# ylongqi/openrec

Measured on NVIDIA H100. Metric: bpr_triplets_per_sec, higher is better.
Workload: dtype f32

## Files before the change

include/orx.h:

```cpp
#ifndef ORX_H_
#define ORX_H_

#include <stdint.h>

#ifdef __cplusplus
extern "C" {
#endif

#define ORX_ABI_VERSION 1
#define ORX_API __attribute__((visibility("default")))

typedef struct orx_ctx* orx_handle_t;
typedef void* orx_stream_t;

enum orx_status {
  ORX_OK = 0,
  ORX_ERR_INVALID = -1,
  ORX_ERR_CUDA = -2,
  ORX_ERR_UNSUPPORTED = -3,
  ORX_ERR_NOMEM = -4
};

enum orx_pair_kind { ORX_PAIR_BPR = 0, ORX_PAIR_UCML = 1 };
enum orx_point_kind { ORX_POINT_GMF = 0, ORX_POINT_WRMF = 1 };
enum orx_score_kind { ORX_SCORE_DOT = 0, ORX_SCORE_NEG_SQDIST = 1 };

enum orx_opt_kind { ORX_OPT_SGD = 0, ORX_OPT_ADAGRAD = 1, ORX_OPT_ADAM_LAZY = 2, ORX_OPT_ADAM_DENSE = 3 };

typedef struct {
  int32_t kind;
  float lr, eps, beta1, beta2;
  int64_t step;
} orx_opt_t;

typedef struct {
  float* var;
  float* s0;
  float* s1;
  int64_t rows;
  int32_t dim;
} orx_table_t;

ORX_API int orx_abi_version(void);
ORX_API const char* orx_last_error_string(void);
ORX_API int orx_create(int device, orx_handle_t* out);
ORX_API int orx_destroy(orx_handle_t h);
ORX_API int orx_device_count(int* n_out_host);
ORX_API int orx_stream_synchronize(orx_handle_t h, orx_stream_t stream);
ORX_API int orx_debug_set_epoch(orx_handle_t h, uint32_t epoch);
enum orx_dispatch_op {
  ORX_OP_GEMM = 0,
  ORX_OP_INTERACT_FWD = 1,
  ORX_OP_INTERACT_BWD = 2,
  ORX_OP_PAIRWISE_STEP = 3,
  ORX_OP_POINTWISE_STEP = 4
};
enum orx_dispatch_variant {
  ORX_VARIANT_GEMM_TMA = 0,
  ORX_VARIANT_GEMM_SIMT = 1,
  ORX_VARIANT_INTERACT_WARP = 2,
  ORX_VARIANT_INTERACT = 3,
  ORX_VARIANT_STEP = 4,
  ORX_VARIANT_STEP_PIPE = 5,
  ORX_VARIANT_STEP_GENERIC = 6
};
#define ORX_DISPATCH_LOG_CAP 64
ORX_API int orx_debug_dispatch_log(orx_handle_t h, int32_t* rec_host, int32_t cap, int32_t* n_host);

ORX_API int orx_profile_enable(orx_handle_t h, int32_t on);
ORX_API int orx_profile_read(orx_handle_t h, float* ms_host, int32_t n_phases, int32_t* n_steps_host);

ORX_API int orx_fill_uniform(orx_handle_t h, float* dst, int64_t n, float lo, float hi, uint64_t seed, orx_stream_t s);
ORX_API int orx_gather(orx_handle_t h, const float* tab, int64_t rows, int32_t dim, const void* ids, int32_t id_is_i64,
               int64_t n, float* out, int32_t* n_bad, orx_stream_t s);
ORX_API int orx_censor(orx_handle_t h, float* tab, int64_t rows, int32_t dim, const int32_t* ids, int32_t n,
               float min_norm, orx_stream_t s);

ORX_API int orx_pairwise_step(orx_handle_t h, int32_t kind, const orx_table_t* user, const orx_table_t* item,
                      const orx_table_t* item_bias, const int32_t* uid, const int32_t* pid, const int32_t* nid,
                      int32_t B, float margin, float c_loss, float c_l2, const orx_opt_t* opt_host,
                      float* out4, orx_stream_t s);
ORX_API int orx_pairwise_step_host(orx_handle_t h, int32_t kind, const orx_table_t* user, const orx_table_t* item,
                           const orx_table_t* item_bias, const int32_t* uid_host, const int32_t* pid_host,
                           const int32_t* nid_host, int32_t B, float margin, float c_loss, float c_l2,
                           const orx_opt_t* opt_host, float* out4_host, orx_stream_t s);
ORX_API int orx_pairwise_prefetch(orx_handle_t h, const orx_table_t* user, const orx_table_t* item, const int32_t* uid,
                                  const int32_t* pid, const int32_t* nid, int32_t B, int32_t opt_kind, int32_t ids_ready,
                                  orx_stream_t ids_stream);
ORX_API int orx_pairwise_fwd(orx_handle_t h, int32_t kind, const orx_table_t* user, const orx_table_t* item,
                     const orx_table_t* item_bias, const int32_t* uid, const int32_t* pid, const int32_t* nid,
                     int32_t B, float margin, float* out4, orx_stream_t s);
ORX_API int orx_pairwise_grad(orx_handle_t h, int32_t kind, const orx_table_t* user, const orx_table_t* item,
                      const orx_table_t* item_bias, const int32_t* uid, const int32_t* pid, const int32_t* nid,
                      int32_t B, float margin, float c_loss, float c_l2, float* d_user, float* d_pos, float* d_neg,
                      float* d_bp, float* d_bn, float* g_out, orx_stream_t s);

ORX_API int orx_pointwise_step(orx_handle_t h, int32_t kind, const orx_table_t* user, const orx_table_t* item,
                       const orx_table_t* item_bias, const orx_table_t* w, const int32_t* uid, const int32_t* iid,
                       const float* label, int32_t B, float a, float b, int32_t use_sigmoid, float c_loss,
                       float c_l2, const orx_opt_t* opt_host, float* out4, orx_stream_t s);
ORX_API int orx_pointwise_fwd(orx_handle_t h, int32_t kind, const orx_table_t* user, const orx_table_t* item,
                      const orx_table_t* item_bias, const orx_table_t* w, const int32_t* uid, const int32_t* iid,
                      const float* label, int32_t B, float a, float b, int32_t use_sigmoid, float* out4,
                      orx_stream_t s);
ORX_API int orx_pointwise_grad(orx_handle_t h, int32_t kind, const orx_table_t* user, const orx_table_t* item,
                       const orx_table_t* item_bias, const orx_table_t* w, const int32_t* uid, const int32_t* iid,
                       const float* label, int32_t B, float a, float b, int32_t use_sigmoid, float c_loss,
                       float c_l2, float* d_user, float* d_item, float* d_bias, float* d_w, float* g_out,
                       orx_stream_t s);

ORX_API int orx_sparse_apply(orx_handle_t h, const orx_table_t* tab, const int32_t* ids, const float* values,
                             int32_t n, const orx_opt_t* opt_host, orx_stream_t s);
ORX_API int orx_sparse_apply_strided(orx_handle_t h, const orx_table_t* tab, const int32_t* ids, int64_t id_stride,
                                     const float* values, int64_t value_ld, int32_t n, const orx_opt_t* opt_host,
                                     orx_stream_t s);
ORX_API int orx_owner_bucket_combined(orx_handle_t h, const int32_t* ids, int32_t n, int32_t n_user, int64_t total_users,
                                      int32_t world, int32_t* counts, int32_t* send_local, int32_t* slot, orx_stream_t s);
ORX_API int orx_pairwise_grad_rows(orx_handle_t h, int32_t kind, const float* rows, int64_t ld, int32_t dim,
                                   const int32_t* uslot, const int32_t* pslot, const int32_t* nslot, int32_t B,
                                   float margin, float c_loss, float c_l2, float inv_B, float* d_rows, float* out4,
                                   orx_stream_t s);

typedef struct {
  int32_t world, rank, dim, batch_cap, home_cap, req_cap, gin_cap, timeout_ms;
  void *tripbox, *idbox, *got, *gotb, *gin, *ginb, *meta, *flags;
} orx_shard_t;
ORX_API int orx_peer_alloc(orx_handle_t h, int64_t bytes, void** dev_ptr_out, uint8_t* handle_out64);
ORX_API int orx_peer_open(orx_handle_t h, const uint8_t* handle64, void** dev_ptr_out);
ORX_API int orx_peer_close(orx_handle_t h, void* dev_ptr);
ORX_API int orx_peer_free(orx_handle_t h, void* dev_ptr);
ORX_API int orx_shard_sizes(const orx_shard_t* x_host, int64_t* n8_host);
ORX_API int orx_shard_step(orx_handle_t h, int32_t kind, const orx_shard_t* x_host, const orx_table_t* user,
                           const orx_table_t* item, const orx_table_t* item_bias, const int32_t* uid, const int32_t* pid,
                           const int32_t* nid, int32_t B, const int32_t* next_uid, const int32_t* next_pid,
                           const int32_t* next_nid, int32_t next_B, int64_t total_users, int64_t total_items, float margin,
                           float c_loss, float c_l2, float inv_B, const orx_opt_t* opt_host, int32_t epoch,
                           int32_t phase_lo, int32_t phase_hi, float* out4, orx_stream_t s);
ORX_API int orx_dense_apply(orx_handle_t h, float* var, float* s0, float* s1, const float* grad, int64_t n,
                    const orx_opt_t* opt_host, orx_stream_t s);

ORX_API int orx_gather_strided(orx_handle_t h, const float* tab, int64_t rows, int32_t dim, const int32_t* ids,
                               int64_t id_stride, int64_t n, float* out, int64_t out_ld, int32_t* n_bad,
                               orx_stream_t s);
ORX_API int orx_mlp_layer_fwd(orx_handle_t h, const float* x, int64_t ldx, int32_t B, int32_t in, const float* w,
                              const float* bias, int32_t out, int32_t act, float* y, int64_t ldy, orx_stream_t s);
ORX_API int orx_mlp_layer_bwd(orx_handle_t h, const float* x, int64_t ldx, const float* y, int64_t ldy, const float* w,
                              int32_t B, int32_t in, int32_t out, int32_t act, float* dy, int64_t lddy, float* dx,
                              int64_t lddx, float* dw, float* db, orx_stream_t s);
ORX_API int orx_interact_fwd(orx_handle_t h, const float* emb, int64_t emb_ld, const float* dense, int64_t dense_ld,
                             int32_t B, int32_t F, int32_t D, int32_t self_interaction, int32_t mode, float* out,
// ... 37 lines not shown
```

openrec_b200/_lib.py:

```python
from __future__ import annotations

import ctypes as C
import os

HERE = os.path.dirname(os.path.abspath(__file__))
LIB_PATH = os.path.join(HERE, "csrc", "liborx.so")

ORX_PAIR_BPR, ORX_PAIR_UCML = 0, 1
ORX_POINT_GMF, ORX_POINT_WRMF = 0, 1
ORX_SCORE_DOT, ORX_SCORE_NEG_SQDIST = 0, 1
ORX_OPT_SGD, ORX_OPT_ADAGRAD, ORX_OPT_ADAM_LAZY, ORX_OPT_ADAM_DENSE = 0, 1, 2, 3
ORX_OP_GEMM, ORX_OP_INTERACT_FWD, ORX_OP_INTERACT_BWD, ORX_OP_PAIRWISE_STEP, ORX_OP_POINTWISE_STEP = 0, 1, 2, 3, 4
ORX_VARIANT_GEMM_TMA, ORX_VARIANT_GEMM_SIMT, ORX_VARIANT_INTERACT_WARP, ORX_VARIANT_INTERACT = 0, 1, 2, 3
ORX_VARIANT_STEP, ORX_VARIANT_STEP_PIPE, ORX_VARIANT_STEP_GENERIC = 4, 5, 6
ORX_DISPATCH_LOG_CAP = 64


class OrxOpt(C.Structure):
    _fields_ = [("kind", C.c_int32), ("lr", C.c_float), ("eps", C.c_float), ("beta1", C.c_float),
                ("beta2", C.c_float), ("step", C.c_int64)]


class OrxTable(C.Structure):
    _fields_ = [("var", C.c_void_p), ("s0", C.c_void_p), ("s1", C.c_void_p), ("rows", C.c_int64),
                ("dim", C.c_int32)]


class OrxShard(C.Structure):
    _fields_ = [("world", C.c_int32), ("rank", C.c_int32), ("dim", C.c_int32), ("batch_cap", C.c_int32),
                ("home_cap", C.c_int32), ("req_cap", C.c_int32), ("gin_cap", C.c_int32), ("timeout_ms", C.c_int32),
                ("tripbox", C.c_void_p), ("idbox", C.c_void_p), ("got", C.c_void_p), ("gotb", C.c_void_p),
                ("gin", C.c_void_p), ("ginb", C.c_void_p), ("meta", C.c_void_p), ("flags", C.c_void_p)]


class OrxSampler(C.Structure):
    _fields_ = [("rec_user", C.c_void_p), ("rec_item", C.c_void_p), ("perm_cur", C.c_void_p), ("perm_next", C.c_void_p),
                ("cursor", C.c_int64), ("n_records", C.c_int64), ("csr_off", C.c_void_p), ("csr_items", C.c_void_p),
                ("total_users", C.c_int32), ("total_items", C.c_int32)]


_vp, _i32, _i64, _f, _u64 = C.c_void_p, C.c_int32, C.c_int64, C.c_float, C.c_uint64
_T = C.POINTER(OrxTable)
_O = C.POINTER(OrxOpt)
_S = C.POINTER(OrxShard)

SIGNATURES = {
    "orx_abi_version": [],
    "orx_last_error_string": [],
    "orx_create": [C.c_int, C.POINTER(_vp)],
    "orx_destroy": [_vp],
    "orx_device_count": [C.POINTER(C.c_int)],
    "orx_stream_synchronize": [_vp, _vp],
    "orx_debug_set_epoch": [_vp, C.c_uint32],
    "orx_debug_dispatch_log": [_vp, C.POINTER(_i32), _i32, C.POINTER(_i32)],
    "orx_profile_enable": [_vp, _i32],
    "orx_profile_read": [_vp, C.POINTER(C.c_float), _i32, C.POINTER(_i32)],
    "orx_fill_uniform": [_vp, _vp, _i64, _f, _f, _u64, _vp],
    "orx_gather": [_vp, _vp, _i64, _i32, _vp, _i32, _i64, _vp, _vp, _vp],
    "orx_censor": [_vp, _vp, _i64, _i32, _vp, _i32, _f, _vp],
    "orx_pairwise_step": [_vp, _i32, _T, _T, _T, _vp, _vp, _vp, _i32, _f, _f, _f, _O, _vp, _vp],
    "orx_pairwise_step_host": [_vp, _i32, _T, _T, _T, _vp, _vp, _vp, _i32, _f, _f, _f, _O, _vp, _vp],
    "orx_pairwise_prefetch": [_vp, _T, _T, _vp, _vp, _vp, _i32, _i32, _i32, _vp],
    "orx_pairwise_fwd": [_vp, _i32, _T, _T, _T, _vp, _vp, _vp, _i32, _f, _vp, _vp],
    "orx_pairwise_grad": [_vp, _i32, _T, _T, _T, _vp, _vp, _vp, _i32, _f, _f, _f, _vp, _vp, _vp, _vp, _vp, _vp, _vp],
    "orx_sparse_apply": [_vp, _T, _vp, _vp, _i32, _O, _vp],
    "orx_sparse_apply_strided": [_vp, _T, _vp, _i64, _vp, _i64, _i32, _O, _vp],
    "orx_gather_strided": [_vp, _vp, _i64, _i32, _vp, _i64, _i64, _vp, _i64, _vp, _vp],
    "orx_mlp_layer_fwd": [_vp, _vp, _i64, _i32, _i32, _vp, _vp, _i32, _i32, _vp, _i64, _vp],
    "orx_mlp_layer_bwd": [_vp, _vp, _i64, _vp, _i64, _vp, _i32, _i32, _i32, _i32, _vp, _i64, _vp, _i64, _vp, _vp, _vp],
    "orx_interact_fwd": [_vp, _vp, _i64, _vp, _i64, _i32, _i32, _i32, _i32, _i32, _vp, _i64, _vp],
    "orx_interact_bwd": [_vp, _vp, _i64, _vp, _i64, _vp, _i64, _i32, _i32, _i32, _i32, _i32, _vp, _i64, _vp, _i64,
                         _vp],
    "orx_pred_loss": [_vp, _vp, _vp, _i32, _i32, _f, _vp, _vp, _vp, _vp],
    "orx_peer_alloc": [_vp, _i64, C.POINTER(_vp), C.c_char_p],
    "orx_peer_open": [_vp, C.c_char_p, C.POINTER(_vp)],
    "orx_peer_close": [_vp, _vp],
    "orx_peer_free": [_vp, _vp],
    "orx_shard_sizes": [_S, C.POINTER(_i64)],
    "orx_shard_step": [_vp, _i32, _S, _T, _T, _T, _vp, _vp, _vp, _i32, _vp, _vp, _vp, _i32, _i64, _i64, _f, _f, _f, _f, _O,
                       _i32, _i32, _i32, _vp, _vp],
    "orx_owner_bucket_combined": [_vp, _vp, _i32, _i32, _i64, _i32, _vp, _vp, _vp, _vp],
    "orx_pairwise_grad_rows": [_vp, _i32, _vp, _i64, _i32, _vp, _vp, _vp, _i32, _f, _f, _f, _f, _vp, _vp, _vp],
    "orx_pointwise_step": [_vp, _i32, _T, _T, _T, _T, _vp, _vp, _vp, _i32, _f, _f, _i32, _f, _f, _O, _vp, _vp],
    "orx_pointwise_fwd": [_vp, _i32, _T, _T, _T, _T, _vp, _vp, _vp, _i32, _f, _f, _i32, _vp, _vp],
    "orx_pointwise_grad": [_vp, _i32, _T, _T, _T, _T, _vp, _vp, _vp, _i32, _f, _f, _i32, _f, _f,
                           _vp, _vp, _vp, _vp, _vp, _vp],
    "orx_dense_apply": [_vp, _vp, _vp, _vp, _vp, _i64, _O, _vp],
    "orx_score_all": [_vp, _i32, _vp, _i64, _vp, _i32, _vp, _vp, _vp, _i64, _i32, _vp, _vp],
    "orx_sample_pairwise": [_vp, C.POINTER(OrxSampler), _u64, _i64, _i32, _vp, _vp, _vp, _vp],
    "orx_sample_stratified": [_vp, C.POINTER(OrxSampler), _u64, _i64, _i32, _f, _vp, _vp, _vp, _vp, _vp],
    "orx_sample_per_positive": [_vp, C.POINTER(OrxSampler), _u64, _i64, _i32, _i32, _vp, _vp, _vp, _vp],
    "orx_rank_metrics": [_vp, _vp, _vp, _vp, _i32, _i64, C.POINTER(_i32), _i32, _vp, _vp, _vp, _vp],
}

_lib = None


def lib():
    global _lib
    if _lib is None:
        if not os.path.exists(LIB_PATH):
            raise RuntimeError(
                f"liborx.so not found at {LIB_PATH}: build it with `python -m openrec_b200.build` "
                "(there is no CPU fallback)")
        l = C.CDLL(LIB_PATH)
        for name, argtypes in SIGNATURES.items():
            fn = getattr(l, name)
            fn.argtypes = argtypes
            fn.restype = C.c_char_p if name == "orx_last_error_string" else C.c_int
        _lib = l
    return _lib


def last_error() -> str:
    s = lib().orx_last_error_string()
    return s.decode() if s else ""


def check(rc: int, what: str = "liborx"):
    if rc != 0:
        raise RuntimeError(f"{what} failed (status {rc}): {last_error()}")
```

openrec_b200/csrc/orx_common.cuh:

```cuda
#pragma once
#include <cuda_runtime.h>
#include <stdint.h>
#include <stdio.h>

#include <initializer_list>
#include <type_traits>

#include "../../include/orx.h"

void orx_set_error(const char* fmt, ...);

#define ORX_CUDA(call)                                                                         \
  do {                                                                                         \
    cudaError_t e__ = (call);                                                                  \
    if (e__ != cudaSuccess) {                                                                  \
      orx_set_error("%s:%d %s -> %s", __FILE__, __LINE__, #call, cudaGetErrorString(e__));     \
      return ORX_ERR_CUDA;                                                                     \
    }                                                                                          \
  } while (0)

#define ORX_REQUIRE(cond, msg)                                  \
  do {                                                          \
    if (!(cond)) {                                              \
      orx_set_error("%s: %s", __func__, msg);                   \
      return ORX_ERR_INVALID;                                   \
    }                                                           \
  } while (0)

#define ORX_LAUNCH_CHECK() ORX_CUDA(cudaGetLastError())

struct OrxHash {
  unsigned long long* slots;
  int32_t* didx;
  int32_t* did;
  int32_t* counter;
  uint32_t mask;
  int32_t shift;
  uint32_t epoch;
};

struct orx_ctx {
  int device;
  int num_sms;
  int64_t cap_B;
  OrxHash hu, hi;
  OrxHash pf_u[2], pf_i[2];
  int32_t* counters;
  float *gu, *gi, *gb, *gw;
  int64_t g_rows_u, g_rows_i;
  int32_t g_dim;
  float* partials;
  int32_t cap_partials;
  int32_t* ids_stage[2];
  float* out_stage[2];
  int64_t stage_cap;
  uint32_t stage_flip;
  int prof_on, prof_n, prof_cap;
  int prof_step;
  cudaEvent_t* prof_ev;
  int32_t* bucket_cursor;
  cudaStream_t side_stream;
  cudaEvent_t side_ev;
  cudaEvent_t pf_done[2], pf_free[2], stage_free[2];
  int pf_free_valid[2], stage_free_valid[2];
  int pf_valid, pf_set, pf_next, pf_B, pf_mode;
  const int32_t *pf_uid, *pf_pid, *pf_nid;
  int64_t pf_rows_u, pf_rows_i;
  uint32_t epoch;
  void* shard_ws;
  int32_t dispatch[ORX_DISPATCH_LOG_CAP][8];
  int64_t dispatch_n;
};

static inline void orx_log_dispatch(orx_ctx* c, int op, int variant, int TA, int TB, int M, int N, int K, int S) {
  int32_t* r = c->dispatch[c->dispatch_n++ % ORX_DISPATCH_LOG_CAP];
  r[0] = op; r[1] = variant; r[2] = TA; r[3] = TB; r[4] = M; r[5] = N; r[6] = K; r[7] = S;
}

int orx_next_epoch(orx_ctx* c, cudaStream_t st);
void orx_shard_ws_release(orx_ctx* c);

#define ORX_PROF_EV 8
static inline bool orx_prof_sampled(const orx_ctx* c) {
  return c->prof_on && (c->prof_step & 7) == 0 && c->prof_n < c->prof_cap;
}
static inline void orx_prof_mark(orx_ctx* c, int k, cudaStream_t st) {
  if (orx_prof_sampled(c)) cudaEventRecord(c->prof_ev[c->prof_n * ORX_PROF_EV + k], st);
}
static inline void orx_prof_next(orx_ctx* c) {
  if (!c->prof_on) return;
  if (orx_prof_sampled(c)) c->prof_n++;
  c->prof_step++;
}

static inline int orx_current_sms() {
  static int sms[64] = {0};
  int dev = 0;
  if (cudaGetDevice(&dev) != cudaSuccess || dev < 0 || dev >= 64) return 132;
  if (sms[dev] <= 0 && cudaDeviceGetAttribute(&sms[dev], cudaDevAttrMultiProcessorCount, dev) != cudaSuccess) sms[dev] = 0;
  return sms[dev] > 0 ? sms[dev] : 132;
}

int orx_ensure_workspace(orx_ctx* c, int64_t B, int32_t dim);
int orx_ensure_stage(orx_ctx* c, int64_t n_ints);

template <int V, int... Vs, typename F>
static inline auto orx_dispatch(int v, F&& f) {
  if constexpr (sizeof...(Vs) == 0) {
    return f(std::integral_constant<int, V>{});
  } else {
    if (v == V) return f(std::integral_constant<int, V>{});
    return orx_dispatch<Vs...>(v, f);
  }
}
template <typename F>
static inline auto orx_dispatch_opt(int opt_kind, F&& f) {
  return orx_dispatch<ORX_OPT_SGD, ORX_OPT_ADAGRAD, ORX_OPT_ADAM_LAZY, ORX_OPT_ADAM_DENSE>(opt_kind, f);
}

static inline bool orx_opt_kind_ok(int kind) { return kind >= ORX_OPT_SGD && kind <= ORX_OPT_ADAM_DENSE; }
bool orx_opt_slots_ok(int kind, std::initializer_list<const orx_table_t*> tabs);

struct OrxOptDev {
  int32_t kind;
  float lr;
  float eps, beta1, beta2;
};

#ifdef __CUDACC__

#define ORX_FULL 0xffffffffu

__device__ __forceinline__ void orx_pdl_wait() { asm volatile("griddepcontrol.wait;" ::: "memory"); }
__device__ __forceinline__ void orx_pdl_trigger() { asm volatile("griddepcontrol.launch_dependents;" ::: "memory"); }

bool orx_pdl_enabled();

template <typename... KArgs, typename... Args>
static inline cudaError_t orx_launch_pdl(void (*kern)(KArgs...), dim3 grid, dim3 block, size_t smem, cudaStream_t st,
                                         Args... args) {
  cudaLaunchConfig_t cfg = {};
  cfg.gridDim = grid;
  cfg.blockDim = block;
  cfg.dynamicSmemBytes = smem;
  cfg.stream = st;
  cudaLaunchAttribute attr[1];
  attr[0].id = cudaLaunchAttributeProgrammaticStreamSerialization;
  attr[0].val.programmaticStreamSerializationAllowed = 1;
  cfg.attrs = attr;
  cfg.numAttrs = orx_pdl_enabled() ? 1 : 0;
// ... 243 lines not shown
  float *U, *Us0, *Us1;
  float *I, *Is0, *Is1;
  float *Bv, *Bs0, *Bs1;
  int D;
  OrxOptDev opt;
  OrxHash hu, hi;
  float *gu, *gi, *gb;
  const float* partials;
  int n_partials;
  float loss_scale;
  int32_t* counters;
  float* out4;
  float *W, *Ws0, *Ws1, *gw;
  float c_l2;
};

#ifdef __CUDACC__
template <int OPT>
__device__ __forceinline__ void orx_tail_rows(const TailArgs& a, int nu, int ni) {
  typedef OrxOptSlots<OPT> SL;
  constexpr bool ZERO_ONLY = SL::STAGE_ONLY;
  const int lane = threadIdx.x & 31;
  const int gwarp = (blockIdx.x * blockDim.x + threadIdx.x) >> 5;
  const int nwarps = (gridDim.x * blockDim.x) >> 5;
  const int D = a.D;
  const float4 z4 = make_float4(0.f, 0.f, 0.f, 0.f);
  const int sub = lane >> 3, sl = lane & 7;
  for (int r0 = gwarp * 4; r0 < nu + ni; r0 += nwarps * 4) {
    const int r = r0 + sub;
    const bool on = r < nu + ni;
    const bool is_u = on && r < nu;
    const int d = on ? (is_u ? r : r - nu) : 0;
    const int id = on ? (is_u ? a.hu.did[d] : a.hi.did[d]) : 0;
    float* G = (is_u ? a.gu : a.gi) + (int64_t)d * D;
    float* W = (is_u ? a.U : a.I) + (int64_t)id * D;
    float* P0 = (is_u ? a.Us0 : a.Is0) + (int64_t)id * D;
    float* P1 = (is_u ? a.Us1 : a.Is1) + (int64_t)id * D;
    if ((D & 3) == 0) {
      const int nq = D >> 2;
      for (int e0 = 0; e0 < nq; e0 += 32) {
        float4 g[4], w[4], s0v[4], s1v[4];
#pragma unroll
        for (int k = 0; k < 4; ++k) {
          const int e = e0 + sl + 8 * k;
          const bool ld = on && e < nq;
          g[k] = ld ? __ldcg(reinterpret_cast<const float4*>(G) + e) : z4;
          w[k] = (ld && !ZERO_ONLY) ? orx_ld4_stream(W + 4 * e) : z4;
          s0v[k] = (ld && SL::S0) ? orx_ld4_stream(P0 + 4 * e) : z4;
          s1v[k] = (ld && SL::S1) ? orx_ld4_stream(P1 + 4 * e) : z4;
        }
#pragma unroll
        for (int k = 0; k < 4; ++k) {
          const int e = e0 + sl + 8 * k;
          if (!on || e >= nq) continue;
          if (!ZERO_ONLY) {
            orx_st4_stream(W + 4 * e, orx_apply4<OPT>(w[k], g[k], s0v[k], s1v[k], a.opt));
            if (SL::S0) orx_st4_stream(P0 + 4 * e, s0v[k]);
            if (SL::S1) orx_st4_stream(P1 + 4 * e, s1v[k]);
          }
          __stcg(reinterpret_cast<float4*>(G) + e, z4);
        }
      }
    } else if (on) {
      for (int e = sl; e < D; e += 8) {
        if (!ZERO_ONLY) orx_update1<OPT>(W + e, P0 + e, P1 + e, W[e], G[e], a.opt);
        G[e] = 0.f;
      }
    }
    if (on && !is_u && sl == 0) {
      if (!ZERO_ONLY) orx_update1<OPT>(a.Bv + id, a.Bs0 + id, a.Bs1 + id, a.Bv[id], a.gb[d], a.opt);
      a.gb[d] = 0.f;
    }
  }
}
#endif

OrxOptDev orx_opt_to_dev(const orx_opt_t* o);
int orx_launch_index_build_strided(orx_ctx* c, const int32_t* a, int64_t stride, int64_t rows, int32_t n,
                                   bool stage_all, cudaStream_t st);
TailArgs orx_tail_args(const orx_ctx* c, const orx_table_t* user, const orx_table_t* item, const orx_table_t* bias,
                       const OrxHash& hu, const OrxHash& hi, const OrxOptDev& o);
int orx_launch_adam_sweeps(orx_ctx* c, const orx_table_t* user, const orx_table_t* item, const orx_table_t* bias,
                           const OrxHash& hu, const OrxHash& hi, const OrxOptDev& o, cudaStream_t st);
int orx_launch_tail(orx_ctx* c, const TailArgs& ta, int opt_kind, cudaStream_t st);
int orx_ensure_partials(orx_ctx* c, int need, cudaStream_t st);
int orx_launch_reduce_partials(const float* partials, int n, float loss_scale, float* out4, cudaStream_t st);
int orx_launch_index_build(orx_ctx* c, const int32_t* a, int64_t rows_a, const int32_t* b0, const int32_t* b1,
                           int64_t rows_b, int32_t n, int mode , cudaStream_t st);
```

openrec_b200/csrc/orx_ctx.cu:

```cuda
#include <stdarg.h>
#include <stdlib.h>
#include <string.h>

#include "orx_common.cuh"

static thread_local char g_err[512] = "";

void orx_set_error(const char* fmt, ...) {
  va_list ap;
  va_start(ap, fmt);
  vsnprintf(g_err, sizeof(g_err), fmt, ap);
  va_end(ap);
}

extern "C" const char* orx_last_error_string(void) { return g_err; }

bool orx_pdl_enabled() {
  static int v = -1;
  if (v < 0) {
    const char* e = getenv("ORX_PDL");
    v = (e && atoi(e) == 0) ? 0 : 1;
  }
  return v != 0;
}
extern "C" int orx_abi_version(void) { return ORX_ABI_VERSION; }

extern "C" int orx_device_count(int* n) {
  ORX_REQUIRE(n != nullptr, "null output");
  *n = 0;
  ORX_CUDA(cudaGetDeviceCount(n));
  return ORX_OK;
}

static void free_hash(OrxHash& t) {
  cudaFree(t.slots);
  cudaFree(t.didx);
  cudaFree(t.did);
  t.slots = nullptr;
  t.didx = nullptr;
  t.did = nullptr;
}

static void free_workspace(orx_ctx* c) {
  free_hash(c->hu);
  free_hash(c->hi);
  for (int k = 0; k < 2; ++k) {
    free_hash(c->pf_u[k]);
    free_hash(c->pf_i[k]);
  }
  cudaFree(c->gu);
  cudaFree(c->gi);
  cudaFree(c->gb);
  cudaFree(c->gw);
  c->gu = c->gi = c->gb = c->gw = nullptr;
  c->cap_B = 0;
  c->g_dim = 0;
}

static uint32_t pow2_at_least(int64_t n) {
  uint32_t p = 1024;
  while ((int64_t)p < n) p <<= 1;
  return p;
}

static int alloc_hash(OrxHash& t, int64_t lookups, int32_t* counter) {
  uint32_t cap = pow2_at_least(4 * lookups);
  int lg = 0;
  while ((1u << lg) < cap) ++lg;
  t.mask = cap - 1;
  t.shift = 32 - lg;
  t.counter = counter;
  ORX_CUDA(cudaMalloc(&t.slots, sizeof(unsigned long long) * cap));
  ORX_CUDA(cudaMalloc(&t.didx, sizeof(int32_t) * cap));
  ORX_CUDA(cudaMalloc(&t.did, sizeof(int32_t) * (lookups + 1)));
  ORX_CUDA(cudaMemset(t.slots, 0, sizeof(unsigned long long) * cap));
  return ORX_OK;
}

int orx_ensure_workspace(orx_ctx* c, int64_t B, int32_t dim) {
  if (B <= c->cap_B && dim <= c->g_dim) return ORX_OK;
  int64_t nb = B > c->cap_B ? B : c->cap_B;
  int32_t nd = dim > c->g_dim ? dim : c->g_dim;
  ORX_CUDA(cudaDeviceSynchronize());
  free_workspace(c);
  int rc;
  if ((rc = alloc_hash(c->hu, nb, c->counters + 0)) != ORX_OK) return rc;
  if ((rc = alloc_hash(c->hi, 2 * nb, c->counters + 1)) != ORX_OK) return rc;
  for (int k = 0; k < 2; ++k) {
    if ((rc = alloc_hash(c->pf_u[k], nb, c->counters + 4 * (1 + k))) != ORX_OK) return rc;
    if ((rc = alloc_hash(c->pf_i[k], 2 * nb, c->counters + 4 * (1 + k) + 1)) != ORX_OK) return rc;
  }
  c->pf_valid = 0;
  c->pf_free_valid[0] = c->pf_free_valid[1] = 0;
  c->g_rows_u = nb;
  c->g_rows_i = 2 * nb;
  size_t bu = sizeof(float) * (size_t)c->g_rows_u * nd, bi = sizeof(float) * (size_t)c->g_rows_i * nd;
  ORX_CUDA(cudaMalloc(&c->gu, bu));
  ORX_CUDA(cudaMalloc(&c->gi, bi));
  ORX_CUDA(cudaMalloc(&c->gb, sizeof(float) * (size_t)c->g_rows_i));
  ORX_CUDA(cudaMalloc(&c->gw, sizeof(float) * (size_t)nd));
  ORX_CUDA(cudaMemset(c->gu, 0, bu));
  ORX_CUDA(cudaMemset(c->gi, 0, bi));
  ORX_CUDA(cudaMemset(c->gb, 0, sizeof(float) * (size_t)c->g_rows_i));
  ORX_CUDA(cudaMemset(c->gw, 0, sizeof(float) * (size_t)nd));
  ORX_CUDA(cudaMemset(c->counters, 0, sizeof(int32_t) * 16));
  ORX_CUDA(cudaDeviceSynchronize());
  c->cap_B = nb;
  c->g_dim = nd;
  c->epoch = 0;
  return ORX_OK;
}

static int zero_hash(OrxHash& t) {
  if (!t.slots) return ORX_OK;
  ORX_CUDA(cudaMemset(t.slots, 0, sizeof(unsigned long long) * ((size_t)t.mask + 1)));
  return ORX_OK;
}

int orx_next_epoch(orx_ctx* c, cudaStream_t ) {
  c->epoch = (c->epoch + 1) & 0x7fffffffu;
  if (c->epoch == 0) {
    ORX_CUDA(cudaDeviceSynchronize());
    int rc;
    if ((rc = zero_hash(c->hu)) || (rc = zero_hash(c->hi))) return rc;
    for (int k = 0; k < 2; ++k)
      if ((rc = zero_hash(c->pf_u[k])) || (rc = zero_hash(c->pf_i[k]))) return rc;
    ORX_CUDA(cudaDeviceSynchronize());
    c->epoch = 1;
  }
  c->hu.epoch = c->hi.epoch = c->epoch;
  return ORX_OK;
}

extern "C" int orx_debug_set_epoch(orx_handle_t h, uint32_t epoch) {
  ORX_REQUIRE(h != nullptr && epoch < 0x80000000u, "null handle / epoch must be < 2^31");
  h->epoch = epoch;
  return ORX_OK;
}

extern "C" int orx_debug_dispatch_log(orx_handle_t h, int32_t* rec, int32_t cap, int32_t* n) {
  ORX_REQUIRE(h != nullptr && n && cap >= 0 && (rec || cap == 0), "bad arguments");
  const int64_t held = h->dispatch_n < ORX_DISPATCH_LOG_CAP ? h->dispatch_n : ORX_DISPATCH_LOG_CAP;
  const int64_t first = h->dispatch_n - held;
  const int64_t take = held < cap ? held : cap;
  for (int64_t i = 0; i < take; ++i) memcpy(rec + 8 * i, h->dispatch[(first + i) % ORX_DISPATCH_LOG_CAP], 8 * sizeof(int32_t));
  *n = (int32_t)take;
  h->dispatch_n = 0;
  return ORX_OK;
}

int orx_ensure_stage(orx_ctx* c, int64_t n_ints) {
  if (n_ints <= c->stage_cap) return ORX_OK;
  ORX_CUDA(cudaDeviceSynchronize());
  for (int i = 0; i < 2; ++i) {
    cudaFree(c->ids_stage[i]);
    c->ids_stage[i] = nullptr;
    ORX_CUDA(cudaMalloc(&c->ids_stage[i], sizeof(int32_t) * (size_t)n_ints));
  }
  c->stage_cap = n_ints;
  return ORX_OK;
}

extern "C" int orx_create(int device, orx_handle_t* out) {
  ORX_REQUIRE(out != nullptr, "null output handle");
  *out = nullptr;
  int n = 0;
  ORX_CUDA(cudaGetDeviceCount(&n));
  ORX_REQUIRE(device >= 0 && device < n, "device ordinal out of range");
  ORX_CUDA(cudaSetDevice(device));
  cudaDeviceProp prop;
  ORX_CUDA(cudaGetDeviceProperties(&prop, device));
  if (prop.major != 9 || prop.minor != 0) {
    orx_set_error("orx_create: liborx is built for sm_90a only; device %d is sm_%d%d", device, prop.major,
                  prop.minor);
    return ORX_ERR_UNSUPPORTED;
  }
  orx_ctx* c = new orx_ctx();
  memset(c, 0, sizeof(*c));
  c->device = device;
  c->num_sms = prop.multiProcessorCount;
  c->cap_partials = c->num_sms * 64;
  if (cudaMalloc(&c->counters, sizeof(int32_t) * 16) != cudaSuccess ||
      cudaMalloc(&c->partials, sizeof(float) * 2 * (size_t)c->cap_partials) != cudaSuccess ||
      cudaMalloc(&c->out_stage[0], sizeof(float) * 8) != cudaSuccess ||
      cudaMalloc(&c->out_stage[1], sizeof(float) * 8) != cudaSuccess) {
    orx_set_error("orx_create: workspace allocation failed: %s", cudaGetErrorString(cudaGetLastError()));
    delete c;
    return ORX_ERR_NOMEM;
  }
  cudaMemset(c->counters, 0, sizeof(int32_t) * 16);
  *out = c;
  return ORX_OK;
}

extern "C" int orx_destroy(orx_handle_t h) {
  if (!h) return ORX_OK;
  cudaSetDevice(h->device);
  cudaDeviceSynchronize();
  free_workspace(h);
  for (int i = 0; i < 2; ++i) {
    cudaFree(h->ids_stage[i]);
    cudaFree(h->out_stage[i]);
  }
  cudaFree(h->counters);
  cudaFree(h->partials);
  cudaFree(h->bucket_cursor);
  orx_shard_ws_release(h);
  if (h->side_stream) {
    cudaStreamDestroy(h->side_stream);
    cudaEventDestroy(h->side_ev);
    for (int i = 0; i < 2; ++i) {
      cudaEventDestroy(h->pf_done[i]);
      cudaEventDestroy(h->pf_free[i]);
      cudaEventDestroy(h->stage_free[i]);
    }
  }
  if (h->prof_ev) {
    for (int i = 0; i < h->prof_cap * ORX_PROF_EV; ++i) cudaEventDestroy(h->prof_ev[i]);
    delete[] h->prof_ev;
  }
  delete h;
  return ORX_OK;
}

extern "C" int orx_profile_enable(orx_handle_t h, int32_t on) {
  ORX_REQUIRE(h != nullptr, "null handle");
  ORX_CUDA(cudaSetDevice(h->device));
  if (on && !h->prof_ev) {
    h->prof_cap = 1024;
    h->prof_ev = new cudaEvent_t[h->prof_cap * ORX_PROF_EV];
    for (int i = 0; i < h->prof_cap * ORX_PROF_EV; ++i) ORX_CUDA(cudaEventCreate(&h->prof_ev[i]));
  }
  h->prof_on = on ? 1 : 0;
// ... 49 lines not shown
```

openrec_b200/csrc/orx_dlrm.cu:

```cuda
#include "orx_common.cuh"

__global__ void __launch_bounds__(256) k_gather_strided(const float* __restrict__ tab, int64_t rows, int D,
                                                        const int32_t* __restrict__ ids, int64_t id_stride, int64_t n,
                                                        float* __restrict__ out, int64_t out_ld, int32_t* n_bad) {
  const int lane = threadIdx.x & 31;
  const int64_t nw = ((int64_t)gridDim.x * blockDim.x) >> 5;
  const bool vec = ((D & 3) == 0) && ((out_ld & 3) == 0);
  for (int64_t b = ((int64_t)blockIdx.x * blockDim.x + threadIdx.x) >> 5; b < n; b += nw) {
    const int64_t id = ids[b * id_stride];
    const bool ok = id >= 0 && id < rows;
    if (!ok && lane == 0 && n_bad) atomicAdd(n_bad, 1);
    if (vec) {
      const float4* src = reinterpret_cast<const float4*>(tab + id * D);
      float4* dst = reinterpret_cast<float4*>(out + b * out_ld);
      for (int e = lane; e < D / 4; e += 32) dst[e] = ok ? __ldg(src + e) : make_float4(0.f, 0.f, 0.f, 0.f);
    } else {
      for (int e = lane; e < D; e += 32) out[b * out_ld + e] = ok ? __ldg(tab + id * D + e) : 0.f;
    }
  }
}

extern "C" int orx_gather_strided(orx_handle_t h, const float* tab, int64_t rows, int32_t dim, const int32_t* ids,
                                  int64_t id_stride, int64_t n, float* out, int64_t out_ld, int32_t* n_bad,
                                  orx_stream_t s) {
  ORX_REQUIRE(h != nullptr && tab && ids && out, "null pointer");
  ORX_REQUIRE(rows > 0 && dim > 0 && n >= 0 && id_stride >= 1 && out_ld >= dim, "bad sizes");
  if (n == 0) return ORX_OK;
  ORX_CUDA(cudaSetDevice(h->device));
  int64_t blocks = (n + 7) / 8;
  if (blocks > (int64_t)h->num_sms * 32) blocks = (int64_t)h->num_sms * 32;
  k_gather_strided<<<(int)blocks, 256, 0, (cudaStream_t)s>>>(tab, rows, dim, ids, id_stride, n, out, out_ld, n_bad);
  ORX_LAUNCH_CHECK();
  return ORX_OK;
}

#define ORX_MAX_F 64

__device__ __forceinline__ bool inter_selected(int mode, int self, int i, int j) {
  return mode == 0 ? (self ? j >= i : j > i) : (self ? j <= i : j < i);
}

__device__ __forceinline__ int inter_index(int mode, int self, int F, int i, int j) {
  if (mode == 0) return self ? i * F - i * (i - 1) / 2 + (j - i) : i * (F - 1) - i * (i - 1) / 2 + (j - i - 1);
  return self ? i * (i + 1) / 2 + j : i * (i - 1) / 2 + j;
}

__device__ __forceinline__ void inter_load(const float* __restrict__ emb, int64_t emb_ld, const float* __restrict__ dense,
                                           int64_t dense_ld, int b, int F, int D, float* sz) {
  const int warp = threadIdx.x >> 5, lane = threadIdx.x & 31, nw = blockDim.x >> 5, Dp = D + 1;
  for (int f = warp; f < F; f += nw) {
    const float* src = f < F - 1 ? emb + (int64_t)b * emb_ld + (int64_t)f * D : dense + (int64_t)b * dense_ld;
    for (int d = lane; d < D; d += 32) sz[f * Dp + d] = src[d];
  }
}

__global__ void __launch_bounds__(128) k_interact_fwd(const float* __restrict__ emb, int64_t emb_ld,
                                                      const float* __restrict__ dense, int64_t dense_ld, int B, int F,
                                                      int D, int self, int mode, float* __restrict__ out,
                                                      int64_t out_ld) {
  extern __shared__ float sz[];
  const int b = blockIdx.x;
  if (b >= B) return;
  const int Dp = D + 1;
  inter_load(emb, emb_ld, dense, dense_ld, b, F, D, sz);
  __syncthreads();
  for (int c = threadIdx.x; c < F * F; c += blockDim.x) {
    const int i = c / F, j = c - i * F;
    if (!inter_selected(mode, self, i, j)) continue;
    float a0 = 0.f, a1 = 0.f, a2 = 0.f, a3 = 0.f;
    if (mode == 1 || j == i) {
      const float* zi = sz + i * Dp;
      const float* zj = sz + j * Dp;
      int d = 0;
      for (; d + 3 < D; d += 4) {
        a0 += zi[d] * zj[d];
        a1 += zi[d + 1] * zj[d + 1];
        a2 += zi[d + 2] * zj[d + 2];
        a3 += zi[d + 3] * zj[d + 3];
      }
      for (; d < D; ++d) a0 += zi[d] * zj[d];
    }
    out[(int64_t)b * out_ld + inter_index(mode, self, F, i, j)] = (a0 + a1) + (a2 + a3);
  }
}

__global__ void __launch_bounds__(128) k_interact_bwd(const float* __restrict__ emb, int64_t emb_ld,
                                                      const float* __restrict__ dense, int64_t dense_ld,
                                                      const float* __restrict__ dout, int64_t dout_ld, int B, int F,
                                                      int D, int self, int mode, float* __restrict__ demb,
                                                      int64_t demb_ld, float* __restrict__ ddense,
                                                      int64_t ddense_ld) {
  extern __shared__ float sm[];
  const int b = blockIdx.x;
  if (b >= B) return;
  const int Dp = D + 1;
  float* sz = sm;
  float* sp = sm + F * Dp;
  inter_load(emb, emb_ld, dense, dense_ld, b, F, D, sz);
  for (int c = threadIdx.x; c < F * F; c += blockDim.x) {
    const int i = c / F, j = c - i * F;
    float v = 0.f;
    if (inter_selected(mode, self, i, j) && (mode == 1 || j == i))
      v = dout[(int64_t)b * dout_ld + inter_index(mode, self, F, i, j)];
    sp[c] = v;
  }
  __syncthreads();
  const int warp = threadIdx.x >> 5, lane = threadIdx.x & 31, nw = blockDim.x >> 5;
  for (int i = warp; i < F; i += nw) {
    for (int d = lane; d < D; d += 32) {
      float acc = 0.f;
      for (int j = 0; j < F; ++j) acc += (sp[i * F + j] + sp[j * F + i]) * sz[j * Dp + d];
// ... 74 lines not shown
        const bool up = lane & 1;
        const float send = up ? v[0] : v[1], keep = up ? v[1] : v[0];
        v[0] = keep + __shfl_xor_sync(0xffffffffu, send, 1);
      }
      if (p0 + lane < P) out[(int64_t)b * out_ld + p0 + lane] = v[0];
    }
  }
}

__global__ void __launch_bounds__(INTER_WARPS * 32) k_interact_bwd_warp(const float* __restrict__ emb, int64_t emb_ld,
                                                                        const float* __restrict__ dense, int64_t dense_ld,
                                                                        const float* __restrict__ dout, int64_t dout_ld,
                                                                        int B, int F, int D, int self,
                                                                        float* __restrict__ demb, int64_t demb_ld,
                                                                        float* __restrict__ ddense, int64_t ddense_ld) {
  extern __shared__ float4 sb_all[];
  constexpr int WLD = 36;
  const int lane = threadIdx.x & 31, wi = threadIdx.x >> 5;
  const size_t per_warp = (size_t)F * 32 + (size_t)F * WLD / 4;
  float4* sz = sb_all + (size_t)wi * per_warp;
  float* sw = reinterpret_cast<float*>(sz + (size_t)F * 32);
  const int nq = D >> 2;
  for (int b = blockIdx.x * INTER_WARPS + wi; b < B; b += gridDim.x * INTER_WARPS) {
    __syncwarp();
    inter_load_warp(emb, emb_ld, dense, dense_ld, b, F, D, lane, sz);
    for (int c = lane; c < F * WLD; c += 32) sw[c] = 0.f;
    __syncwarp();
    const int P = self ? F * (F + 1) / 2 : F * (F - 1) / 2;
    for (int p = lane; p < P; p += 32) {
      int i = (int)((sqrtf(8.f * (float)p + 1.f) - 1.f) * 0.5f) + (self ? 0 : 1);
      while ((self ? i * (i + 1) / 2 : i * (i - 1) / 2) > p) --i;
      while ((self ? (i + 1) * (i + 2) / 2 : (i + 1) * i / 2) <= p) ++i;
      const int j = p - (self ? i * (i + 1) / 2 : i * (i - 1) / 2);
      const float g = dout[(int64_t)b * dout_ld + p];
      if (i == j) sw[j * WLD + i] = 2.f * g;
      else { sw[j * WLD + i] = g; sw[i * WLD + j] = g; }
    }
    __syncwarp();
    for (int i0 = 0; i0 < F; i0 += 9) {
      float4 acc[9];
#pragma unroll
      for (int k = 0; k < 9; ++k) acc[k] = make_float4(0.f, 0.f, 0.f, 0.f);
      for (int j = 0; j < F; ++j) {
        const float4 zj = sz[j * 32 + lane];
        const float* wr = sw + j * WLD + i0;
        float wv[9];
#pragma unroll
        for (int k = 0; k < 9; ++k) wv[k] = wr[k];
#pragma unroll
        for (int k = 0; k < 9; ++k) {
          acc[k].x += wv[k] * zj.x; acc[k].y += wv[k] * zj.y; acc[k].z += wv[k] * zj.z; acc[k].w += wv[k] * zj.w;
        }
      }
      if (lane < nq) {
#pragma unroll
        for (int k = 0; k < 9; ++k) {
          const int i = i0 + k;
          if (i >= F) break;
          if (i < F - 1) {
            reinterpret_cast<float4*>(demb + (int64_t)b * demb_ld + (int64_t)i * D)[lane] = acc[k];
          } else {
            float4* dd = reinterpret_cast<float4*>(ddense + (int64_t)b * ddense_ld) + lane;
            float4 o = *dd;
            o.x += acc[k].x; o.y += acc[k].y; o.z += acc[k].z; o.w += acc[k].w;
            *dd = o;
          }
        }
      }
    }
  }
}

static bool inter_fast_ok(int F, int D, int mode, const void* a, const void* b, int64_t lda, int64_t ldb) {
  return mode == 1 && F >= 2 && F <= 32 && (D & 3) == 0 && D <= 128 && (lda & 3) == 0 && (ldb & 3) == 0 &&
         ((((uintptr_t)a) | ((uintptr_t)b)) & 15) == 0;
}

extern "C" int orx_interact_fwd(orx_handle_t h, const float* emb, int64_t emb_ld, const float* dense,
                                int64_t dense_ld, int32_t B, int32_t F, int32_t D, int32_t self_interaction,
                                int32_t mode, float* out, int64_t out_ld, orx_stream_t s) {
  ORX_REQUIRE(h != nullptr && dense && out && (F == 1 || emb), "null pointer");
  ORX_REQUIRE(B >= 0 && F >= 1 && F <= ORX_MAX_F && D > 0 && (mode == 0 || mode == 1), "bad sizes/mode");
  if (B == 0) return ORX_OK;
  ORX_CUDA(cudaSetDevice(h->device));
  if (inter_fast_ok(F, D, mode, emb ? (const void*)emb : (const void*)dense, dense, emb_ld, dense_ld)) {
    const size_t sm = sizeof(float4) * (size_t)INTER_WARPS * F * 32;
    static bool attr = false;
    if (!attr) { ORX_CUDA(cudaFuncSetAttribute(k_interact_fwd_warp, cudaFuncAttributeMaxDynamicSharedMemorySize, 200 * 1024)); attr = true; }
    int grid = (B + INTER_WARPS - 1) / INTER_WARPS;
    if (grid > h->num_sms * 4) grid = h->num_sms * 4;
    k_interact_fwd_warp<<<grid, INTER_WARPS * 32, sm, (cudaStream_t)s>>>(emb, emb_ld, dense, dense_ld, B, F, D, self_interaction, out, out_ld);
    ORX_LAUNCH_CHECK();
    orx_log_dispatch(h, ORX_OP_INTERACT_FWD, ORX_VARIANT_INTERACT_WARP, 0, 0, B, F, D, 1);
    return ORX_OK;
  }
  const size_t smem = sizeof(float) * (size_t)F * (D + 1);
  ORX_REQUIRE(smem <= 200 * 1024, "F*D too large for the interaction kernel");
  if (smem > 48 * 1024) ORX_CUDA(cudaFuncSetAttribute(k_interact_fwd, cudaFuncAttributeMaxDynamicSharedMemorySize, (int)smem));
  k_interact_fwd<<<B, 128, smem, (cudaStream_t)s>>>(emb, emb_ld, dense, dense_ld, B, F, D, self_interaction, mode, out, out_ld);
  ORX_LAUNCH_CHECK();
  orx_log_dispatch(h, ORX_OP_INTERACT_FWD, ORX_VARIANT_INTERACT, 0, 0, B, F, D, 1);
  return ORX_OK;
}

extern "C" int orx_interact_bwd(orx_handle_t h, const float* emb, int64_t emb_ld, const float* dense,
                                int64_t dense_ld, const float* dout, int64_t dout_ld, int32_t B, int32_t F, int32_t D,
                                int32_t self_interaction, int32_t mode, float* demb, int64_t demb_ld, float* ddense,
                                int64_t ddense_ld, orx_stream_t s) {
  ORX_REQUIRE(h != nullptr && dense && dout && ddense && (F == 1 || (emb && demb)), "null pointer");
  ORX_REQUIRE(B >= 0 && F >= 1 && F <= ORX_MAX_F && D > 0 && (mode == 0 || mode == 1), "bad sizes/mode");
  if (B == 0) return ORX_OK;
  ORX_CUDA(cudaSetDevice(h->device));
  if (inter_fast_ok(F, D, mode, emb ? (const void*)emb : (const void*)dense, dense, emb_ld, dense_ld) && (demb_ld & 3) == 0 &&
      (ddense_ld & 3) == 0 && ((((uintptr_t)(demb ? (const void*)demb : (const void*)ddense)) | ((uintptr_t)ddense)) & 15) == 0) {
    const size_t sm = (size_t)INTER_WARPS * (sizeof(float4) * (size_t)F * 32 + sizeof(float) * (size_t)F * 36);
    static bool attr = false;
    if (!attr) { ORX_CUDA(cudaFuncSetAttribute(k_interact_bwd_warp, cudaFuncAttributeMaxDynamicSharedMemorySize, 200 * 1024)); attr = true; }
    int grid = (B + INTER_WARPS - 1) / INTER_WARPS;
    if (grid > h->num_sms * 3) grid = h->num_sms * 3;
    k_interact_bwd_warp<<<grid, INTER_WARPS * 32, sm, (cudaStream_t)s>>>(emb, emb_ld, dense, dense_ld, dout, dout_ld, B, F, D, self_interaction, demb, demb_ld, ddense, ddense_ld);
    ORX_LAUNCH_CHECK();
    orx_log_dispatch(h, ORX_OP_INTERACT_BWD, ORX_VARIANT_INTERACT_WARP, 0, 0, B, F, D, 1);
    return ORX_OK;
  }
  const size_t smem = sizeof(float) * ((size_t)F * (D + 1) + (size_t)F * F);
  ORX_REQUIRE(smem <= 200 * 1024, "F*D too large for the interaction kernel");
  if (smem > 48 * 1024) ORX_CUDA(cudaFuncSetAttribute(k_interact_bwd, cudaFuncAttributeMaxDynamicSharedMemorySize, (int)smem));
  k_interact_bwd<<<B, 128, smem, (cudaStream_t)s>>>(emb, emb_ld, dense, dense_ld, dout, dout_ld, B, F, D, self_interaction, mode, demb, demb_ld, ddense, ddense_ld);
  ORX_LAUNCH_CHECK();
  orx_log_dispatch(h, ORX_OP_INTERACT_BWD, ORX_VARIANT_INTERACT, 0, 0, B, F, D, 1);
  return ORX_OK;
}

template <int TA, int TB>
__global__ void __launch_bounds__(256) k_gemm(const float* __restrict__ A, int64_t lda, const float* __restrict__ Bm,
                                              int64_t ldb, float* __restrict__ C, int64_t ldc, int M, int N, int K,
                                              const float* __restrict__ bias, int act, float* __restrict__ part) {
  constexpr int T = 64, KC = 16;
  __shared__ float sa[KC][T + 4], sb[KC][T + 4];
  const int tx = threadIdx.x & 15, ty = threadIdx.x >> 4;
  const int m0 = blockIdx.y * T, n0 = blockIdx.x * T;
  float acc[4][4];
#pragma unroll
  for (int i = 0; i < 4; ++i)
#pragma unroll
    for (int j = 0; j < 4; ++j) acc[i][j] = 0.f;
  const int kper = ((K + (int)gridDim.z - 1) / (int)gridDim.z + KC - 1) / KC * KC;
  const int k_lo = blockIdx.z * kper, k_hi = min(K, k_lo + kper);
  for (int k0 = k_lo; k0 < k_hi; k0 += KC) {
    for (int e = threadIdx.x; e < T * KC; e += 256) {
      int r, k;
      if (TA == 0) { r = e / KC; k = e % KC; } else { k = e / T; r = e % T; }
      float v = 0.f;
      if (m0 + r < M && k0 + k < k_hi) v = TA == 0 ? A[(int64_t)(m0 + r) * lda + k0 + k] : A[(int64_t)(k0 + k) * lda + m0 + r];
      sa[k][r] = v;
    }
    for (int e = threadIdx.x; e < T * KC; e += 256) {
      int c, k;
      if (TB == 0) { k = e / T; c = e % T; } else { c = e / KC; k = e % KC; }
      float v = 0.f;
      if (n0 + c < N && k0 + k < k_hi) v = TB == 0 ? Bm[(int64_t)(k0 + k) * ldb + n0 + c] : Bm[(int64_t)(n0 + c) * ldb + k0 + k];
      sb[k][c] = v;
    }
    __syncthreads();
#pragma unroll
    for (int k = 0; k < KC; ++k) {
      float a[4], b[4];
#pragma unroll
      for (int i = 0; i < 4; ++i) a[i] = sa[k][ty * 4 + i];
#pragma unroll
      for (int j = 0; j < 4; ++j) b[j] = sb[k][tx + 16 * j];
#pragma unroll
      for (int i = 0; i < 4; ++i)
#pragma unroll
        for (int j = 0; j < 4; ++j) acc[i][j] += a[i] * b[j];
    }
    __syncthreads();
  }
#pragma unroll
  for (int i = 0; i < 4; ++i) {
    const int m = m0 + ty * 4 + i;
    if (m >= M) continue;
#pragma unroll
    for (int j = 0; j < 4; ++j) {
      const int n = n0 + tx + 16 * j;
      if (n >= N) continue;
      if (gridDim.z > 1) {
        part[(size_t)blockIdx.z * (size_t)M * (size_t)N + (size_t)m * N + n] = acc[i][j];
        continue;
      }
      float v = acc[i][j] + (bias ? bias[n] : 0.f);
      if (act == 1) v = fmaxf(v, 0.f);
      else if (act == 2) v = orx_sigmoid(v);
      C[(int64_t)m * ldc + n] = v;
    }
  }
}

int orx_launch_gemm_tc(orx_ctx* h, int TA, int TB, const float* A, int64_t lda, const float* Bm, int64_t ldb, float* C,
                       int64_t ldc, int M, int N, int K, const float* bias, int act, cudaStream_t st);
float* orx_splitk_workspace(size_t floats);
int orx_launch_splitk_reduce(const float* part, int S, int M, int N, float* C, int64_t ldc, const float* bias, int act,
                             cudaStream_t st);

template <int TA, int TB>
static int launch_gemm(orx_ctx* h, const float* A, int64_t lda, const float* Bm, int64_t ldb, float* C, int64_t ldc, int M,
                       int N, int K, const float* bias, int act, cudaStream_t st) {
  const int rc = orx_launch_gemm_tc(h, TA, TB, A, lda, Bm, ldb, C, ldc, M, N, K, bias, act, st);
  if (rc != ORX_ERR_UNSUPPORTED) return rc;
  const int tiles = ((N + 63) / 64) * ((M + 63) / 64);
  int S = 1;
  const int sms = orx_current_sms();
  if (tiles < sms && K >= 1024) {
    S = (2 * sms + tiles - 1) / tiles;
    if (S > K / 256) S = K / 256;
    if (S > 65535) S = 65535;
  }
  float* part = nullptr;
  if (S > 1) {
    part = orx_splitk_workspace((size_t)S * (size_t)M * (size_t)N);
    if (!part) { orx_set_error("split-K workspace allocation failed"); return ORX_ERR_CUDA; }
  }
  dim3 grid((N + 63) / 64, (M + 63) / 64, S);
  k_gemm<TA, TB><<<grid, 256, 0, st>>>(A, lda, Bm, ldb, C, ldc, M, N, K, bias, act, part);
  ORX_LAUNCH_CHECK();
  orx_log_dispatch(h, ORX_OP_GEMM, ORX_VARIANT_GEMM_SIMT, TA, TB, M, N, K, S);
  if (S > 1) return orx_launch_splitk_reduce(part, S, M, N, C, ldc, bias, act, st);
  return ORX_OK;
}

extern "C" int orx_mlp_layer_fwd(orx_handle_t h, const float* x, int64_t ldx, int32_t B, int32_t in, const float* w,
                                 const float* bias, int32_t out, int32_t act, float* y, int64_t ldy, orx_stream_t s) {
  ORX_REQUIRE(h != nullptr && x && w && y, "null pointer");
  ORX_REQUIRE(B >= 0 && in > 0 && out > 0 && ldx >= in && ldy >= out && act >= 0 && act <= 2, "bad sizes");
  if (B == 0) return ORX_OK;
  ORX_CUDA(cudaSetDevice(h->device));
  return launch_gemm<0, 0>(h, x, ldx, w, out, y, ldy, B, out, in, bias, act, (cudaStream_t)s);
}

__global__ void k_act_bwd(const float* __restrict__ y, int64_t ldy, float* __restrict__ dy, int64_t lddy, int B,
                          int N, int act) {
  const int64_t i = (int64_t)blockIdx.x * blockDim.x + threadIdx.x;
  if (i >= (int64_t)B * N) return;
  const int b = (int)(i / N), n = (int)(i % N);
  const float yv = y[(int64_t)b * ldy + n];
  float g = dy[(int64_t)b * lddy + n];
  if (act == 1) g = yv > 0.f ? g : 0.f;
  else if (act == 2) g = g * yv * (1.f - yv);
  dy[(int64_t)b * lddy + n] = g;
}

__global__ void __launch_bounds__(256) k_col_sum(const float* __restrict__ dz, int64_t ld, int B, int N,
                                                 float* __restrict__ out) {
  __shared__ float sh[8][33];
  const int n = blockIdx.x * 32 + (threadIdx.x & 31), r = threadIdx.x >> 5;
  const int per = (B + (int)gridDim.y - 1) / (int)gridDim.y;
  const int b_lo = blockIdx.y * per, b_hi = min(B, b_lo + per);
  float acc = 0.f;
  if (n < N)
    for (int b = b_lo + r; b < b_hi; b += 8) acc += dz[(int64_t)b * ld + n];
  sh[r][threadIdx.x & 31] = acc;
  __syncthreads();
  if (r == 0 && n < N) {
    float t = 0.f;
    for (int k = 0; k < 8; ++k) t += sh[k][threadIdx.x & 31];
    out[(size_t)blockIdx.y * N + n] = t;
  }
}

extern "C" int orx_mlp_layer_bwd(orx_handle_t h, const float* x, int64_t ldx, const float* y, int64_t ldy,
                                 const float* w, int32_t B, int32_t in, int32_t out, int32_t act, float* dy,
                                 int64_t lddy, float* dx, int64_t lddx, float* dw, float* db, orx_stream_t s) {
  ORX_REQUIRE(h != nullptr && x && y && w && dy && dw, "null pointer");
  ORX_REQUIRE(B > 0 && in > 0 && out > 0 && act >= 0 && act <= 2, "bad sizes");
  ORX_CUDA(cudaSetDevice(h->device));
  cudaStream_t st = (cudaStream_t)s;
  if (act != 0) {
    const int64_t n = (int64_t)B * out;
    k_act_bwd<<<(unsigned)((n + 255) / 256), 256, 0, st>>>(y, ldy, dy, lddy, B, out, act);
    ORX_LAUNCH_CHECK();
  }
  if (db) {
    const int cb = (out + 31) / 32;
    int S = 1;
    if (B >= 4096) {
      S = (2 * h->num_sms + cb - 1) / cb;
      if (S > B / 256) S = B / 256;
    }
    if (S > 1) {
      float* part = orx_splitk_workspace((size_t)S * (size_t)out);
      if (!part) { orx_set_error("split workspace allocation failed"); return ORX_ERR_CUDA; }
      k_col_sum<<<dim3(cb, S), 256, 0, st>>>(dy, lddy, B, out, part);
      ORX_LAUNCH_CHECK();
      const int rc2 = orx_launch_splitk_reduce(part, S, 1, out, db, out, nullptr, 0, st);
      if (rc2) return rc2;
    } else {
      k_col_sum<<<cb, 256, 0, st>>>(dy, lddy, B, out, db);
      ORX_LAUNCH_CHECK();
    }
  }
  int rc = launch_gemm<1, 0>(h, x, ldx, dy, lddy, dw, out, in, out, B, nullptr, 0, st);
  if (rc) return rc;
  if (dx) rc = launch_gemm<0, 1>(h, dy, lddy, w, out, dx, lddx, B, in, out, nullptr, 0, st);
  return rc;
}

__global__ void __launch_bounds__(256) k_pred_loss(const float* __restrict__ pred, const float* __restrict__ label,
                                                   int B, int kind, float thr, float* __restrict__ pred_out,
                                                   float* __restrict__ dpred, float* partials) {
  __shared__ float sh[256];
  float acc = 0.f;
  const float invB = 1.f / (float)B;
  for (int b = blockIdx.x * blockDim.x + threadIdx.x; b < B; b += gridDim.x * blockDim.x) {
    float p = pred[b];
    float pass = 1.f;
    if (thr > 0.f && thr < 1.f) {
      pass = (p >= thr && p <= 1.f - thr) ? 1.f : 0.f;
      p = fminf(fmaxf(p, thr), 1.f - thr);
    }
    const float y = label[b];
    float d;
    if (kind == 0) {
      acc += (y - p) * (y - p);
      d = 2.f * (p - y) * invB;
    } else {
      const float eps = 1e-7f;
      const float ph = fminf(fmaxf(p, eps), 1.f - eps);
      acc += -(y * logf(ph + eps) + (1.f - y) * logf(1.f - ph + eps));
      d = (p >= eps && p <= 1.f - eps) ? -(y / (ph + eps) - (1.f - y) / (1.f - ph + eps)) * invB : 0.f;
    }
    if (pred_out) pred_out[b] = p;
    if (dpred) dpred[b] = d * pass;
  }
  sh[threadIdx.x] = acc;
  __syncthreads();
  for (int s = 128; s > 0; s >>= 1) {
    if (threadIdx.x < s) sh[threadIdx.x] += sh[threadIdx.x + s];
    __syncthreads();
  }
  if (threadIdx.x == 0) {
    partials[2 * blockIdx.x] = sh[0];
    partials[2 * blockIdx.x + 1] = 0.f;
  }
}

extern "C" int orx_pred_loss(orx_handle_t h, const float* pred, const float* label, int32_t B, int32_t kind,
                             float clip_threshold, float* pred_out, float* dpred, float* out4, orx_stream_t s) {
  ORX_REQUIRE(h != nullptr && pred && label && out4, "null pointer");
  ORX_REQUIRE(B > 0 && (kind == 0 || kind == 1), "bad sizes/kind");
  ORX_CUDA(cudaSetDevice(h->device));
  cudaStream_t st = (cudaStream_t)s;
  int blocks = (B + 255) / 256;
  if (blocks > 256) blocks = 256;
  int rc = orx_ensure_partials(h, blocks, st);
  if (rc) return rc;
  k_pred_loss<<<blocks, 256, 0, st>>>(pred, label, B, kind, clip_threshold, pred_out, dpred, h->partials);
  ORX_LAUNCH_CHECK();
  return orx_launch_reduce_partials(h->partials, blocks, 1.0f / (float)B, out4, st);
}
```

openrec_b200/csrc/orx_misc.cu:

```cuda
#include "orx_common.cuh"

__device__ __forceinline__ uint64_t splitmix64(uint64_t x) {
  x += 0x9E3779B97F4A7C15ull;
  x = (x ^ (x >> 30)) * 0xBF58476D1CE4E5B9ull;
  x = (x ^ (x >> 27)) * 0x94D049BB133111EBull;
  return x ^ (x >> 31);
}

__global__ void k_fill_uniform(float* dst, int64_t n, float lo, float hi, uint64_t seed) {
  const int64_t stride = (int64_t)gridDim.x * blockDim.x;
  const float top = nextafterf(hi, lo);
  for (int64_t i = (int64_t)blockIdx.x * blockDim.x + threadIdx.x; i < n; i += stride) {
    const uint64_t r = splitmix64(seed * 0xD1342543DE82EF95ull + (uint64_t)i);
    const float u = (float)(r >> 40) * (1.0f / 16777216.0f);
    dst[i] = fminf(lo + (hi - lo) * u, top);
  }
}

extern "C" int orx_fill_uniform(orx_handle_t h, float* dst, int64_t n, float lo, float hi, uint64_t seed,
                                orx_stream_t s) {
  ORX_REQUIRE(h != nullptr && dst != nullptr && n >= 0, "null handle/dst or negative n");
  if (n == 0) return ORX_OK;
  ORX_CUDA(cudaSetDevice(h->device));
  int64_t blocks = (n + 1023) / 1024;
  if (blocks > (int64_t)h->num_sms * 16) blocks = (int64_t)h->num_sms * 16;
  k_fill_uniform<<<(int)blocks, 256, 0, (cudaStream_t)s>>>(dst, n, lo, hi, seed);
  ORX_LAUNCH_CHECK();
  return ORX_OK;
}

template <typename IdT>
__global__ void __launch_bounds__(256) k_gather(const float* __restrict__ tab, int64_t rows, int D,
                                                const IdT* __restrict__ ids, int64_t n, float* __restrict__ out,
                                                int32_t* n_bad) {
  const int lane = threadIdx.x & 31;
  const int64_t nw = ((int64_t)gridDim.x * blockDim.x) >> 5;
  const bool vec = (D & 3) == 0;
  for (int64_t b = ((int64_t)blockIdx.x * blockDim.x + threadIdx.x) >> 5; b < n; b += nw) {
    const int64_t id = (int64_t)ids[b];
    const bool ok = id >= 0 && id < rows;
    if (!ok && lane == 0 && n_bad) atomicAdd(n_bad, 1);
    if (vec) {
      const float4* src = reinterpret_cast<const float4*>(tab + id * D);
      float4* dst = reinterpret_cast<float4*>(out + b * D);
      for (int e = lane; e < D / 4; e += 32) dst[e] = ok ? __ldg(src + e) : make_float4(0.f, 0.f, 0.f, 0.f);
    } else {
      for (int e = lane; e < D; e += 32) out[b * D + e] = ok ? __ldg(tab + id * D + e) : 0.f;
    }
  }
}

extern "C" int orx_gather(orx_handle_t h, const float* tab, int64_t rows, int32_t dim, const void* ids,
                          int32_t id_is_i64, int64_t n, float* out, int32_t* n_bad, orx_stream_t s) {
  ORX_REQUIRE(h != nullptr && tab, "null pointer");
  ORX_REQUIRE(rows > 0 && dim > 0 && n >= 0, "bad sizes");
  if (n == 0) return ORX_OK;
  ORX_REQUIRE(ids && out, "null pointer");
  ORX_CUDA(cudaSetDevice(h->device));
  int64_t blocks = (n + 7) / 8;
  if (blocks > (int64_t)h->num_sms * 32) blocks = (int64_t)h->num_sms * 32;
  if (id_is_i64)
    k_gather<int64_t><<<(int)blocks, 256, 0, (cudaStream_t)s>>>(tab, rows, dim, (const int64_t*)ids, n, out, n_bad);
  else
    k_gather<int32_t><<<(int)blocks, 256, 0, (cudaStream_t)s>>>(tab, rows, dim, (const int32_t*)ids, n, out, n_bad);
  ORX_LAUNCH_CHECK();
  return ORX_OK;
}

__global__ void __launch_bounds__(256) k_censor(float* tab, int64_t rows, int D, const int32_t* __restrict__ ids,
                                                int n, float min_norm, OrxHash hsh) {
  const int lane = threadIdx.x & 31;
  const int nw = (gridDim.x * blockDim.x) >> 5;
  const bool vec = (D & 3) == 0 && D <= 128;
  for (int b0 = ((blockIdx.x * blockDim.x + threadIdx.x) >> 5) * 8; b0 < n; b0 += nw * 8) {
    int32_t my_id = -1;
    if (lane < 8 && b0 + lane < n) {
      const int32_t id = ids[b0 + lane];
      if (id >= 0 && (int64_t)id < rows && orx_hash_insert(hsh, id, 2) == 0u) my_id = id;
    }
    if (vec) {
      const int nq = D >> 2;
      float4 v[8];
#pragma unroll
      for (int k = 0; k < 8; ++k) {
        const int32_t id = __shfl_sync(ORX_FULL, my_id, k);
        v[k] = (id >= 0 && lane < nq) ? __ldcg(reinterpret_cast<const float4*>(tab + (int64_t)id * D) + lane)
                                      : make_float4(0.f, 0.f, 0.f, 0.f);
      }
#pragma unroll
      for (int k = 0; k < 8; ++k) {
        const int32_t id = __shfl_sync(ORX_FULL, my_id, k);
        if (id < 0) continue;
        float sq = v[k].x * v[k].x + v[k].y * v[k].y + v[k].z * v[k].z + v[k].w * v[k].w;
        sq = orx_group_sum<32>(sq);
        const float den = fmaxf(sqrtf(sq), min_norm);
        if (lane < nq)
          __stcg(reinterpret_cast<float4*>(tab + (int64_t)id * D) + lane,
                 make_float4(v[k].x / den, v[k].y / den, v[k].z / den, v[k].w / den));
      }
    } else {
      for (int k = 0; k < 8; ++k) {
        const int32_t id = __shfl_sync(ORX_FULL, my_id, k);
        if (id < 0) continue;
        float* row = tab + (int64_t)id * D;
        float sq = 0.f;
        for (int e = lane; e < D; e += 32) sq += row[e] * row[e];
        sq = orx_group_sum<32>(sq);
        const float den = fmaxf(sqrtf(sq), min_norm);
        for (int e = lane; e < D; e += 32) row[e] = row[e] / den;
      }
    }
  }
}

extern "C" int orx_censor(orx_handle_t h, float* tab, int64_t rows, int32_t dim, const int32_t* ids, int32_t n,
                          float min_norm, orx_stream_t s) {
  ORX_REQUIRE(h != nullptr && tab && ids, "null pointer");
  ORX_REQUIRE(rows > 0 && dim > 0 && n >= 0, "bad sizes");
  if (n == 0) return ORX_OK;
  ORX_CUDA(cudaSetDevice(h->device));
  cudaStream_t st = (cudaStream_t)s;
  int rc = orx_ensure_workspace(h, n, h->g_dim > 0 ? h->g_dim : 1);
  if (rc) return rc;
  if ((rc = orx_next_epoch(h, st))) return rc;
  int blocks = (n + 63) / 64;
  if (blocks > h->num_sms * 8) blocks = h->num_sms * 8;
  k_censor<<<blocks, 256, 0, st>>>(tab, rows, dim, ids, n, min_norm, h->hu);
  ORX_LAUNCH_CHECK();
  return ORX_OK;
}

template <int OPT>
__global__ void k_dense_apply(float* var, float* s0, float* s1, const float* __restrict__ grad, int64_t n,
                              OrxOptDev o) {
  const int64_t stride = (int64_t)gridDim.x * blockDim.x;
  for (int64_t i = (int64_t)blockIdx.x * blockDim.x + threadIdx.x; i < n; i += stride)
    orx_update1<OPT>(var + i, s0 + i, s1 + i, var[i], grad[i], o);
}

extern "C" int orx_dense_apply(orx_handle_t h, float* var, float* s0, float* s1, const float* grad, int64_t n,
                               const orx_opt_t* opt, orx_stream_t s) {
  ORX_REQUIRE(h != nullptr && var && grad && opt, "null pointer");
  ORX_REQUIRE(n >= 0, "negative n");
  if (n == 0) return ORX_OK;
  ORX_CUDA(cudaSetDevice(h->device));
  const OrxOptDev o = orx_opt_to_dev(opt);
  int64_t blocks = (n + 255) / 256;
  if (blocks > (int64_t)h->num_sms * 16) blocks = (int64_t)h->num_sms * 16;
  cudaStream_t st = (cudaStream_t)s;
  ORX_REQUIRE(orx_opt_kind_ok(opt->kind), "unknown optimizer kind");
  const orx_table_t t = {var, s0, s1, n, 1};
  ORX_REQUIRE(orx_opt_slots_ok(opt->kind, {&t}), "optimizer slot rows missing");
  const int kind = opt->kind == ORX_OPT_ADAM_DENSE ? ORX_OPT_ADAM_LAZY : opt->kind;
  orx_dispatch<ORX_OPT_SGD, ORX_OPT_ADAGRAD, ORX_OPT_ADAM_LAZY>(kind, [&](auto O) {
    k_dense_apply<decltype(O)::value><<<(int)blocks, 256, 0, st>>>(var, s0, s1, grad, n, o);
  });
  ORX_LAUNCH_CHECK();
  return ORX_OK;
}

template <int KIND>
__global__ void __launch_bounds__(256) k_score_all(const float* __restrict__ user_tab, int64_t U,
                                                   const int32_t* __restrict__ uid, int Bu,
                                                   const float* __restrict__ scale, const float* __restrict__ item_tab,
                                                   const float* __restrict__ bias, int64_t I, int D,
                                                   float* __restrict__ scores) {
  constexpr int T = 64, KC = 16;
  __shared__ float su[KC][T + 1], si[KC][T + 1];
  const int tx = threadIdx.x & 15, ty = threadIdx.x >> 4;
  const int64_t i0 = (int64_t)blockIdx.x * T;
  const int u0 = blockIdx.y * T;
  float acc[4][4];
#pragma unroll
  for (int a = 0; a < 4; ++a)
#pragma unroll
    for (int b = 0; b < 4; ++b) acc[a][b] = 0.f;
  for (int k0 = 0; k0 < D; k0 += KC) {
    for (int e = threadIdx.x; e < T * KC; e += 256) {
      const int r = e / KC, k = e % KC;
      float uv = 0.f, iv = 0.f;
      if (k0 + k < D) {
        if (u0 + r < Bu) {
          const int32_t id = uid[u0 + r];
          if (id >= 0 && (int64_t)id < U) {
            uv = user_tab[(int64_t)id * D + k0 + k];
            if (scale) uv *= scale[k0 + k];
          }
        }
        if (i0 + r < I) iv = item_tab[(i0 + r) * D + k0 + k];
      }
      su[k][r] = uv;
      si[k][r] = iv;
    }
    __syncthreads();
#pragma unroll
    for (int k = 0; k < KC; ++k) {
      if (k0 + k < D) {
        float uu[4], ii[4];
#pragma unroll
        for (int a = 0; a < 4; ++a) uu[a] = su[k][ty * 4 + a];
#pragma unroll
        for (int b = 0; b < 4; ++b) ii[b] = si[k][tx + 16 * b];
#pragma unroll
        for (int a = 0; a < 4; ++a)
#pragma unroll
          for (int b = 0; b < 4; ++b) {
            if (KIND == ORX_SCORE_DOT) acc[a][b] += uu[a] * ii[b];
            else acc[a][b] -= (uu[a] - ii[b]) * (uu[a] - ii[b]);
          }
      }
    }
    __syncthreads();
  }
#pragma unroll
  for (int a = 0; a < 4; ++a) {
    const int u = u0 + ty * 4 + a;
    if (u >= Bu) continue;
#pragma unroll
    for (int b = 0; b < 4; ++b) {
      const int64_t i = i0 + tx + 16 * b;
      if (i < I) scores[(int64_t)u * I + i] = acc[a][b] + (bias ? bias[i] : 0.f);
    }
  }
}

extern "C" int orx_score_all(orx_handle_t h, int32_t kind, const float* user_tab, int64_t U, const int32_t* uid,
                             int32_t Bu, const float* scale, const float* item_tab, const float* item_bias, int64_t I,
                             int32_t dim, float* scores, orx_stream_t s) {
  ORX_REQUIRE(h != nullptr && user_tab && uid && item_tab && scores, "null pointer");
  ORX_REQUIRE(kind == ORX_SCORE_DOT || kind == ORX_SCORE_NEG_SQDIST, "unknown score kind");
  ORX_REQUIRE(U > 0 && I > 0 && dim > 0 && Bu >= 0, "bad sizes");
  if (Bu == 0) return ORX_OK;
  ORX_CUDA(cudaSetDevice(h->device));
  dim3 grid((unsigned)((I + 63) / 64), (unsigned)((Bu + 63) / 64));
  if (kind == ORX_SCORE_DOT)
    k_score_all<ORX_SCORE_DOT><<<grid, 256, 0, (cudaStream_t)s>>>(user_tab, U, uid, Bu, scale, item_tab, item_bias, I, dim, scores);
  else
    k_score_all<ORX_SCORE_NEG_SQDIST><<<grid, 256, 0, (cudaStream_t)s>>>(user_tab, U, uid, Bu, scale, item_tab, item_bias, I, dim, scores);
  ORX_LAUNCH_CHECK();
  return ORX_OK;
}

#define ORX_MAX_AT 8
struct RankArgs {
  const float* pred;
  const uint8_t *pos, *excl;
  int R;
  int64_t I;
  int at[ORX_MAX_AT];
  int n_at;
  float *auc, *ndcg, *recall;
};

__global__ void __launch_bounds__(256) k_rank_metrics(const RankArgs a) {
  constexpr int TILE = 1024;
  __shared__ int s_idx[TILE];
  __shared__ int s_n, s_npos, s_neval;
  __shared__ unsigned long long s_auc;
  __shared__ double s_dcg[ORX_MAX_AT];
  __shared__ int s_hit[ORX_MAX_AT];
  const int r = blockIdx.x;
  const float* pred = a.pred + (int64_t)r * a.I;
  const uint8_t* pos = a.pos + (int64_t)r * a.I;
  const uint8_t* excl = a.excl + (int64_t)r * a.I;
  const int lane = threadIdx.x & 31, warp = threadIdx.x >> 5, nwarp = blockDim.x >> 5;
  if (threadIdx.x == 0) {
    s_npos = 0;
    s_neval = 0;
    s_auc = 0ull;
  }
  if (threadIdx.x < ORX_MAX_AT) {
    s_dcg[threadIdx.x] = 0.0;
    s_hit[threadIdx.x] = 0;
  }
  __syncthreads();
  int np = 0, ne = 0;
  for (int64_t i = threadIdx.x; i < a.I; i += blockDim.x) {
    np += pos[i] ? 1 : 0;
    ne += (pos[i] || excl[i]) ? 0 : 1;
  }
  atomicAdd(&s_npos, np);
  atomicAdd(&s_neval, ne);
  for (int64_t t0 = 0; t0 < a.I; t0 += TILE) {
    __syncthreads();
    if (threadIdx.x == 0) s_n = 0;
    __syncthreads();
    for (int64_t i = t0 + threadIdx.x; i < t0 + TILE && i < a.I; i += blockDim.x)
      if (pos[i]) s_idx[atomicAdd(&s_n, 1)] = (int)i;
    __syncthreads();
    for (int q = warp; q < s_n; q += nwarp) {
      const int p = s_idx[q];
      const float pp = pred[p];
      const float sp = expf(pp) * (excl[p] ? 0.f : 1.f);
      unsigned int c_auc = 0, c_rank = 0;
      for (int64_t i = lane; i < a.I; i += 32) {
        const float pi = pred[i];
        const bool ex = excl[i] != 0;
        if (!(pos[i] || ex) && pi <= pp) ++c_auc;
        const float si = expf(pi) * (ex ? 0.f : 1.f);
        if (si > sp) ++c_rank;
      }
#pragma unroll
      for (int o = 16; o > 0; o >>= 1) {
        c_auc += __shfl_xor_sync(ORX_FULL, c_auc, o);
        c_rank += __shfl_xor_sync(ORX_FULL, c_rank, o);
      }
      if (lane == 0) {
        atomicAdd(&s_auc, (unsigned long long)c_auc);
        const float ra = (float)c_rank;
        const float rec = 1.f / (logf(ra + 2.f) / logf(2.0f));
        for (int k = 0; k < a.n_at; ++k)
          if (ra < (float)a.at[k]) {
            atomicAdd(&s_dcg[k], (double)rec);
            atomicAdd(&s_hit[k], 1);
          }
      }
    }
  }
  __syncthreads();
  if (threadIdx.x == 0 && a.auc) a.auc[r] = (float)s_auc / (float)((long long)s_npos * (long long)s_neval);
  if (threadIdx.x < a.n_at) {
    if (a.ndcg) a.ndcg[(int64_t)r * a.n_at + threadIdx.x] = (float)s_dcg[threadIdx.x];
    if (a.recall) a.recall[(int64_t)r * a.n_at + threadIdx.x] = (float)s_hit[threadIdx.x] / (float)s_npos;
  }
}

extern "C" int orx_rank_metrics(orx_handle_t h, const float* pred, const uint8_t* pos, const uint8_t* excl, int32_t R,
                                int64_t I, const int32_t* at_host, int32_t n_at, float* auc, float* ndcg,
                                float* recall, orx_stream_t s) {
  ORX_REQUIRE(h != nullptr && pred && pos && excl, "null pointer");
  ORX_REQUIRE(R >= 0 && I > 0 && n_at >= 0 && n_at <= ORX_MAX_AT, "bad sizes (at most 8 cut-offs)");
  ORX_REQUIRE(n_at == 0 || at_host, "null cut-offs");
  if (R == 0) return ORX_OK;
  ORX_CUDA(cudaSetDevice(h->device));
  RankArgs a;
  a.pred = pred; a.pos = pos; a.excl = excl; a.R = R; a.I = I; a.n_at = n_at;
  for (int k = 0; k < ORX_MAX_AT; ++k) a.at[k] = k < n_at ? at_host[k] : 0;
  a.auc = auc; a.ndcg = ndcg; a.recall = recall;
  k_rank_metrics<<<R, 256, 0, (cudaStream_t)s>>>(a);
  ORX_LAUNCH_CHECK();
  return ORX_OK;
}
```

openrec_b200/csrc/orx_pairwise.cu:

```cuda
#include <stdlib.h>
#include <string.h>

#include "orx_common.cuh"
#include "orx_pair.cuh"

__global__ void k_index_build(OrxHash hu, OrxHash hi, const int32_t* __restrict__ a, int64_t rows_a,
                              const int32_t* __restrict__ b0, const int32_t* __restrict__ b1, int64_t rows_b, int n,
                              int stage_all, int32_t* bad) {
  const int i = blockIdx.x * blockDim.x + threadIdx.x;
  if (i >= (b1 ? 3 : 2) * n) return;
  const int t = i < n ? i : (i < 2 * n ? i - n : i - 2 * n);
  const int32_t ia = a[t], ib0 = b0[t], ib1 = b1 ? b1[t] : 0;
  const bool ga = ia >= 0 && (int64_t)ia < rows_a, gb0 = ib0 >= 0 && (int64_t)ib0 < rows_b,
             gb1 = ib1 >= 0 && (int64_t)ib1 < rows_b;
  const bool all = ga && gb0 && gb1;
  if (i < n) {
    if (!ga) atomicAdd(bad, 1);
    else if (all) orx_hash_insert(hu, ia, stage_all);
  } else {
    const bool g = i < 2 * n ? gb0 : gb1;
    if (!g) atomicAdd(bad, 1);
    else if (all) orx_hash_insert(hi, i < 2 * n ? ib0 : ib1, stage_all);
  }
}

__global__ void k_index_build_strided(OrxHash hu, const int32_t* __restrict__ a, int64_t stride, int64_t rows, int n,
                                       int stage_all, int32_t* bad) {
  for (int i = blockIdx.x * blockDim.x + threadIdx.x; i < n; i += gridDim.x * blockDim.x) {
    const int32_t id = a[(int64_t)i * stride];
    if (id >= 0 && (int64_t)id < rows) orx_hash_insert(hu, id, stage_all);
    else atomicAdd(bad, 1);
  }
}

int orx_launch_index_build_strided(orx_ctx* c, const int32_t* a, int64_t stride, int64_t rows, int32_t n,
                                   bool stage_all, cudaStream_t st) {
  if (n <= 0) return ORX_OK;
  int rc = orx_next_epoch(c, st);
  if (rc) return rc;
  k_index_build_strided<<<(n + 255) / 256, 256, 0, st>>>(c->hu, a, stride, rows, n, stage_all ? 1 : 0, c->counters + 3);
  ORX_LAUNCH_CHECK();
  return ORX_OK;
}

int orx_launch_index_build(orx_ctx* c, const int32_t* a, int64_t rows_a, const int32_t* b0, const int32_t* b1,
                           int64_t rows_b, int32_t n, int mode, cudaStream_t st) {
  const int total = (b1 ? 3 : 2) * n;
  if (total <= 0) return ORX_OK;
  int rc = orx_next_epoch(c, st);
  if (rc) return rc;
  k_index_build<<<(total + 255) / 256, 256, 0, st>>>(c->hu, c->hi, a, rows_a, b0, b1, rows_b, n, mode, c->counters + 3);
  ORX_LAUNCH_CHECK();
  return ORX_OK;
}

template <int K, bool S0, bool S1>
struct TripRegs {
  float4 u[K], p[K], n[K];
  float4 us0[K], ps0[K], ns0[K];
  float4 us1[K], ps1[K], ns1[K];
  int fl, uu, pp, nn, du, dp, dn;
  float bp, bn;
};

template <int KIND, int OPT, int D, int CH, int MINB, bool PIPE>
__global__ void __launch_bounds__(256, MINB) k_pair_step(const PairArgs a) {
  constexpr int G = (D / 4 < 32) ? D / 4 : 32;
  constexpr int K = D / (4 * G);
  constexpr int TPW = 32 / G;
  typedef OrxOptSlots<OPT> SL;
  static_assert(CH % TPW == 0, "chunk must be a multiple of the triplets per warp");
  typedef TripRegs<K, SL::S0, SL::S1> Regs;

  const int lane = threadIdx.x & 31;
  const int warp = (blockIdx.x * blockDim.x + threadIdx.x) >> 5;
  const int grp = lane / G, gl = lane % G;
  const int t = warp * CH + lane;
  const float4 z4 = make_float4(0.f, 0.f, 0.f, 0.f);
  orx_pdl_wait();

  int u_id = 0, p_id = 0, n_id = 0, du = -1, dp = -1, dn = -1, flags = 0;
  if (lane < CH && t < a.B) {
    u_id = a.uid[t];
    p_id = a.pid[t];
    n_id = a.nid[t];
    flags = (u_id >= 0 && u_id < a.rowsU && p_id >= 0 && p_id < a.rowsI && n_id >= 0 && n_id < a.rowsI) ? 1 : 0;
  }

  auto load_var = [&](int j, Regs& r) {
    const int src = j + grp;
    r.fl = __shfl_sync(ORX_FULL, flags, src) & 1;
    r.uu = __shfl_sync(ORX_FULL, u_id, src);
    r.pp = __shfl_sync(ORX_FULL, p_id, src);
    r.nn = __shfl_sync(ORX_FULL, n_id, src);
#pragma unroll
    for (int k = 0; k < K; ++k) {
      const int off = (k * G + gl) * 4;
      r.u[k] = r.fl ? orx_ld4_stream(a.U + (int64_t)r.uu * D + off) : z4;
      r.p[k] = r.fl ? orx_ld4_stream(a.I + (int64_t)r.pp * D + off) : z4;
      r.n[k] = r.fl ? orx_ld4_stream(a.I + (int64_t)r.nn * D + off) : z4;
    }
  };
  Regs ra, rb;
  load_var(0, ra);
  if (PIPE && TPW < CH) load_var(TPW, rb);

  float bp = 0.f, bn = 0.f, bps0 = 0.f, bps1 = 0.f, bns0 = 0.f, bns1 = 0.f;
  if (flags & 1) {
    const uint32_t cu = orx_hash_find<!SL::STAGE_ONLY, true>(a.hu, u_id, &du);
    const uint32_t cp = orx_hash_find<!SL::STAGE_ONLY, true>(a.hi, p_id, &dp);
    const uint32_t cn = orx_hash_find<!SL::STAGE_ONLY, true>(a.hi, n_id, &dn);
    bp = orx_ld_keep(a.Bv + p_id);
    bn = orx_ld_keep(a.Bv + n_id);
    if (!SL::STAGE_ONLY) {
      flags |= (cu == 1u ? 2 : 0) | (cp == 1u ? 4 : 0) | (cn == 1u ? 8 : 0);
      if (SL::S0) {
        if (flags & 4) bps0 = orx_ld_keep(a.Bs0 + p_id);
        if (flags & 8) bns0 = orx_ld_keep(a.Bs0 + n_id);
      }
      if (SL::S1) {
        if (flags & 4) bps1 = orx_ld_keep(a.Bs1 + p_id);
        if (flags & 8) bns1 = orx_ld_keep(a.Bs1 + n_id);
      }
    }
  }

  auto load_slots = [&](int j, Regs& r) {
    const int src = j + grp;
    r.fl = __shfl_sync(ORX_FULL, flags, src);
    r.du = __shfl_sync(ORX_FULL, du, src);
    r.dp = __shfl_sync(ORX_FULL, dp, src);
    r.dn = __shfl_sync(ORX_FULL, dn, src);
    r.bp = __shfl_sync(ORX_FULL, bp, src);
    r.bn = __shfl_sync(ORX_FULL, bn, src);
// ... 119 lines not shown
  const int warp = (blockIdx.x * blockDim.x + threadIdx.x) >> 5;
  const int D = a.D;
  float loss_acc = 0.f, l2_acc = 0.f;
  orx_pdl_wait();
  for (int j = 0; j < CH; ++j) {
    const int t = warp * CH + j;
    if (t >= a.B) break;
    const int uu = a.uid[t], pp = a.pid[t], nn = a.nid[t];
    const bool ok = uu >= 0 && uu < a.rowsU && pp >= 0 && pp < a.rowsI && nn >= 0 && nn < a.rowsI;
    if (!ok) {
      if (a.g_out && lane == 0) a.g_out[t] = 0.f;
      continue;
    }
    int du, dp, dn;
    const uint32_t cu = orx_hash_find<!STAGE_ONLY>(a.hu, uu, &du);
    const uint32_t cp = orx_hash_find<!STAGE_ONLY>(a.hi, pp, &dp);
    const uint32_t cn = orx_hash_find<!STAGE_ONLY>(a.hi, nn, &dn);
    const bool fu = !STAGE_ONLY && cu == 1u, fp = !STAGE_ONLY && cp == 1u, fn = !STAGE_ONLY && cn == 1u;
    float* ur = a.U + (int64_t)uu * D;
    float* pr = a.I + (int64_t)pp * D;
    float* nr = a.I + (int64_t)nn * D;
    float s1 = 0.f, s2 = 0.f, sq = 0.f;
    for (int d = lane; d < D; d += 32) {
      const float u = ur[d], p = pr[d], n = nr[d];
      if (KIND == ORX_PAIR_BPR) {
        s1 += u * p;
        s2 += u * n;
      } else {
        s1 += (u - p) * (u - p);
        s2 += (u - n) * (u - n);
      }
      sq += u * u + p * p + n * n;
    }
    l2_acc += sq;
    s1 = orx_group_sum<32>(s1);
    s2 = orx_group_sum<32>(s2);
    const float bp = a.Bv[pp], bn = a.Bv[nn];
    float lt, g;
    pair_score<KIND>(s1, s2, bp, bn, a.margin, a.c_loss, a.inv_B, &lt, &g);
    if (lane == 0) loss_acc += lt;
    for (int d = lane; d < D; d += 32) {
      const float u = ur[d], p = pr[d], n = nr[d];
      float gu, gp, gn;
      pair_grads1<KIND>(g, a.c_l2, u, p, n, &gu, &gp, &gn);
      const int64_t ou = (int64_t)uu * D + d, op = (int64_t)pp * D + d, on = (int64_t)nn * D + d;
      if (fu) orx_update1<OPT>(ur + d, a.Us0 + ou, a.Us1 + ou, u, gu, a.opt);
      else atomicAdd(a.gu + (int64_t)du * D + d, gu);
      if (fp) orx_update1<OPT>(pr + d, a.Is0 + op, a.Is1 + op, p, gp, a.opt);
      else atomicAdd(a.gi + (int64_t)dp * D + d, gp);
      if (fn) orx_update1<OPT>(nr + d, a.Is0 + on, a.Is1 + on, n, gn, a.opt);
      else atomicAdd(a.gi + (int64_t)dn * D + d, gn);
    }
    if (lane == 0) {
      const float gbias = (KIND == ORX_PAIR_BPR) ? g : -g;
      if (fp) orx_update1<OPT>(a.Bv + pp, a.Bs0 + pp, a.Bs1 + pp, bp, gbias, a.opt);
      else atomicAdd(a.gb + dp, gbias);
      if (fn) orx_update1<OPT>(a.Bv + nn, a.Bs0 + nn, a.Bs1 + nn, bn, -gbias, a.opt);
      else atomicAdd(a.gb + dn, -gbias);
      if (a.g_out) a.g_out[t] = g;
    }
  }
  orx_block_partial(loss_acc, l2_acc, a.partials);
}

__global__ void __launch_bounds__(256) k_adam_sweep(float* var, float* m, float* v, int64_t rows, int D, OrxHash h,
                                                    const float* gstage, OrxOptDev o) {
  const int lane = threadIdx.x & 31;
  const int64_t nw = ((int64_t)gridDim.x * blockDim.x) >> 5;
  for (int64_t r = ((int64_t)blockIdx.x * blockDim.x + threadIdx.x) >> 5; r < rows; r += nw) {
    int d = -1;
    uint32_t c = 0;
    if (lane == 0) c = orx_hash_find(h, (int32_t)r, &d);
    c = __shfl_sync(ORX_FULL, c, 0);
    d = __shfl_sync(ORX_FULL, d, 0);
    for (int e = lane; e < D; e += 32)
      orx_adam_dense1(var, m, v, r * D + e, c ? gstage[(int64_t)d * D + e] : 0.f, o);
  }
}


template <int OPT>
__global__ void __launch_bounds__(256) k_sparse_tail(const TailArgs a) {
  __shared__ bool last;
  orx_pdl_wait();
  const int nu = *a.hu.counter, ni = a.I ? *a.hi.counter : 0;
  orx_tail_rows<OPT>(a, nu, ni);

  if (blockIdx.x == 0 && a.out4) {
    double l, q;
    orx_block_sum_partials(a.partials, a.n_partials, a.W, a.W ? a.D : 0, &l, &q);
    if (threadIdx.x == 0) {
      a.out4[0] = (float)(l * (double)a.loss_scale);
      a.out4[1] = (float)(0.5 * q);
      a.out4[2] = (float)a.counters[3];
      a.out4[3] = (float)(nu + ni);
    }
    if (a.W) {
      for (int e = threadIdx.x; e < a.D; e += blockDim.x) {
        const float g = a.gw[e] + a.c_l2 * a.W[e];
        if (OrxOptSlots<OPT>::STAGE_ONLY) orx_adam_dense1(a.W, a.Ws0, a.Ws1, e, g, a.opt);
        else orx_update1<OPT>(a.W + e, a.Ws0 + e, a.Ws1 + e, a.W[e], g, a.opt);
        a.gw[e] = 0.f;
      }
    }
  }
  __syncthreads();
  if (threadIdx.x == 0) {
    __threadfence();
    const int tk = atomicAdd(a.counters + 2, 1);
    last = (tk == (int)gridDim.x - 1);
  }
  __syncthreads();
  if (last && threadIdx.x < 4) a.counters[threadIdx.x] = 0;
}

int orx_launch_tail(orx_ctx* c, const TailArgs& ta, int opt_kind, cudaStream_t st) {
  const int grid = c->num_sms * 4;
  orx_dispatch_opt(opt_kind, [&](auto O) {
    orx_launch_pdl(k_sparse_tail<decltype(O)::value>, dim3(grid), dim3(256), 0, st, ta);
  });
  ORX_LAUNCH_CHECK();
  return ORX_OK;
}

int orx_launch_adam_sweeps(orx_ctx* c, const orx_table_t* user, const orx_table_t* item, const orx_table_t* bias,
                           const OrxHash& hu, const OrxHash& hi, const OrxOptDev& o, cudaStream_t st) {
  struct { const orx_table_t* t; int D; const OrxHash* h; const float* g; } sw[3] = {
      {user, user->dim, &hu, c->gu}, {item, user->dim, &hi, c->gi}, {bias, 1, &hi, c->gb}};
  for (const auto& s : sw) {
    if (!s.t) continue;
    int64_t blocks = (s.t->rows + 7) / 8;
    const int64_t cap = (int64_t)c->num_sms * 16;
    if (blocks > cap) blocks = cap;
    if (blocks < 1) blocks = 1;
    k_adam_sweep<<<(int)blocks, 256, 0, st>>>(s.t->var, s.t->s0, s.t->s1, s.t->rows, s.D, *s.h, s.g, o);
    ORX_LAUNCH_CHECK();
  }
  return ORX_OK;
}

TailArgs orx_tail_args(const orx_ctx* c, const orx_table_t* user, const orx_table_t* item, const orx_table_t* bias,
                       const OrxHash& hu, const OrxHash& hi, const OrxOptDev& o) {
  TailArgs ta;
  memset(&ta, 0, sizeof(ta));
  ta.U = user->var; ta.Us0 = user->s0; ta.Us1 = user->s1;
  if (item) { ta.I = item->var; ta.Is0 = item->s0; ta.Is1 = item->s1; }
  if (bias) { ta.Bv = bias->var; ta.Bs0 = bias->s0; ta.Bs1 = bias->s1; }
  ta.D = user->dim; ta.opt = o; ta.hu = hu; ta.hi = hi;
  ta.gu = c->gu; ta.gi = c->gi; ta.gb = c->gb;
  return ta;
}

template <int KIND, int OPT>
static int launch_pair_step_kind_opt(const PairArgs& pa, cudaStream_t st, int* n_partials, int* variant, int* minb) {
  const int B = pa.B;
  constexpr bool LAZY = (OPT == ORX_OPT_ADAM_LAZY);
  auto go = [&](auto kern, int ch, int v, int mb) {
    const int nw = (B + ch - 1) / ch;
    const int blocks = (nw + 7) / 8;
    *n_partials = blocks;
    *variant = v;
    *minb = mb;
    orx_launch_pdl(kern, dim3(blocks), dim3(256), 0, st, pa);
  };
  constexpr int PV = LAZY ? ORX_VARIANT_STEP : ORX_VARIANT_STEP_PIPE;
  switch (pa.D) {
    case 32: go(k_pair_step<KIND, OPT, 32, 8, 2, !LAZY>, 8, PV, 2); break;
    case 64: go(k_pair_step<KIND, OPT, 64, 8, 2, !LAZY>, 8, PV, 2); break;
    case 128:
      if (LAZY) go(k_pair_step<KIND, OPT, 128, 8, 3, false>, 8, ORX_VARIANT_STEP, 3);
      else go(k_pair_step<KIND, OPT, 128, 8, 4, false>, 8, ORX_VARIANT_STEP, 4);
      break;
    case 256: go(k_pair_step<KIND, OPT, 256, 8, 2, !LAZY>, 8, PV, 2); break;
    default: go(k_pair_step_generic<KIND, OPT>, 8, ORX_VARIANT_STEP_GENERIC, 0); break;
  }
  ORX_LAUNCH_CHECK();
  return ORX_OK;
}

static int check_tables(const orx_table_t* user, const orx_table_t* item, const orx_table_t* bias, int opt_kind) {
  ORX_REQUIRE(user && item && bias, "null table");
  ORX_REQUIRE(user->var && item->var && bias->var, "null table storage");
  ORX_REQUIRE(user->dim == item->dim && user->dim > 0, "user/item dims must match and be positive");
  ORX_REQUIRE(bias->dim == 1 && bias->rows == item->rows, "item_bias must be [item.rows, 1]");
  ORX_REQUIRE(user->rows > 0 && item->rows > 0 && user->rows <= 0x7fffffffLL && item->rows <= 0x7fffffffLL,
              "row counts must fit int32 ids");
  ORX_REQUIRE(orx_opt_slots_ok(opt_kind, {user, item, bias}), "optimizer slot rows missing");
  return ORX_OK;
}

static int side_stream_ensure(orx_ctx* c) {
  if (c->side_stream) return ORX_OK;
  ORX_CUDA(cudaStreamCreateWithFlags(&c->side_stream, cudaStreamNonBlocking));
  ORX_CUDA(cudaEventCreateWithFlags(&c->side_ev, cudaEventDisableTiming));
  for (int i = 0; i < 2; ++i) {
    ORX_CUDA(cudaEventCreateWithFlags(&c->pf_done[i], cudaEventDisableTiming));
    ORX_CUDA(cudaEventCreateWithFlags(&c->pf_free[i], cudaEventDisableTiming));
    ORX_CUDA(cudaEventCreateWithFlags(&c->stage_free[i], cudaEventDisableTiming));
    c->pf_free_valid[i] = c->stage_free_valid[i] = 0;
  }
  return ORX_OK;
}

static int prefetch_drop(orx_ctx* c, cudaStream_t st) {
  if (!c->pf_valid) return ORX_OK;
  const int k = c->pf_set;
  ORX_CUDA(cudaStreamWaitEvent(st, c->pf_done[k], 0));
  ORX_CUDA(cudaMemsetAsync(c->counters + 4 * (1 + k), 0, sizeof(int32_t) * 4, st));
  ORX_CUDA(cudaEventRecord(c->pf_free[k], st));
  c->pf_free_valid[k] = 1;
  c->pf_valid = 0;
  return ORX_OK;
}

static int prefetch_issue(orx_ctx* c, const int32_t* uid, const int32_t* pid, const int32_t* nid, int B, int64_t rows_u,
                          int64_t rows_i, int mode) {
  const int k = c->pf_next;
  c->pf_next ^= 1;
  cudaStream_t ss = c->side_stream;
  if (c->pf_free_valid[k]) ORX_CUDA(cudaStreamWaitEvent(ss, c->pf_free[k], 0));
  int rc = orx_next_epoch(c, ss);
  if (rc) return rc;
  c->pf_u[k].epoch = c->pf_i[k].epoch = c->epoch;
  k_index_build<<<(3 * B + 255) / 256, 256, 0, ss>>>(c->pf_u[k], c->pf_i[k], uid, rows_u, pid, nid, rows_i, B, mode,
                                                     c->counters + 4 * (1 + k) + 3);
  ORX_LAUNCH_CHECK();
  ORX_CUDA(cudaEventRecord(c->pf_done[k], ss));
  c->pf_valid = 1; c->pf_set = k; c->pf_uid = uid; c->pf_pid = pid; c->pf_nid = nid; c->pf_B = B;
  c->pf_rows_u = rows_u; c->pf_rows_i = rows_i; c->pf_mode = mode;
  return ORX_OK;
}

extern "C" int orx_pairwise_prefetch(orx_handle_t h, const orx_table_t* user, const orx_table_t* item, const int32_t* uid,
                                     const int32_t* pid, const int32_t* nid, int32_t B, int32_t opt_kind, int32_t ids_ready,
                                     orx_stream_t ids_stream) {
  ORX_REQUIRE(h != nullptr && user && item && uid && pid && nid && B > 0, "bad arguments");
  ORX_REQUIRE(orx_opt_kind_ok(opt_kind), "unknown optimizer kind");
  ORX_CUDA(cudaSetDevice(h->device));
  cudaStream_t is = (cudaStream_t)ids_stream;
  int rc = orx_ensure_workspace(h, B, user->dim);
  if (rc) return rc;
  if ((rc = side_stream_ensure(h))) return rc;
  if ((rc = prefetch_drop(h, is))) return rc;
  if (!ids_ready) {
    ORX_CUDA(cudaEventRecord(h->side_ev, is));
    ORX_CUDA(cudaStreamWaitEvent(h->side_stream, h->side_ev, 0));
  }
  return prefetch_issue(h, uid, pid, nid, B, user->rows, item->rows, opt_kind == ORX_OPT_ADAM_DENSE ? 1 : 0);
}

static int pairwise_step_impl(orx_ctx* c, int kind, const orx_table_t* user, const orx_table_t* item,
                              const orx_table_t* bias, const int32_t* uid, const int32_t* pid, const int32_t* nid,
                              int B, float margin, float c_loss, float c_l2, const orx_opt_t* opt, float* out4,
                              cudaStream_t st) {
  ORX_REQUIRE(kind == ORX_PAIR_BPR || kind == ORX_PAIR_UCML, "unknown pairwise kind");
  ORX_REQUIRE(opt != nullptr && out4 != nullptr, "null opt/out");
  ORX_REQUIRE(orx_opt_kind_ok(opt->kind), "unknown optimizer kind");
  ORX_REQUIRE(B > 0 && uid && pid && nid, "empty batch or null ids");
  int rc = check_tables(user, item, bias, opt->kind);
  if (rc) return rc;
  const int D = user->dim;
  if ((rc = orx_ensure_workspace(c, B, D))) return rc;
  const bool dense = opt->kind == ORX_OPT_ADAM_DENSE;
  PairArgs pa;
  pa.U = user->var; pa.Us0 = user->s0; pa.Us1 = user->s1;
  pa.I = item->var; pa.Is0 = item->s0; pa.Is1 = item->s1;
  pa.Bv = bias->var; pa.Bs0 = bias->s0; pa.Bs1 = bias->s1;
  pa.rowsU = user->rows; pa.rowsI = item->rows; pa.D = D;
  pa.uid = uid; pa.pid = pid; pa.nid = nid; pa.B = B;
  pa.margin = margin; pa.c_loss = c_loss; pa.c_l2 = c_l2; pa.inv_B = 1.0f / (float)B;
  pa.opt = orx_opt_to_dev(opt);
  pa.gu = c->gu; pa.gi = c->gi; pa.gb = c->gb;
  pa.g_out = nullptr;
  if ((rc = orx_ensure_partials(c, (B + 63) / 64 + 8 > c->num_sms ? (B + 63) / 64 + 8 : c->num_sms, st))) return rc;
  pa.partials = c->partials;
  orx_prof_mark(c, 0, st);
  int set = 0;
  if (c->pf_valid && c->pf_uid == uid && c->pf_pid == pid && c->pf_nid == nid && c->pf_B == B &&
      c->pf_rows_u == user->rows && c->pf_rows_i == item->rows && c->pf_mode == (dense ? 1 : 0)) {
    set = 1 + c->pf_set;
    ORX_CUDA(cudaStreamWaitEvent(st, c->pf_done[c->pf_set], 0));
    c->pf_valid = 0;
  } else {
    if ((rc = prefetch_drop(c, st))) return rc;
    if ((rc = orx_launch_index_build(c, uid, user->rows, pid, nid, item->rows, B, dense ? 1 : 0, st))) return rc;
  }
  const OrxHash& HU = set ? c->pf_u[set - 1] : c->hu;
  const OrxHash& HI = set ? c->pf_i[set - 1] : c->hi;
  int32_t* ctr = c->counters + 4 * set;
  orx_prof_mark(c, 1, st);
  pa.hu = HU; pa.hi = HI;
  int n_partials = 0, variant = 0, minb = 0;
  rc = orx_dispatch<ORX_PAIR_BPR, ORX_PAIR_UCML>(kind, [&](auto K) {
    return orx_dispatch_opt(opt->kind, [&](auto O) {
      return launch_pair_step_kind_opt<decltype(K)::value, decltype(O)::value>(pa, st, &n_partials, &variant, &minb);
    });
  });
  if (rc) return rc;
  orx_log_dispatch(c, ORX_OP_PAIRWISE_STEP, variant, kind, opt->kind, B, D, minb, set);
  orx_prof_mark(c, 2, st);
  if (dense && (rc = orx_launch_adam_sweeps(c, user, item, bias, HU, HI, pa.opt, st))) return rc;
  TailArgs ta = orx_tail_args(c, user, item, bias, HU, HI, pa.opt);
  ta.partials = c->partials; ta.n_partials = n_partials;
  ta.loss_scale = (kind == ORX_PAIR_BPR) ? pa.inv_B : 1.0f;
  ta.counters = ctr; ta.out4 = out4;
  rc = orx_launch_tail(c, ta, opt->kind, st);
  if (set) {
    ORX_CUDA(cudaEventRecord(c->pf_free[set - 1], st));
    c->pf_free_valid[set - 1] = 1;
  }
  orx_prof_mark(c, 3, st);
  orx_prof_next(c);
  return rc;
}

extern "C" int orx_pairwise_step(orx_handle_t h, int32_t kind, const orx_table_t* user, const orx_table_t* item,
                                 const orx_table_t* item_bias, const int32_t* uid, const int32_t* pid,
                                 const int32_t* nid, int32_t B, float margin, float c_loss, float c_l2,
                                 const orx_opt_t* opt, float* out4, orx_stream_t s) {
  ORX_REQUIRE(h != nullptr, "null handle");
  ORX_CUDA(cudaSetDevice(h->device));
  return pairwise_step_impl(h, kind, user, item, item_bias, uid, pid, nid, B, margin, c_loss, c_l2, opt, out4,
                            (cudaStream_t)s);
}

extern "C" int orx_pairwise_step_host(orx_handle_t h, int32_t kind, const orx_table_t* user, const orx_table_t* item,
                                      const orx_table_t* item_bias, const int32_t* uid_host, const int32_t* pid_host,
                                      const int32_t* nid_host, int32_t B, float margin, float c_loss, float c_l2,
                                      const orx_opt_t* opt, float* out4_host, orx_stream_t s) {
  ORX_REQUIRE(h != nullptr, "null handle");
  ORX_REQUIRE(B > 0 && uid_host && pid_host && nid_host && out4_host && user && item && opt, "empty batch or null host buffers");
  ORX_CUDA(cudaSetDevice(h->device));
  cudaStream_t st = (cudaStream_t)s;
  int rc = orx_ensure_stage(h, 3 * (int64_t)B);
  if (rc) return rc;
  if ((rc = orx_ensure_workspace(h, B, user->dim))) return rc;
  if ((rc = side_stream_ensure(h))) return rc;
  if ((rc = prefetch_drop(h, st))) return rc;
  const uint32_t f = (h->stage_flip++) & 1u;
  int32_t* ids = h->ids_stage[f];
  cudaStream_t ss = h->side_stream;
  if (h->stage_free_valid[f]) ORX_CUDA(cudaStreamWaitEvent(ss, h->stage_free[f], 0));
  ORX_CUDA(cudaMemcpyAsync(ids, uid_host, sizeof(int32_t) * B, cudaMemcpyHostToDevice, ss));
  ORX_CUDA(cudaMemcpyAsync(ids + B, pid_host, sizeof(int32_t) * B, cudaMemcpyHostToDevice, ss));
  ORX_CUDA(cudaMemcpyAsync(ids + 2 * (int64_t)B, nid_host, sizeof(int32_t) * B, cudaMemcpyHostToDevice, ss));
  if ((rc = prefetch_issue(h, ids, ids + B, ids + 2 * (int64_t)B, B, user->rows, item->rows,
                           opt->kind == ORX_OPT_ADAM_DENSE ? 1 : 0)))
    return rc;
  rc = pairwise_step_impl(h, kind, user, item, item_bias, ids, ids + B, ids + 2 * (int64_t)B, B, margin, c_loss, c_l2,
                          opt, h->out_stage[f], st);
  if (rc) return rc;
  ORX_CUDA(cudaEventRecord(h->stage_free[f], st));
  h->stage_free_valid[f] = 1;
  ORX_CUDA(cudaMemcpyAsync(out4_host, h->out_stage[f], sizeof(float) * 4, cudaMemcpyDeviceToHost, st));
  return ORX_OK;
}

struct PairGradArgs {
  const float *U, *I, *Bv;
  int64_t rowsU, rowsI;
  int D;
  const int32_t *uid, *pid, *nid;
  int B;
  float margin, c_loss, c_l2, inv_B;
  float *d_user, *d_pos, *d_neg, *d_bp, *d_bn, *g_out;
  float* partials;
  int64_t ld;
};

template <int KIND>
__global__ void __launch_bounds__(256) k_pair_fwd_grad(const PairGradArgs a) {
  const int lane = threadIdx.x & 31;
  const int warp = (blockIdx.x * blockDim.x + threadIdx.x) >> 5;
  const int D = a.D;
  const bool row_form = a.ld != 0;
  const int64_t ld = row_form ? a.ld : D;
  float loss_acc = 0.f, l2_acc = 0.f;
  for (int j = 0; j < 8; ++j) {
    const int t = warp * 8 + j;
    if (t >= a.B) break;
    const int uu = a.uid[t], pp = a.pid[t], nn = a.nid[t];
    const bool ok = uu >= 0 && uu < a.rowsU && pp >= 0 && pp < a.rowsI && nn >= 0 && nn < a.rowsI;
    float s1 = 0.f, s2 = 0.f, sq = 0.f, bp = 0.f, bn = 0.f, lt = 0.f, g = 0.f;
    const float* ur = a.U + (int64_t)uu * ld;
    const float* pr = a.I + (int64_t)pp * ld;
    const float* nr = a.I + (int64_t)nn * ld;
    if (ok) {
      for (int d = lane; d < D; d += 32) {
        const float u = ur[d], p = pr[d], n = nr[d];
        if (KIND == ORX_PAIR_BPR) {
          s1 += u * p;
          s2 += u * n;
        } else {
          s1 += (u - p) * (u - p);
          s2 += (u - n) * (u - n);
        }
        sq += u * u + p * p + n * n;
      }
      bp = row_form ? pr[D] : a.Bv[pp];
      bn = row_form ? nr[D] : a.Bv[nn];
    }
    l2_acc += sq;
    s1 = orx_group_sum<32>(s1);
    s2 = orx_group_sum<32>(s2);
    if (ok) pair_score<KIND>(s1, s2, bp, bn, a.margin, a.c_loss, a.inv_B, &lt, &g);
    if (lane == 0) loss_acc += lt;
    if (a.d_user || a.d_pos || a.d_neg) {
      for (int d = lane; d < D; d += 32) {
        float gu = 0.f, gp = 0.f, gn = 0.f;
        if (ok) pair_grads1<KIND>(g, a.c_l2, ur[d], pr[d], nr[d], &gu, &gp, &gn);
        if (row_form) {
          if (ok) {
            a.d_user[(int64_t)uu * ld + d] = gu;
            a.d_pos[(int64_t)pp * ld + d] = gp;
            a.d_neg[(int64_t)nn * ld + d] = gn;
          }
        } else {
          const int64_t o = (int64_t)t * D + d;
          if (a.d_user) a.d_user[o] = gu;
          if (a.d_pos) a.d_pos[o] = gp;
          if (a.d_neg) a.d_neg[o] = gn;
        }
      }
    }
    if (lane == 0) {
      const float gbias = (KIND == ORX_PAIR_BPR) ? g : -g;
      if (row_form) {
        if (ok) {
          for (int64_t c = D; c < ld; ++c) {
            a.d_user[(int64_t)uu * ld + c] = 0.f;
            a.d_pos[(int64_t)pp * ld + c] = c == D ? gbias : 0.f;
            a.d_neg[(int64_t)nn * ld + c] = c == D ? -gbias : 0.f;
          }
        }
      } else {
        if (a.d_bp) a.d_bp[t] = gbias;
        if (a.d_bn) a.d_bn[t] = -gbias;
      }
      if (a.g_out) a.g_out[t] = g;
    }
  }
  orx_warp_partial(loss_acc, l2_acc, a.partials);
}

__global__ void k_reduce_partials(const float* partials, int n, float loss_scale, float* out4) {
  double l, q;
  orx_block_sum_partials(partials, n, nullptr, 0, &l, &q);
  if (threadIdx.x == 0) {
    out4[0] = (float)(l * (double)loss_scale);
    out4[1] = (float)(0.5 * q);
    out4[2] = 0.f;
    out4[3] = 0.f;
  }
}

int orx_launch_reduce_partials(const float* partials, int n, float loss_scale, float* out4, cudaStream_t st) {
  k_reduce_partials<<<1, 256, 0, st>>>(partials, n, loss_scale, out4);
  ORX_LAUNCH_CHECK();
  return ORX_OK;
}

int orx_ensure_partials(orx_ctx* c, int need, cudaStream_t st) {
  if (need <= c->cap_partials) return ORX_OK;
  ORX_CUDA(cudaStreamSynchronize(st));
  cudaFree(c->partials);
  c->partials = nullptr;
  c->cap_partials = need * 2;
  ORX_CUDA(cudaMalloc(&c->partials, sizeof(float) * 2 * (size_t)c->cap_partials));
  return ORX_OK;
}

static int launch_pair_fwd_grad(orx_ctx* c, int kind, PairGradArgs a, float* out4, cudaStream_t st) {
  const int nw = (a.B + 7) / 8, blocks = (nw + 7) / 8;
  int rc = orx_ensure_partials(c, blocks * 8, st);
  if (rc) return rc;
  a.partials = c->partials;
  orx_dispatch<ORX_PAIR_BPR, ORX_PAIR_UCML>(kind, [&](auto K) {
    k_pair_fwd_grad<decltype(K)::value><<<blocks, 256, 0, st>>>(a);
  });
  ORX_LAUNCH_CHECK();
  if (!out4) return ORX_OK;
  return orx_launch_reduce_partials(c->partials, blocks * 8, kind == ORX_PAIR_BPR ? a.inv_B : 1.f, out4, st);
}

static int pair_fwd_grad(orx_ctx* c, int kind, const orx_table_t* user, const orx_table_t* item,
                         const orx_table_t* bias, const int32_t* uid, const int32_t* pid, const int32_t* nid, int B,
                         float margin, float c_loss, float c_l2, float* d_user, float* d_pos, float* d_neg,
                         float* d_bp, float* d_bn, float* g_out, float* out4, cudaStream_t st) {
  ORX_REQUIRE(kind == ORX_PAIR_BPR || kind == ORX_PAIR_UCML, "unknown pairwise kind");
  ORX_REQUIRE(B > 0 && uid && pid && nid, "empty batch or null ids");
  int rc = check_tables(user, item, bias, ORX_OPT_SGD);
  if (rc) return rc;
  PairGradArgs a = {};
  a.U = user->var; a.I = item->var; a.Bv = bias->var;
  a.rowsU = user->rows; a.rowsI = item->rows; a.D = user->dim;
  a.uid = uid; a.pid = pid; a.nid = nid; a.B = B;
  a.margin = margin; a.c_loss = c_loss; a.c_l2 = c_l2; a.inv_B = 1.0f / (float)B;
  a.d_user = d_user; a.d_pos = d_pos; a.d_neg = d_neg; a.d_bp = d_bp; a.d_bn = d_bn; a.g_out = g_out;
  return launch_pair_fwd_grad(c, kind, a, out4, st);
}

extern "C" int orx_pairwise_fwd(orx_handle_t h, int32_t kind, const orx_table_t* user, const orx_table_t* item,
                                const orx_table_t* item_bias, const int32_t* uid, const int32_t* pid,
                                const int32_t* nid, int32_t B, float margin, float* out4, orx_stream_t s) {
  ORX_REQUIRE(h != nullptr && out4 != nullptr, "null handle/out");
  ORX_CUDA(cudaSetDevice(h->device));
  return pair_fwd_grad(h, kind, user, item, item_bias, uid, pid, nid, B, margin, 1.f, 1.f, nullptr, nullptr, nullptr,
                       nullptr, nullptr, nullptr, out4, (cudaStream_t)s);
}

extern "C" int orx_pairwise_grad(orx_handle_t h, int32_t kind, const orx_table_t* user, const orx_table_t* item,
                                 const orx_table_t* item_bias, const int32_t* uid, const int32_t* pid,
                                 const int32_t* nid, int32_t B, float margin, float c_loss, float c_l2, float* d_user,
                                 float* d_pos, float* d_neg, float* d_bp, float* d_bn, float* g_out, orx_stream_t s) {
  ORX_REQUIRE(h != nullptr, "null handle");
  ORX_CUDA(cudaSetDevice(h->device));
  return pair_fwd_grad(h, kind, user, item, item_bias, uid, pid, nid, B, margin, c_loss, c_l2, d_user, d_pos, d_neg,
                       d_bp, d_bn, g_out, nullptr, (cudaStream_t)s);
}

extern "C" int orx_pairwise_grad_rows(orx_handle_t h, int32_t kind, const float* rows, int64_t ld, int32_t dim,
                                      const int32_t* uslot, const int32_t* pslot, const int32_t* nslot, int32_t B,
                                      float margin, float c_loss, float c_l2, float inv_B, float* d_rows, float* out4,
                                      orx_stream_t s) {
  ORX_REQUIRE(h != nullptr && rows && uslot && pslot && nslot && d_rows && out4, "null pointer");
  ORX_REQUIRE(kind == ORX_PAIR_BPR || kind == ORX_PAIR_UCML, "unknown pairwise kind");
  ORX_REQUIRE(B > 0 && dim > 0 && ld > dim, "bad sizes (ld must exceed dim: the bias lives in column dim)");
  ORX_CUDA(cudaSetDevice(h->device));
  PairGradArgs a = {};
  a.U = rows; a.I = rows;
  a.rowsU = 3 * (int64_t)B; a.rowsI = 3 * (int64_t)B; a.D = dim;
  a.uid = uslot; a.pid = pslot; a.nid = nslot; a.B = B;
  a.margin = margin; a.c_loss = c_loss; a.c_l2 = c_l2; a.inv_B = inv_B;
  a.d_user = d_rows; a.d_pos = d_rows; a.d_neg = d_rows;
  a.ld = ld;
  return launch_pair_fwd_grad(h, kind, a, out4, (cudaStream_t)s);
}
```

openrec_b200/csrc/orx_pointwise.cu:

```cuda
#include "orx_common.cuh"

struct PointArgs {
  float *U, *Us0, *Us1;
  float *I, *Is0, *Is1;
  float *Bv, *Bs0, *Bs1;
  const float* W;
  float* gw;
  int64_t rowsU, rowsI;
  int D;
  const int32_t *uid, *iid;
  const float* label;
  int B;
  float wa, wb, c_loss, c_l2, inv_B;
  int use_sigmoid;
  OrxOptDev opt;
  OrxHash hu, hi;
  float *gu, *gi, *gb;
  float* partials;
  float *d_user, *d_item, *d_bias, *g_out;
};

template <int KIND>
__device__ __forceinline__ void point_score(float s, float bias, float label, const PointArgs& a, float* lt,
                                            float* g) {
// ... 210 lines not shown
        if (a.d_bias) a.d_bias[t] = g;
        if (a.g_out) a.g_out[t] = g;
      }
    }
  }
  orx_warp_partial(loss_acc, l2_acc, a.partials);
}

__global__ void k_gmf_w_terms(const float* W, int D, float* out4, float* d_w, float c_l2) {
  __shared__ float sh[256];
  float q = 0.f;
  for (int e = threadIdx.x; e < D; e += blockDim.x) {
    q += W[e] * W[e];
    if (d_w) d_w[e] += c_l2 * W[e];
  }
  sh[threadIdx.x] = q;
  __syncthreads();
  for (int s = 128; s > 0; s >>= 1) {
    if (threadIdx.x < s) sh[threadIdx.x] += sh[threadIdx.x + s];
    __syncthreads();
  }
  if (threadIdx.x == 0 && out4) out4[1] += 0.5f * sh[0];
}

template <int KIND, int OPT>
static int launch_point_kind_opt(const PointArgs& pa, cudaStream_t st, int* n_partials, int* variant) {
  const int nw = (pa.B + 7) / 8, blocks = (nw + 7) / 8;
  *n_partials = blocks * 8;
  *variant = ORX_VARIANT_STEP;
  switch (pa.D) {
    case 32: k_point_step<KIND, OPT, 32, 8><<<blocks, 256, 0, st>>>(pa); break;
    case 64: k_point_step<KIND, OPT, 64, 8><<<blocks, 256, 0, st>>>(pa); break;
    case 128: k_point_step<KIND, OPT, 128, 8><<<blocks, 256, 0, st>>>(pa); break;
    case 256: k_point_step<KIND, OPT, 256, 8><<<blocks, 256, 0, st>>>(pa); break;
    default:
      *variant = ORX_VARIANT_STEP_GENERIC;
      k_point_generic<KIND, OPT, 0><<<blocks, 256, 0, st>>>(pa);
      break;
  }
  ORX_LAUNCH_CHECK();
  return ORX_OK;
}

static int check_point(int kind, const orx_table_t* user, const orx_table_t* item, const orx_table_t* bias,
                       const orx_table_t* w, int opt_kind) {
  ORX_REQUIRE(kind == ORX_POINT_GMF || kind == ORX_POINT_WRMF, "unknown pointwise kind");
  ORX_REQUIRE(user && item && bias && user->var && item->var && bias->var, "null table");
  ORX_REQUIRE(user->dim == item->dim && user->dim > 0, "user/item dims must match and be positive");
  ORX_REQUIRE(bias->dim == 1 && bias->rows == item->rows, "item_bias must be [item.rows, 1]");
  ORX_REQUIRE(user->rows > 0 && item->rows > 0 && user->rows <= 0x7fffffffLL && item->rows <= 0x7fffffffLL,
              "row counts must fit int32 ids");
  if (kind == ORX_POINT_GMF) ORX_REQUIRE(w && w->var && w->dim == user->dim, "GMF needs w with dim == D");
  ORX_REQUIRE(orx_opt_slots_ok(opt_kind, {user, item, bias, kind == ORX_POINT_GMF ? w : nullptr}),
              "optimizer slot rows missing");
  return ORX_OK;
}

static void fill_point_args(PointArgs& pa, orx_ctx* c, int kind, const orx_table_t* user, const orx_table_t* item,
                            const orx_table_t* bias, const orx_table_t* w, const int32_t* uid, const int32_t* iid,
                            const float* label, int B, float a, float b, int use_sigmoid, float c_loss, float c_l2) {
  pa.U = user->var; pa.Us0 = user->s0; pa.Us1 = user->s1;
  pa.I = item->var; pa.Is0 = item->s0; pa.Is1 = item->s1;
  pa.Bv = bias->var; pa.Bs0 = bias->s0; pa.Bs1 = bias->s1;
  pa.W = (kind == ORX_POINT_GMF) ? w->var : nullptr;
  pa.gw = nullptr;
  pa.rowsU = user->rows; pa.rowsI = item->rows; pa.D = user->dim;
  pa.uid = uid; pa.iid = iid; pa.label = label; pa.B = B;
  pa.wa = a; pa.wb = b; pa.c_loss = c_loss; pa.c_l2 = c_l2; pa.inv_B = 1.0f / (float)B;
  pa.use_sigmoid = use_sigmoid;
  pa.hu = c->hu; pa.hi = c->hi; pa.gu = c->gu; pa.gi = c->gi; pa.gb = c->gb;
  pa.partials = c->partials;
  pa.d_user = pa.d_item = pa.d_bias = pa.g_out = nullptr;
  pa.opt.kind = 0; pa.opt.lr = 0.f; pa.opt.eps = 0.f; pa.opt.beta1 = 0.f; pa.opt.beta2 = 0.f;
}

extern "C" int orx_pointwise_step(orx_handle_t h, int32_t kind, const orx_table_t* user, const orx_table_t* item,
                                  const orx_table_t* item_bias, const orx_table_t* w, const int32_t* uid,
                                  const int32_t* iid, const float* label, int32_t B, float a, float b,
                                  int32_t use_sigmoid, float c_loss, float c_l2, const orx_opt_t* opt, float* out4,
                                  orx_stream_t s) {
  ORX_REQUIRE(h != nullptr && opt != nullptr && out4 != nullptr, "null handle/opt/out");
  ORX_REQUIRE(orx_opt_kind_ok(opt->kind), "unknown optimizer kind");
  ORX_REQUIRE(B > 0 && uid && iid && label, "empty batch or null inputs");
  ORX_CUDA(cudaSetDevice(h->device));
  cudaStream_t st = (cudaStream_t)s;
  int rc = check_point(kind, user, item, item_bias, w, opt->kind);
  if (rc) return rc;
  const int D = user->dim;
  const bool dense = opt->kind == ORX_OPT_ADAM_DENSE;
  if ((rc = orx_ensure_workspace(h, B, D))) return rc;
  if ((rc = orx_ensure_partials(h, (B + 7) / 8 + 8, st))) return rc;
  if ((rc = orx_launch_index_build(h, uid, user->rows, iid, nullptr, item->rows, B, dense, st))) return rc;
  PointArgs pa;
  fill_point_args(pa, h, kind, user, item, item_bias, w, uid, iid, label, B, a, b, use_sigmoid, c_loss, c_l2);
  pa.opt = orx_opt_to_dev(opt);
  pa.gw = (kind == ORX_POINT_GMF) ? h->gw : nullptr;
  int n_partials = 0, variant = 0;
  rc = orx_dispatch<ORX_POINT_GMF, ORX_POINT_WRMF>(kind, [&](auto K) {
    return orx_dispatch_opt(opt->kind, [&](auto O) {
      return launch_point_kind_opt<decltype(K)::value, decltype(O)::value>(pa, st, &n_partials, &variant);
    });
  });
  if (rc) return rc;
  orx_log_dispatch(h, ORX_OP_POINTWISE_STEP, variant, kind, opt->kind, B, D, 0, 0);
  if (dense && (rc = orx_launch_adam_sweeps(h, user, item, item_bias, h->hu, h->hi, pa.opt, st))) return rc;
  TailArgs ta = orx_tail_args(h, user, item, item_bias, h->hu, h->hi, pa.opt);
  ta.partials = h->partials; ta.n_partials = n_partials;
  ta.loss_scale = (kind == ORX_POINT_GMF) ? pa.inv_B : 1.0f;
  ta.counters = h->counters; ta.out4 = out4;
  if (kind == ORX_POINT_GMF) {
    ta.W = w->var; ta.Ws0 = w->s0; ta.Ws1 = w->s1; ta.gw = h->gw; ta.c_l2 = c_l2;
  }
  return orx_launch_tail(h, ta, opt->kind, st);
}

static int point_fwd_grad(orx_ctx* h, int kind, const orx_table_t* user, const orx_table_t* item,
                          const orx_table_t* bias, const orx_table_t* w, const int32_t* uid, const int32_t* iid,
                          const float* label, int B, float a, float b, int use_sigmoid, float c_loss, float c_l2,
                          float* d_user, float* d_item, float* d_bias, float* d_w, float* g_out, float* out4,
                          cudaStream_t st) {
  ORX_REQUIRE(B > 0 && uid && iid && label, "empty batch or null inputs");
  int rc = check_point(kind, user, item, bias, w, ORX_OPT_SGD);
  if (rc) return rc;
  const int nw = (B + 7) / 8, blocks = (nw + 7) / 8;
  if ((rc = orx_ensure_partials(h, blocks * 8, st))) return rc;
  PointArgs pa;
  fill_point_args(pa, h, kind, user, item, bias, w, uid, iid, label, B, a, b, use_sigmoid, c_loss, c_l2);
  pa.d_user = d_user; pa.d_item = d_item; pa.d_bias = d_bias; pa.g_out = g_out;
  if (kind == ORX_POINT_GMF && d_w) {
    ORX_CUDA(cudaMemsetAsync(d_w, 0, sizeof(float) * user->dim, st));
    pa.gw = d_w;
  }
  if (kind == ORX_POINT_GMF) k_point_generic<ORX_POINT_GMF, ORX_OPT_SGD, 1><<<blocks, 256, 0, st>>>(pa);
  else k_point_generic<ORX_POINT_WRMF, ORX_OPT_SGD, 1><<<blocks, 256, 0, st>>>(pa);
  ORX_LAUNCH_CHECK();
  if (out4) {
    rc = orx_launch_reduce_partials(h->partials, blocks * 8, kind == ORX_POINT_GMF ? pa.inv_B : 1.f, out4, st);
    if (rc) return rc;
  }
  if (kind == ORX_POINT_GMF && (out4 || d_w)) {
    k_gmf_w_terms<<<1, 256, 0, st>>>(w->var, user->dim, out4, d_w, c_l2);
    ORX_LAUNCH_CHECK();
  }
  return ORX_OK;
}

extern "C" int orx_pointwise_fwd(orx_handle_t h, int32_t kind, const orx_table_t* user, const orx_table_t* item,
                                 const orx_table_t* item_bias, const orx_table_t* w, const int32_t* uid,
                                 const int32_t* iid, const float* label, int32_t B, float a, float b,
                                 int32_t use_sigmoid, float* out4, orx_stream_t s) {
  ORX_REQUIRE(h != nullptr && out4 != nullptr, "null handle/out");
  ORX_CUDA(cudaSetDevice(h->device));
  return point_fwd_grad(h, kind, user, item, item_bias, w, uid, iid, label, B, a, b, use_sigmoid, 1.f, 1.f, nullptr,
                        nullptr, nullptr, nullptr, nullptr, out4, (cudaStream_t)s);
}

extern "C" int orx_pointwise_grad(orx_handle_t h, int32_t kind, const orx_table_t* user, const orx_table_t* item,
                                  const orx_table_t* item_bias, const orx_table_t* w, const int32_t* uid,
                                  const int32_t* iid, const float* label, int32_t B, float a, float b,
                                  int32_t use_sigmoid, float c_loss, float c_l2, float* d_user, float* d_item,
                                  float* d_bias, float* d_w, float* g_out, orx_stream_t s) {
  ORX_REQUIRE(h != nullptr, "null handle");
  ORX_CUDA(cudaSetDevice(h->device));
  return point_fwd_grad(h, kind, user, item, item_bias, w, uid, iid, label, B, a, b, use_sigmoid, c_loss, c_l2, d_user,
                        d_item, d_bias, d_w, g_out, nullptr, (cudaStream_t)s);
}
```

openrec_b200/csrc/orx_sampler.cu:

```cuda
#include "orx_common.cuh"

__device__ __forceinline__ uint64_t smix64(uint64_t x) {
  x += 0x9E3779B97F4A7C15ull;
  x = (x ^ (x >> 30)) * 0xBF58476D1CE4E5B9ull;
  x = (x ^ (x >> 27)) * 0x94D049BB133111EBull;
  return x ^ (x >> 31);
}
__device__ __forceinline__ uint64_t srand3(uint64_t seed, uint64_t a, uint64_t b) { return smix64(seed ^ smix64((a << 24) ^ b)); }

struct SamplerData {
  const int32_t *rec_user, *rec_item;
  const int64_t *perm_cur, *perm_next;
  int64_t cursor, n_records;
  const int64_t* csr_off;
  const int32_t* csr_items;
  int32_t total_users, total_items;
};

__device__ __forceinline__ int64_t sampler_record(const SamplerData& d, int64_t k) {
  const int64_t left = d.n_records - d.cursor;
  return k < left ? d.perm_cur[d.cursor + k] : d.perm_next[(k - left) % d.n_records];
}
__device__ __forceinline__ bool sampler_is_positive(const SamplerData& d, int32_t u, int32_t i) {
  int64_t lo = d.csr_off[u];
// ... 44 lines not shown
    for (int w = 0; w < 32; ++w) {
      const int s = warp_sum[w];
      if (w < wid) before += s;
      total += s;
    }
    if (live) {
      int32_t u, i;
      if (pos) {
        const int64_t r = sampler_record(d, base + before);
        u = d.rec_user[r];
        i = d.rec_item[r];
      } else {
        for (uint32_t attempt = 1;; ++attempt) {
          const uint64_t x = srand3(seed, (uint64_t)(pos0 + b), attempt);
          u = (int32_t)((x >> 32) % (uint64_t)d.total_users);
          i = (int32_t)((x & 0xffffffffull) % (uint64_t)d.total_items);
          if (!sampler_is_positive(d, u, i) || attempt > 1000000u) break;
        }
      }
      uid[b] = u;
      iid[b] = i;
      label[b] = pos ? 1.f : 0.f;
    }
    __syncthreads();
    if (threadIdx.x == 0) base += total;
    __syncthreads();
  }
  if (threadIdx.x == 0) *n_pos_out = (int32_t)base;
}

#define ORX_MAX_QUOTA 64
__global__ void k_sample_per_positive(SamplerData d, uint64_t seed, int64_t pos0, int32_t B, int32_t quota,
                                      int32_t* __restrict__ uid, int32_t* __restrict__ iid, float* __restrict__ label) {
  const int b = blockIdx.x * blockDim.x + threadIdx.x;
  if (b >= B) return;
  const int64_t s = pos0 + b, g = quota + 1;
  const int64_t grp = s / g, grp0 = pos0 / g;
  const int m = (int)(s - grp * g);
  const int64_t r = sampler_record(d, grp - grp0);
  const int32_t u = d.rec_user[r], p = d.rec_item[r];
  int32_t item = p;
  if (m > 0) {
    int32_t cand[ORX_MAX_QUOTA + 1];
    int n = 0, kept = 0;
    uint32_t attempt = 0;
    while (n < quota + 1) {
      const int32_t c = (int32_t)(srand3(seed, (uint64_t)grp, attempt++) % (uint64_t)d.total_items);
      bool dup = false;
      for (int k = 0; k < n; ++k) dup = dup || cand[k] == c;
      if (dup && attempt < 100000u) continue;
      cand[n++] = c;
    }
    for (int k = 0; k < quota + 1; ++k) {
      if (cand[k] == p) continue;
      if (++kept == m) { item = cand[k]; break; }
    }
  }
  uid[b] = u;
  iid[b] = item;
  label[b] = m == 0 ? 1.f : 0.f;
}

static int sampler_check(orx_handle_t h, const orx_sampler_t* sd) {
  ORX_REQUIRE(h != nullptr && sd != nullptr, "null handle / sampler data");
  ORX_REQUIRE(sd->rec_user && sd->rec_item && sd->perm_cur && sd->perm_next && sd->csr_off && sd->csr_items, "null pointer");
  ORX_REQUIRE(sd->n_records > 0 && sd->cursor >= 0 && sd->cursor <= sd->n_records && sd->total_users > 0 && sd->total_items > 0,
              "bad sizes");
  return ORX_OK;
}
static SamplerData sampler_dev(const orx_sampler_t* s) {
  SamplerData d;
  d.rec_user = s->rec_user; d.rec_item = s->rec_item; d.perm_cur = s->perm_cur; d.perm_next = s->perm_next;
  d.cursor = s->cursor; d.n_records = s->n_records; d.csr_off = s->csr_off; d.csr_items = s->csr_items;
  d.total_users = s->total_users; d.total_items = s->total_items;
  return d;
}

extern "C" int orx_sample_pairwise(orx_handle_t h, const orx_sampler_t* sd, uint64_t seed, int64_t stream_pos, int32_t B,
                                   int32_t* uid, int32_t* pid, int32_t* nid, orx_stream_t s) {
  int rc = sampler_check(h, sd);
  if (rc) return rc;
  ORX_REQUIRE(uid && pid && nid && B >= 0 && (int64_t)B <= sd->n_records, "bad batch (at most one epoch per batch)");
  if (B == 0) return ORX_OK;
  ORX_CUDA(cudaSetDevice(h->device));
  k_sample_pairwise<<<(B + 255) / 256, 256, 0, (cudaStream_t)s>>>(sampler_dev(sd), seed, stream_pos, B, uid, pid, nid);
  ORX_LAUNCH_CHECK();
  return ORX_OK;
}

extern "C" int orx_sample_stratified(orx_handle_t h, const orx_sampler_t* sd, uint64_t seed, int64_t stream_pos, int32_t B,
                                     float pos_ratio, int32_t* uid, int32_t* iid, float* label, int32_t* n_pos_out,
                                     orx_stream_t s) {
  int rc = sampler_check(h, sd);
  if (rc) return rc;
  ORX_REQUIRE(uid && iid && label && n_pos_out && B >= 0 && (int64_t)B <= sd->n_records, "bad batch (at most one epoch per batch)");
  ORX_REQUIRE(pos_ratio >= 0.f && pos_ratio <= 1.f, "pos_ratio must be in [0, 1]");
  if (B == 0) return ORX_OK;
  ORX_CUDA(cudaSetDevice(h->device));
  k_sample_stratified<<<1, 1024, 0, (cudaStream_t)s>>>(sampler_dev(sd), seed, stream_pos, B, pos_ratio, uid, iid, label, n_pos_out);
  ORX_LAUNCH_CHECK();
  return ORX_OK;
}

extern "C" int orx_sample_per_positive(orx_handle_t h, const orx_sampler_t* sd, uint64_t seed, int64_t stream_pos, int32_t B,
                                       int32_t quota, int32_t* uid, int32_t* iid, float* label, orx_stream_t s) {
  int rc = sampler_check(h, sd);
  if (rc) return rc;
  ORX_REQUIRE(uid && iid && label && B >= 0 && quota >= 0 && quota <= ORX_MAX_QUOTA && quota < sd->total_items, "bad batch / quota");
  ORX_REQUIRE((int64_t)B / (quota + 1) + 2 <= sd->n_records, "at most one epoch of records per batch");
  if (B == 0) return ORX_OK;
  ORX_CUDA(cudaSetDevice(h->device));
  k_sample_per_positive<<<(B + 127) / 128, 128, 0, (cudaStream_t)s>>>(sampler_dev(sd), seed, stream_pos, B, quota, uid, iid, label);
  ORX_LAUNCH_CHECK();
  return ORX_OK;
}
```

openrec_b200/csrc/orx_shard.cu:

```cuda
#include <stdlib.h>
#include <string.h>

#include "orx_common.cuh"
#include "orx_pair.cuh"

#define SH_MAX_R 64
#define SH_META 16
#define SH_NPH 4
#define SH_ERR_WORD (SH_NPH * SH_MAX_R)
#define SH_IDX_BITS 24

enum { SH_M_TRIPS = 0,
       SH_M_REQS = 1,
       SH_M_GOTOFF = 2,
       SH_M_GINBASE = 3,
       SH_M_LOSS = 4, SH_M_L2 = 5 };

enum { SH_C_CURH = 0, SH_C_CURO = SH_MAX_R, SH_C_GOFF = 2 * SH_MAX_R, SH_C_RCO = 3 * SH_MAX_R + 1,
       SH_C_DONE = 4 * SH_MAX_R + 1, SH_C_T = SH_C_DONE + 8, SH_C_NREQ = SH_C_T + 1, SH_C_ACUR = SH_C_T + 2,
       SH_C_BAD = SH_C_T + 4 , SH_C_WORDS = SH_C_T + 8 };

struct ShardHost {
  int32_t world, rank, dim, batch_cap, home_cap, req_cap, gin_cap, timeout_ms;
  void *tripbox, *idbox, *got, *gotb, *gin, *ginb, *meta, *flags;
// ... 699 lines not shown

static int shard_check(orx_handle_t h, const ShardHost* x) {
  ORX_REQUIRE(h != nullptr && x != nullptr, "null handle / descriptor");
  ORX_REQUIRE(x->world >= 1 && x->world <= SH_MAX_R && x->rank >= 0 && x->rank < x->world, "bad world / rank");
  ORX_REQUIRE(x->dim >= 4 && (x->dim & 3) == 0 && x->dim <= 512, "dim must be a multiple of 4 in [4, 512]");
  ORX_REQUIRE(x->batch_cap > 0 && x->home_cap > 0 && x->req_cap > 0 && x->gin_cap >= 32 && x->timeout_ms > 0, "bad capacities");
  ORX_REQUIRE(x->req_cap < (1 << SH_IDX_BITS), "req_cap must stay below 2^24");
  ORX_REQUIRE(x->tripbox && x->idbox && x->got && x->gotb && x->gin && x->ginb && x->meta && x->flags, "null mailbox pointer table");
  return ORX_OK;
}

static ShardDev shard_to_dev(const ShardHost* x) {
  ShardDev d;
  d.world = x->world; d.rank = x->rank; d.D = x->dim; d.batch_cap = x->batch_cap; d.home_cap = x->home_cap;
  d.req_cap = x->req_cap; d.gin_cap = x->gin_cap; d.got_rows = sh_got_rows(x->home_cap, x->world);
  d.timeout_ns = (unsigned long long)x->timeout_ms * 1000000ull;
  d.tripbox = (int32_t* const*)x->tripbox; d.idbox = (int32_t* const*)x->idbox;
  d.got = (float* const*)x->got; d.gotb = (float* const*)x->gotb;
  d.gin = (float* const*)x->gin; d.ginb = (float* const*)x->ginb;
  d.meta = (int32_t* const*)x->meta; d.flags = (int32_t* const*)x->flags;
  return d;
}

extern "C" int orx_shard_sizes(const orx_shard_t* xs, int64_t* n8_host) {
  const ShardHost* x = (const ShardHost*)xs;
  ORX_REQUIRE(x != nullptr && n8_host != nullptr, "null pointer");
  ORX_REQUIRE(x->world >= 1 && x->world <= SH_MAX_R && x->dim > 0 && x->batch_cap > 0 && x->home_cap > 0 && x->req_cap > 0 &&
              x->gin_cap > 0, "bad descriptor");
  const int64_t got_rows = sh_got_rows(x->home_cap, x->world);
  n8_host[0] = (int64_t)x->world * 3 * x->batch_cap;
  n8_host[1] = (int64_t)x->world * x->req_cap;
  n8_host[2] = got_rows * x->dim;
  n8_host[3] = got_rows;
  n8_host[4] = (int64_t)x->gin_cap * x->dim;
  n8_host[5] = x->gin_cap;
  n8_host[6] = (int64_t)x->world * SH_META;
  n8_host[7] = SH_ERR_WORD + 1;
  return ORX_OK;
}

template <typename F>
static inline auto sh_dispatch_opt(int opt_kind, F&& f) {
  return orx_dispatch<ORX_OPT_SGD, ORX_OPT_ADAGRAD, ORX_OPT_ADAM_LAZY>(opt_kind, f);
}
template <typename F>
static inline auto sh_dispatch_nq(int nq, F&& f) {
  return orx_dispatch<1, 2, 4>(nq <= 32 ? 1 : (nq <= 64 ? 2 : 4), f);
}

static int shard_take_epochs(orx_ctx* c, cudaStream_t st, bool may_drain, uint32_t* eu, uint32_t* ei) {
  if (c->epoch >= 0x7ffffff0u) {
    if (!may_drain) return 1;
    c->epoch = 0x7fffffffu;
  }
  int rc;
  if ((rc = orx_next_epoch(c, st))) return rc;
  *eu = c->epoch;
  if ((rc = orx_next_epoch(c, st))) return rc;
  *ei = c->epoch;
  return ORX_OK;
}

extern "C" int orx_shard_step(orx_handle_t h, int32_t kind, const orx_shard_t* xs, const orx_table_t* user,
                              const orx_table_t* item, const orx_table_t* item_bias, const int32_t* uid, const int32_t* pid,
                              const int32_t* nid, int32_t B, const int32_t* next_uid, const int32_t* next_pid,
                              const int32_t* next_nid, int32_t next_B, int64_t total_users, int64_t total_items, float margin,
                              float c_loss, float c_l2, float inv_B, const orx_opt_t* opt, int32_t epoch, int32_t phase_lo,
                              int32_t phase_hi, float* out4, orx_stream_t s) {
  const ShardHost* x = (const ShardHost*)xs;
  int rc = shard_check(h, x);
  if (rc) return rc;
  ORX_REQUIRE(kind == ORX_PAIR_BPR || kind == ORX_PAIR_UCML, "unknown pairwise kind");
  ORX_REQUIRE(user && item && item_bias && user->var && item->var && item_bias->var && opt && out4, "null pointer");
  ORX_REQUIRE(user->dim == x->dim && item->dim == x->dim && item_bias->dim == 1 && item_bias->rows == item->rows, "table shapes");
  ORX_REQUIRE(B > 0 && B <= x->batch_cap && uid && pid && nid, "bad batch (larger than the mailboxes were built for?)");
  const bool announce = next_uid != nullptr;
  ORX_REQUIRE(announce == (next_pid != nullptr) && announce == (next_nid != nullptr), "next_uid / next_pid / next_nid: all or none");
  if (announce) ORX_REQUIRE(next_B > 0 && next_B <= x->batch_cap, "bad announced batch");
  ORX_REQUIRE(total_users > 0 && total_items > 0 && epoch > 0 && epoch < 0x7ffffffe, "bad totals / epoch");
  ORX_REQUIRE(phase_lo >= 0 && phase_hi <= 5 && phase_lo <= phase_hi, "bad phase range");
  ORX_REQUIRE(opt->kind == ORX_OPT_SGD || opt->kind == ORX_OPT_ADAGRAD || opt->kind == ORX_OPT_ADAM_LAZY,
              "the sharded step supports SGD, Adagrad and row-sparse Adam");
  ORX_REQUIRE(orx_opt_slots_ok(opt->kind, {user, item, item_bias}), "optimizer slot rows missing");
  ORX_CUDA(cudaSetDevice(h->device));
  cudaStream_t st = (cudaStream_t)s;
  const int64_t need = x->home_cap > (x->gin_cap + 1) / 2 ? x->home_cap : (x->gin_cap + 1) / 2;
  if ((rc = orx_ensure_workspace(h, need, x->dim))) return rc;
  if ((rc = shard_ws_ensure(h, x, st))) return rc;
  orx_shard_ws* S = (orx_shard_ws*)h->shard_ws;
  if (S->owner != x->flags) {
    ORX_REQUIRE(S->serve_epoch == S->tail_epoch && S->pro_route[0] <= S->tail_epoch && S->pro_route[1] <= S->tail_epoch,
                "another sharded model on this handle has a step in flight or an announced batch outstanding");
    memset(S->pro_route, 0, sizeof(S->pro_route));
    memset(S->pro_request, 0, sizeof(S->pro_request));
    S->serve_epoch = S->tail_epoch = 0;
    S->owner = x->flags;
  }
  ORX_REQUIRE(!h->pf_valid, "this handle has an index prefetched by orx_pairwise_prefetch outstanding (the sharded step uses the same index sets)");
  const ShardWs& w = S->w;
  const ShardDev xd = shard_to_dev(x);
  const int par = epoch & 1;
  const OrxOptDev od = orx_opt_to_dev(opt);
  const int nq = x->dim >> 2;
  if ((rc = orx_ensure_partials(h, h->num_sms * 4 * 8, st))) return rc;
  const int route_blocks = (B + 1023) / 1024;
  int request_blocks = (x->home_cap + 511) / 512;
  if (request_blocks > h->num_sms) request_blocks = h->num_sms;

  if (phase_lo == 0 && S->pro_route[par] != epoch) {
    if ((rc = shard_take_epochs(h, st, S->serve_epoch == S->tail_epoch, &S->ep_u[par], &S->ep_i[par])) != ORX_OK) {
      if (rc == 1) { orx_set_error("orx_shard_step: index epochs are about to wrap; issue this step's route after the previous step's tail"); return ORX_ERR_INVALID; }
      return rc;
    }
    S->ids_u[par] = uid; S->ids_p[par] = pid; S->ids_n[par] = nid; S->ids_B[par] = B;
  }
  if (S->pro_route[par] == epoch || phase_lo == 0)
    ORX_REQUIRE(S->ids_u[par] == uid && S->ids_p[par] == pid && S->ids_n[par] == nid && S->ids_B[par] == B,
                "this step's batch differs from the one its route was issued for (announced as next_* in the previous call)");
  OrxHash hu = h->pf_u[par];
  hu.epoch = S->ep_u[par];
  OrxHash hi = h->hi;
  hi.epoch = S->ep_i[par];

  ShCompArgs ca;
  ca.U = user->var; ca.Us0 = user->s0; ca.Us1 = user->s1; ca.hu = hu; ca.gu = h->gu;
  ca.margin = margin; ca.c_loss = c_loss; ca.c_l2 = c_l2; ca.inv_B = inv_B; ca.opt = od; ca.partials = h->partials;
  ca.loss_scale = kind == ORX_PAIR_BPR ? inv_B : 1.f;
  ShApplyArgs aa;
  aa.I = item->var; aa.Is0 = item->s0; aa.Is1 = item->s1;
  aa.Bv = item_bias->var; aa.Bs0 = item_bias->s0; aa.Bs1 = item_bias->s1;
  aa.hi = hi; aa.gi = h->gi; aa.gb = h->gb; aa.opt = od;
  const bool whole = phase_lo == 0 && phase_hi == 5;
  for (int ph = phase_lo; ph <= phase_hi; ++ph) {
    if (whole) orx_prof_mark(h, ph, st);
    switch (ph) {
      case 0: {
        if (S->pro_route[par] == epoch) break;
        ShRouteArgs ra;
        ra.uid = uid; ra.pid = pid; ra.nid = nid; ra.B = B; ra.U = total_users; ra.I = total_items;
        ORX_CUDA(orx_launch_pdl(k_sh_route, dim3(route_blocks), dim3(256), 0, st, xd, w, ra, epoch));
        S->pro_route[par] = epoch;
        break;
      }
      case 1:
        if (S->pro_request[par] == epoch) break;
        ORX_REQUIRE(S->pro_route[par] == epoch, "phase 1 before phase 0");
        ORX_CUDA(orx_launch_pdl(k_sh_request, dim3(request_blocks), dim3(256), 0, st, xd, w, hu, epoch));
        S->pro_request[par] = epoch;
        break;
      case 2:
        ORX_REQUIRE(S->pro_request[par] == epoch, "phase 2 before this step's phases 0 and 1");
        sh_dispatch_nq(nq, [&](auto Q) {
          auto kern = k_sh_serve<decltype(Q)::value>;
          orx_launch_pdl(kern, dim3(h->num_sms * sh_ctas_per_sm((const void*)kern, 4)), dim3(256), 0, st, xd, w,
                         (const float*)item->var, (const float*)item_bias->var, (int64_t)item->rows, hi, epoch);
        });
        S->serve_epoch = epoch;
        break;
      case 3:
        orx_dispatch<ORX_PAIR_BPR, ORX_PAIR_UCML>(kind, [&](auto K) {
          sh_dispatch_opt(opt->kind, [&](auto O) {
            sh_dispatch_nq(nq, [&](auto Q) {
              auto kern = k_sh_compute<decltype(K)::value, decltype(O)::value, decltype(Q)::value>;
              orx_launch_pdl(kern, dim3(h->num_sms * sh_ctas_per_sm((const void*)kern, 4)), dim3(256), 0, st, xd, w,
                             ca, epoch);
            });
          });
// ... 48 lines not shown
```

openrec_b200/csrc/orx_sharded.cu:

```cuda
#include "orx_common.cuh"

__global__ void k_owner_hist(const int32_t* __restrict__ ids, int n, int R, int32_t* counts) {
  extern __shared__ int32_t sh[];
  for (int r = threadIdx.x; r < R; r += blockDim.x) sh[r] = 0;
  __syncthreads();
  for (int i = blockIdx.x * blockDim.x + threadIdx.x; i < n; i += gridDim.x * blockDim.x) {
    const int32_t id = ids[i];
    atomicAdd(&sh[id >= 0 ? id % R : 0], 1);
  }
  __syncthreads();
  for (int r = threadIdx.x; r < R; r += blockDim.x)
    if (sh[r]) atomicAdd(counts + r, sh[r]);
}

__global__ void k_owner_scan(const int32_t* counts, int R, int32_t* cursor) {
  if (threadIdx.x == 0) {
    int acc = 0;
    for (int r = 0; r < R; ++r) {
      cursor[r] = acc;
      acc += counts[r];
    }
  }
}

__global__ void __launch_bounds__(256) k_owner_scatter(const int32_t* __restrict__ ids, int n, int n_user, int64_t U,
                                                       int R, int32_t* cursor, int32_t* __restrict__ send_local,
                                                       int32_t* __restrict__ slot) {
  extern __shared__ int32_t sh[];
  int32_t* cnt = sh;
  int32_t* base = sh + R;
  for (int r = threadIdx.x; r < R; r += blockDim.x) cnt[r] = 0;
  __syncthreads();
  const int i = blockIdx.x * blockDim.x + threadIdx.x;
  int32_t id = -1;
  int r = 0, rank_in_block = 0;
  if (i < n) {
    id = ids[i];
    r = id >= 0 ? id % R : 0;
    rank_in_block = atomicAdd(&cnt[r], 1);
  }
  __syncthreads();
  for (int q = threadIdx.x; q < R; q += blockDim.x) base[q] = cnt[q] ? atomicAdd(cursor + q, cnt[q]) : 0;
  __syncthreads();
  if (i < n) {
    const int s = base[r] + rank_in_block;
    const int32_t user_rows_on_r = (i >= n_user) ? (int32_t)((U - r + R - 1) / R) : 0;
    send_local[s] = id >= 0 ? id / R + user_rows_on_r : -1;
    slot[i] = s;
  }
}

extern "C" int orx_owner_bucket_combined(orx_handle_t h, const int32_t* ids, int32_t n, int32_t n_user,
                                         int64_t total_users, int32_t world, int32_t* counts, int32_t* send_local,
                                         int32_t* slot, orx_stream_t s) {
  ORX_REQUIRE(h != nullptr && ids && counts && send_local && slot, "null pointer");
  ORX_REQUIRE(n >= 0 && n_user >= 0 && n_user <= n && world >= 1 && world <= 1024 && total_users > 0, "bad sizes");
  ORX_CUDA(cudaSetDevice(h->device));
  cudaStream_t st = (cudaStream_t)s;
  ORX_CUDA(cudaMemsetAsync(counts, 0, sizeof(int32_t) * world, st));
  if (n == 0) return ORX_OK;
  if (!h->bucket_cursor) ORX_CUDA(cudaMalloc(&h->bucket_cursor, sizeof(int32_t) * 1024));
  int blocks = (n + 255) / 256;
  if (blocks > h->num_sms * 4) blocks = h->num_sms * 4;
  k_owner_hist<<<blocks, 256, sizeof(int32_t) * world, st>>>(ids, n, world, counts);
  ORX_LAUNCH_CHECK();
  k_owner_scan<<<1, 32, 0, st>>>(counts, world, h->bucket_cursor);
  ORX_LAUNCH_CHECK();
  k_owner_scatter<<<(n + 255) / 256, 256, 2 * sizeof(int32_t) * world, st>>>(ids, n, n_user, total_users, world,
                                                                             h->bucket_cursor, send_local, slot);
  ORX_LAUNCH_CHECK();
  return ORX_OK;
}

template <int OPT>
__global__ void __launch_bounds__(256) k_sparse_apply(float* var, float* s0, float* s1, int64_t rows, int D,
                                                      const int32_t* __restrict__ ids, int64_t id_stride,
                                                      const float* __restrict__ vals, int64_t val_ld, int n,
                                                      OrxHash hsh, float* gstage, OrxOptDev o) {
  typedef OrxOptSlots<OPT> SL;
  const int lane = threadIdx.x & 31;
  const int nw = (gridDim.x * blockDim.x) >> 5;
  for (int b0 = ((blockIdx.x * blockDim.x + threadIdx.x) >> 5) * 8; b0 < n; b0 += nw * 8) {
  int32_t my_id = -1;
  int my_d = -1;
  uint32_t my_c = 0;
  if (lane < 8 && b0 + lane < n) {
    my_id = ids[(int64_t)(b0 + lane) * id_stride];
    if (my_id < 0 || (int64_t)my_id >= rows) my_id = -1;
    else my_c = orx_hash_find(hsh, my_id, &my_d);
  }
#pragma unroll 2
  for (int k = 0; k < 8; ++k) {
  const int b = b0 + k;
  if (b >= n) break;
  const int32_t id = __shfl_sync(ORX_FULL, my_id, k);
  const uint32_t c = __shfl_sync(ORX_FULL, my_c, k);
  const int d = __shfl_sync(ORX_FULL, my_d, k);
  if (id < 0) continue;
  const float* v = vals + (int64_t)b * val_ld;
  const bool own = !SL::STAGE_ONLY && c == 1u;
  if (((D & 3) == 0) && ((val_ld & 3) == 0)) {
    const float4 z4 = make_float4(0.f, 0.f, 0.f, 0.f);
    for (int e = lane * 4; e < D; e += 128) {
      const int64_t off = (int64_t)id * D + e;
      const float4 g = __ldcg(reinterpret_cast<const float4*>(v + e));
      const float4 wv = own ? __ldcg(reinterpret_cast<const float4*>(var + off)) : z4;
      float4 a = (SL::S0 && own) ? __ldcg(reinterpret_cast<const float4*>(s0 + off)) : z4;
      float4 bb = (SL::S1 && own) ? __ldcg(reinterpret_cast<const float4*>(s1 + off)) : z4;
      orx_own_or_stage4<OPT, false>(own, var, s0, s1, id, gstage, d, D, e, wv, g, a, bb, o);
    }
  } else {
    for (int e = lane; e < D; e += 32) {
      const int64_t off = (int64_t)id * D + e;
      if (own) orx_update1<OPT>(var + off, s0 + off, s1 + off, var[off], v[e], o);
      else atomicAdd(gstage + (int64_t)d * D + e, v[e]);
    }
  }
  }
  }
}

static int sparse_apply_impl(orx_handle_t h, const orx_table_t* tab, const int32_t* ids, int64_t id_stride,
                             const float* values, int64_t value_ld, int32_t n, const orx_opt_t* opt, orx_stream_t s);

extern "C" int orx_sparse_apply(orx_handle_t h, const orx_table_t* tab, const int32_t* ids, const float* values,
                                int32_t n, const orx_opt_t* opt, orx_stream_t s) {
  ORX_REQUIRE(tab != nullptr, "null table");
  return sparse_apply_impl(h, tab, ids, 1, values, tab->dim, n, opt, s);
}

extern "C" int orx_sparse_apply_strided(orx_handle_t h, const orx_table_t* tab, const int32_t* ids, int64_t id_stride,
                                        const float* values, int64_t value_ld, int32_t n, const orx_opt_t* opt,
                                        orx_stream_t s) {
  ORX_REQUIRE(tab != nullptr && id_stride >= 1 && value_ld >= tab->dim, "bad strides");
  return sparse_apply_impl(h, tab, ids, id_stride, values, value_ld, n, opt, s);
}

static int sparse_apply_impl(orx_handle_t h, const orx_table_t* tab, const int32_t* ids, int64_t id_stride,
                             const float* values, int64_t value_ld, int32_t n, const orx_opt_t* opt, orx_stream_t s) {
  ORX_REQUIRE(h != nullptr && tab && tab->var && opt, "null pointer");
  ORX_REQUIRE(n >= 0 && tab->rows > 0 && tab->dim > 0, "bad sizes");
  ORX_REQUIRE(orx_opt_kind_ok(opt->kind), "unknown optimizer kind");
  ORX_REQUIRE(orx_opt_slots_ok(opt->kind, {tab}), "optimizer slot rows missing");
  ORX_CUDA(cudaSetDevice(h->device));
  cudaStream_t st = (cudaStream_t)s;
  const bool dense = opt->kind == ORX_OPT_ADAM_DENSE;
  if (n == 0 && !dense) return ORX_OK;
  ORX_REQUIRE(n == 0 || (ids && values), "null ids/values");
  const int D = tab->dim;
  int rc = orx_ensure_workspace(h, n > 0 ? n : 1, D);
  if (rc) return rc;
  const OrxOptDev o = orx_opt_to_dev(opt);
  if (n > 0) {
    if ((rc = orx_launch_index_build_strided(h, ids, id_stride, tab->rows, n, dense, st))) return rc;
    const int blocks = (n + 63) / 64;
    orx_dispatch_opt(opt->kind, [&](auto O) {
      k_sparse_apply<decltype(O)::value><<<blocks, 256, 0, st>>>(tab->var, tab->s0, tab->s1, tab->rows, D, ids, id_stride,
                                                                 values, value_ld, n, h->hu, h->gu, o);
    });
    ORX_LAUNCH_CHECK();
  }
  if (dense && (rc = orx_launch_adam_sweeps(h, tab, nullptr, nullptr, h->hu, h->hi, o, st))) return rc;
  TailArgs ta = orx_tail_args(h, tab, nullptr, nullptr, h->hu, h->hi, o);
  ta.counters = h->counters;
  return orx_launch_tail(h, ta, opt->kind, st);
}
```

openrec_b200/native.py:

```python
from __future__ import annotations

import ctypes as C
from collections import namedtuple

import torch

from . import _lib
from ._lib import (ORX_OP_GEMM, ORX_OP_INTERACT_BWD, ORX_OP_INTERACT_FWD, ORX_OP_PAIRWISE_STEP, ORX_OP_POINTWISE_STEP,
                   ORX_OPT_ADAGRAD, ORX_OPT_ADAM_DENSE, ORX_OPT_ADAM_LAZY, ORX_OPT_SGD, ORX_PAIR_BPR, ORX_PAIR_UCML,
                   ORX_POINT_GMF, ORX_POINT_WRMF, ORX_SCORE_DOT, ORX_SCORE_NEG_SQDIST, ORX_VARIANT_GEMM_SIMT,
                   ORX_VARIANT_GEMM_TMA, ORX_VARIANT_INTERACT, ORX_VARIANT_INTERACT_WARP, ORX_VARIANT_STEP,
                   ORX_VARIANT_STEP_GENERIC, ORX_VARIANT_STEP_PIPE, OrxOpt, OrxTable)

__all__ = ["Engine", "engine", "table", "opt", "ORX_PAIR_BPR", "ORX_PAIR_UCML", "ORX_POINT_GMF", "ORX_POINT_WRMF",
           "ORX_OPT_SGD", "ORX_OPT_ADAGRAD", "ORX_OPT_ADAM_LAZY", "ORX_OPT_ADAM_DENSE", "ORX_SCORE_DOT",
           "ORX_SCORE_NEG_SQDIST", "ORX_OP_GEMM", "ORX_OP_INTERACT_FWD", "ORX_OP_INTERACT_BWD", "ORX_OP_PAIRWISE_STEP",
           "ORX_OP_POINTWISE_STEP", "ORX_VARIANT_GEMM_TMA", "ORX_VARIANT_GEMM_SIMT", "ORX_VARIANT_INTERACT_WARP",
           "ORX_VARIANT_INTERACT", "ORX_VARIANT_STEP", "ORX_VARIANT_STEP_PIPE", "ORX_VARIANT_STEP_GENERIC", "Dispatch"]

_engines = {}

Dispatch = namedtuple("Dispatch", "op variant ta tb m n k s")


# ... 22 lines not shown
    rows, dim = (var.shape[0], var.shape[1]) if var.dim() == 2 else (1, var.numel())
    return OrxTable(var.data_ptr(), s0.data_ptr() if s0 is not None else None,
                    s1.data_ptr() if s1 is not None else None, rows, dim)


def opt(kind, lr, eps=1e-7, beta1=0.9, beta2=0.999, step=1):
    return OrxOpt(kind, lr, eps, beta1, beta2, step)


class Engine:

    def __init__(self, index: int):
        self.index = index
        self.lib = _lib.lib()
        h = C.c_void_p()
        _lib.check(self.lib.orx_create(index, C.byref(h)), "orx_create")
        self.h = h
        self.device = torch.device("cuda", index)

    def close(self):
        if self.h:
            self.lib.orx_destroy(self.h)
            self.h = None

    def stream(self):
        return C.c_void_p(torch.cuda.current_stream(self.device).cuda_stream)

    make_table = staticmethod(table)
    make_opt = staticmethod(opt)

    def profile_enable(self, on=True):
        _lib.check(self.lib.orx_profile_enable(self.h, 1 if on else 0))

    def profile_read(self, n_phases=3):
        ms = (C.c_float * n_phases)()
        n = C.c_int32()
        _lib.check(self.lib.orx_profile_read(self.h, ms, n_phases, C.byref(n)))
        return list(ms), n.value

    def fill_uniform(self, dst, lo, hi, seed):
        _lib.check(self.lib.orx_fill_uniform(self.h, _ptr(_f32(dst, "dst")), dst.numel(), lo, hi, seed, self.stream()))

    def gather(self, tab, ids, n_bad=None):
        is64 = ids.dtype == torch.int64
        if not is64:
            ids = ids32(ids)
        ids = ids.contiguous().reshape(-1)
        out = torch.empty((ids.numel(), tab.shape[1]), dtype=torch.float32, device=tab.device)
        _lib.check(self.lib.orx_gather(self.h, _ptr(_f32(tab, "tab")), tab.shape[0], tab.shape[1], _ptr(ids),
                                       1 if is64 else 0, ids.numel(), _ptr(out), _ptr(n_bad), self.stream()))
        return out

    def censor(self, tab, ids, min_norm=0.1):
        ids = ids32(ids)
        _lib.check(self.lib.orx_censor(self.h, _ptr(_f32(tab, "tab")), tab.shape[0], tab.shape[1], _ptr(ids),
                                       ids.numel(), min_norm, self.stream()))

    def pairwise_step(self, kind, user, item, bias, uid, pid, nid, o, out4, margin=0.5, c_loss=1.0, c_l2=1.0):
        _lib.check(self.lib.orx_pairwise_step(self.h, kind, C.byref(user), C.byref(item), C.byref(bias), _ptr(uid),
                                              _ptr(pid), _ptr(nid), uid.numel(), margin, c_loss, c_l2, C.byref(o),
                                              _ptr(out4), self.stream()), "orx_pairwise_step")

    def pairwise_step_host(self, kind, user, item, bias, uid_h, pid_h, nid_h, o, out4_h, margin=0.5, c_loss=1.0,
                           c_l2=1.0):
        _lib.check(self.lib.orx_pairwise_step_host(self.h, kind, C.byref(user), C.byref(item), C.byref(bias),
                                                   _ptr(uid_h), _ptr(pid_h), _ptr(nid_h), uid_h.numel(), margin,
                                                   c_loss, c_l2, C.byref(o), _ptr(out4_h), self.stream()),
                   "orx_pairwise_step_host")

    def pairwise_prefetch(self, user, item, uid, pid, nid, opt_kind, ids_ready=False):
        _lib.check(self.lib.orx_pairwise_prefetch(self.h, C.byref(user), C.byref(item), _ptr(uid), _ptr(pid), _ptr(nid),
                                                  uid.numel(), opt_kind, 1 if ids_ready else 0, self.stream()),
                   "orx_pairwise_prefetch")

    def debug_set_epoch(self, epoch):
        _lib.check(self.lib.orx_debug_set_epoch(self.h, epoch), "orx_debug_set_epoch")

    def debug_dispatch_log(self):
        rec = (C.c_int32 * (8 * _lib.ORX_DISPATCH_LOG_CAP))()
        n = C.c_int32()
        _lib.check(self.lib.orx_debug_dispatch_log(self.h, rec, _lib.ORX_DISPATCH_LOG_CAP, C.byref(n)),
                   "orx_debug_dispatch_log")
        return [Dispatch(*rec[8 * i:8 * i + 8]) for i in range(n.value)]

    def pairwise_fwd(self, kind, user, item, bias, uid, pid, nid, out4, margin=0.5):
        _lib.check(self.lib.orx_pairwise_fwd(self.h, kind, C.byref(user), C.byref(item), C.byref(bias), _ptr(uid),
                                             _ptr(pid), _ptr(nid), uid.numel(), margin, _ptr(out4), self.stream()),
                   "orx_pairwise_fwd")

    def pairwise_grad(self, kind, user, item, bias, uid, pid, nid, margin=0.5, c_loss=1.0, c_l2=1.0, *, d_user=None,
                      d_pos=None, d_neg=None, d_bp=None, d_bn=None, g_out=None):
        _lib.check(self.lib.orx_pairwise_grad(self.h, kind, C.byref(user), C.byref(item), C.byref(bias), _ptr(uid),
                                              _ptr(pid), _ptr(nid), uid.numel(), margin, c_loss, c_l2, _ptr(d_user),
                                              _ptr(d_pos), _ptr(d_neg), _ptr(d_bp), _ptr(d_bn), _ptr(g_out),
                                              self.stream()), "orx_pairwise_grad")

    def sparse_apply(self, tab, ids, values, o):
        n = 0 if ids is None else ids.numel()
        _lib.check(self.lib.orx_sparse_apply(self.h, C.byref(tab), _ptr(ids), _ptr(values), n, C.byref(o),
                                             self.stream()), "orx_sparse_apply")

    def sparse_apply_strided(self, tab, ids2d, col, values3d, o):
        n, F = ids2d.shape
        D = values3d.shape[2]
        _lib.check(self.lib.orx_sparse_apply_strided(
            self.h, C.byref(tab), C.c_void_p(ids2d.data_ptr() + 4 * col), F,
            C.c_void_p(values3d.data_ptr() + 4 * col * D), values3d.shape[1] * D, n, C.byref(o), self.stream()),
            "orx_sparse_apply_strided")

    @staticmethod
    def _ld(t):
        if t.dim() != 2 or t.stride(1) != 1:
            raise ValueError("expected a 2-D float32 view with unit inner stride")
        return t.stride(0)

    def gather_strided(self, tab, ids2d, col, out2d):
        n, F = ids2d.shape
        _lib.check(self.lib.orx_gather_strided(self.h, _ptr(tab), tab.shape[0], tab.shape[1],
                                               C.c_void_p(ids2d.data_ptr() + 4 * col), F, n, _ptr(out2d),
                                               self._ld(out2d), None, self.stream()), "orx_gather_strided")

    def mlp_fwd(self, x, w, bias, act, y):
        _lib.check(self.lib.orx_mlp_layer_fwd(self.h, _ptr(x), self._ld(x), x.shape[0], w.shape[0], _ptr(w), _ptr(bias),
                                              w.shape[1], act, _ptr(y), self._ld(y), self.stream()),
                   "orx_mlp_layer_fwd")

    def mlp_bwd(self, x, y, w, act, dy, dx, dw, db):
        _lib.check(self.lib.orx_mlp_layer_bwd(self.h, _ptr(x), self._ld(x), _ptr(y), self._ld(y), _ptr(w), x.shape[0],
                                              w.shape[0], w.shape[1], act, _ptr(dy), self._ld(dy), _ptr(dx),
                                              self._ld(dx) if dx is not None else 0, _ptr(dw), _ptr(db),
                                              self.stream()), "orx_mlp_layer_bwd")

    def interact_fwd(self, emb3d, dense2d, self_interaction, mode, out2d):
        B, Fm1, D = emb3d.shape
        _lib.check(self.lib.orx_interact_fwd(self.h, _ptr(emb3d), Fm1 * D, _ptr(dense2d), self._ld(dense2d), B,
                                             Fm1 + 1, D, int(self_interaction), mode, _ptr(out2d), self._ld(out2d),
                                             self.stream()), "orx_interact_fwd")

    def interact_bwd(self, emb3d, dense2d, dout2d, self_interaction, mode, demb3d, ddense2d):
        B, Fm1, D = emb3d.shape
        _lib.check(self.lib.orx_interact_bwd(self.h, _ptr(emb3d), Fm1 * D, _ptr(dense2d), self._ld(dense2d),
                                             _ptr(dout2d), self._ld(dout2d), B, Fm1 + 1, D, int(self_interaction),
                                             mode, _ptr(demb3d), Fm1 * D, _ptr(ddense2d), self._ld(ddense2d),
                                             self.stream()), "orx_interact_bwd")

    def pred_loss(self, pred, label, kind, clip, pred_out, dpred, out4):
        _lib.check(self.lib.orx_pred_loss(self.h, _ptr(pred), _ptr(label), pred.numel(), kind, clip, _ptr(pred_out),
                                          _ptr(dpred), _ptr(out4), self.stream()), "orx_pred_loss")

    def owner_bucket_combined(self, ids, n_user, total_users, world):
        n = ids.numel()
        counts = torch.empty(world, dtype=torch.int32, device=ids.device)
        send_local = torch.empty(n, dtype=torch.int32, device=ids.device)
        slot = torch.empty(n, dtype=torch.int32, device=ids.device)
        _lib.check(self.lib.orx_owner_bucket_combined(self.h, _ptr(ids), n, n_user, total_users, world, _ptr(counts),
                                                      _ptr(send_local), _ptr(slot), self.stream()),
                   "orx_owner_bucket_combined")
        return counts, send_local, slot

    def pairwise_grad_rows(self, kind, rows, dim, uslot, pslot, nslot, inv_B, d_rows, out4, margin=0.5, c_loss=1.0,
                           c_l2=1.0):
        _lib.check(self.lib.orx_pairwise_grad_rows(self.h, kind, _ptr(rows), rows.shape[1], dim, _ptr(uslot),
                                                   _ptr(pslot), _ptr(nslot), uslot.numel(), margin, c_loss, c_l2,
                                                   inv_B, _ptr(d_rows), _ptr(out4), self.stream()),
                   "orx_pairwise_grad_rows")

# ... 58 lines not shown
```

Baseline: 358.1 million.

## Chain in-stream prefetch index build behind sparse tail with PDL

When the next batch's ids are already ready on the same stream that just ran the step's tail, the prefetch index-build kernel is now launched in that stream with programmatic dependent launch instead of on the side stream. This avoids side-stream event waits and records. Event release for the prefetch buffer is made lazy, and the tail kernel triggers early so dependents can start. The tail grid can also be sized to one occupancy wave. Every API entry now resets a chain-armed flag, and a debug query reports which prefetch mode ran. This adds fairly complex state tracking across calls and a risk of ordering bugs.

```diff
diff --git a/include/orx.h b/include/orx.h
--- a/include/orx.h
+++ b/include/orx.h
@@ -66,6 +66,12 @@
 };
 #define ORX_DISPATCH_LOG_CAP 64
 ORX_API int orx_debug_dispatch_log(orx_handle_t h, int32_t* rec_host, int32_t cap, int32_t* n_host);
+enum orx_prefetch_mode {
+  ORX_PREFETCH_NONE = 0,
+  ORX_PREFETCH_SIDE_STREAM = 1,
+  ORX_PREFETCH_IN_STREAM = 2
+};
+ORX_API int orx_debug_last_prefetch_mode(orx_handle_t h, int32_t* mode_host);
 
 ORX_API int orx_profile_enable(orx_handle_t h, int32_t on);
 ORX_API int orx_profile_read(orx_handle_t h, float* ms_host, int32_t n_phases, int32_t* n_steps_host);
diff --git a/openrec_b200/_lib.py b/openrec_b200/_lib.py
--- a/openrec_b200/_lib.py
+++ b/openrec_b200/_lib.py
@@ -14,6 +14,7 @@
 ORX_VARIANT_GEMM_TMA, ORX_VARIANT_GEMM_SIMT, ORX_VARIANT_INTERACT_WARP, ORX_VARIANT_INTERACT = 0, 1, 2, 3
 ORX_VARIANT_STEP, ORX_VARIANT_STEP_PIPE, ORX_VARIANT_STEP_GENERIC = 4, 5, 6
 ORX_DISPATCH_LOG_CAP = 64
+ORX_PREFETCH_NONE, ORX_PREFETCH_SIDE_STREAM, ORX_PREFETCH_IN_STREAM = 0, 1, 2
 
 
 class OrxOpt(C.Structure):
@@ -53,6 +54,7 @@
     "orx_stream_synchronize": [_vp, _vp],
     "orx_debug_set_epoch": [_vp, C.c_uint32],
     "orx_debug_dispatch_log": [_vp, C.POINTER(_i32), _i32, C.POINTER(_i32)],
+    "orx_debug_last_prefetch_mode": [_vp, C.POINTER(_i32)],
     "orx_profile_enable": [_vp, _i32],
     "orx_profile_read": [_vp, C.POINTER(C.c_float), _i32, C.POINTER(_i32)],
     "orx_fill_uniform": [_vp, _vp, _i64, _f, _f, _u64, _vp],
diff --git a/openrec_b200/csrc/orx_common.cuh b/openrec_b200/csrc/orx_common.cuh
--- a/openrec_b200/csrc/orx_common.cuh
+++ b/openrec_b200/csrc/orx_common.cuh
@@ -28,6 +28,12 @@
   } while (0)
 
 #define ORX_LAUNCH_CHECK() ORX_CUDA(cudaGetLastError())
+
+#define ORX_ENTER(h)                      \
+  do {                                    \
+    ORX_CUDA(cudaSetDevice((h)->device)); \
+    (h)->chain_armed = 0;                 \
+  } while (0)
 
 struct OrxHash {
   unsigned long long* slots;
@@ -63,9 +69,16 @@
   cudaEvent_t side_ev;
   cudaEvent_t pf_done[2], pf_free[2], stage_free[2];
   int pf_free_valid[2], stage_free_valid[2];
+  cudaStream_t pf_rel_st[2];
+  int pf_rel_lazy[2];
   int pf_valid, pf_set, pf_next, pf_B, pf_mode;
   const int32_t *pf_uid, *pf_pid, *pf_nid;
   int64_t pf_rows_u, pf_rows_i;
+  int pf_in_stream;
+  cudaStream_t pf_stream;
+  int pf_last_mode;
+  int chain_armed;
+  cudaStream_t chain_st;
   uint32_t epoch;
   void* shard_ws;
   int32_t dispatch[ORX_DISPATCH_LOG_CAP][8];
@@ -475,7 +488,7 @@
                        const OrxHash& hu, const OrxHash& hi, const OrxOptDev& o);
 int orx_launch_adam_sweeps(orx_ctx* c, const orx_table_t* user, const orx_table_t* item, const orx_table_t* bias,
                            const OrxHash& hu, const OrxHash& hi, const OrxOptDev& o, cudaStream_t st);
-int orx_launch_tail(orx_ctx* c, const TailArgs& ta, int opt_kind, cudaStream_t st);
+int orx_launch_tail(orx_ctx* c, const TailArgs& ta, int opt_kind, cudaStream_t st, bool one_wave = false);
 int orx_ensure_partials(orx_ctx* c, int need, cudaStream_t st);
 int orx_launch_reduce_partials(const float* partials, int n, float loss_scale, float* out4, cudaStream_t st);
 int orx_launch_index_build(orx_ctx* c, const int32_t* a, int64_t rows_a, const int32_t* b0, const int32_t* b1,
diff --git a/openrec_b200/csrc/orx_ctx.cu b/openrec_b200/csrc/orx_ctx.cu
--- a/openrec_b200/csrc/orx_ctx.cu
+++ b/openrec_b200/csrc/orx_ctx.cu
@@ -92,6 +92,7 @@
   }
   c->pf_valid = 0;
   c->pf_free_valid[0] = c->pf_free_valid[1] = 0;
+  c->pf_rel_lazy[0] = c->pf_rel_lazy[1] = 0;
   c->g_rows_u = nb;
   c->g_rows_i = 2 * nb;
   size_t bu = sizeof(float) * (size_t)c->g_rows_u * nd, bi = sizeof(float) * (size_t)c->g_rows_i * nd;
@@ -149,6 +150,12 @@
   return ORX_OK;
 }
 
+extern "C" int orx_debug_last_prefetch_mode(orx_handle_t h, int32_t* mode) {
+  ORX_REQUIRE(h != nullptr && mode != nullptr, "bad arguments");
+  *mode = h->pf_last_mode;
+  return ORX_OK;
+}
+
 int orx_ensure_stage(orx_ctx* c, int64_t n_ints) {
   if (n_ints <= c->stage_cap) return ORX_OK;
   ORX_CUDA(cudaDeviceSynchronize());
diff --git a/openrec_b200/csrc/orx_dlrm.cu b/openrec_b200/csrc/orx_dlrm.cu
--- a/openrec_b200/csrc/orx_dlrm.cu
+++ b/openrec_b200/csrc/orx_dlrm.cu
@@ -26,7 +26,7 @@
   ORX_REQUIRE(h != nullptr && tab && ids && out, "null pointer");
   ORX_REQUIRE(rows > 0 && dim > 0 && n >= 0 && id_stride >= 1 && out_ld >= dim, "bad sizes");
   if (n == 0) return ORX_OK;
-  ORX_CUDA(cudaSetDevice(h->device));
+  ORX_ENTER(h);
   int64_t blocks = (n + 7) / 8;
   if (blocks > (int64_t)h->num_sms * 32) blocks = (int64_t)h->num_sms * 32;
   k_gather_strided<<<(int)blocks, 256, 0, (cudaStream_t)s>>>(tab, rows, dim, ids, id_stride, n, out, out_ld, n_bad);
@@ -267,7 +267,7 @@
   ORX_REQUIRE(h != nullptr && dense && out && (F == 1 || emb), "null pointer");
   ORX_REQUIRE(B >= 0 && F >= 1 && F <= ORX_MAX_F && D > 0 && (mode == 0 || mode == 1), "bad sizes/mode");
   if (B == 0) return ORX_OK;
-  ORX_CUDA(cudaSetDevice(h->device));
+  ORX_ENTER(h);
   if (inter_fast_ok(F, D, mode, emb ? (const void*)emb : (const void*)dense, dense, emb_ld, dense_ld)) {
     const size_t sm = sizeof(float4) * (size_t)INTER_WARPS * F * 32;
     static bool attr = false;
@@ -295,7 +295,7 @@
   ORX_REQUIRE(h != nullptr && dense && dout && ddense && (F == 1 || (emb && demb)), "null pointer");
   ORX_REQUIRE(B >= 0 && F >= 1 && F <= ORX_MAX_F && D > 0 && (mode == 0 || mode == 1), "bad sizes/mode");
   if (B == 0) return ORX_OK;
-  ORX_CUDA(cudaSetDevice(h->device));
+  ORX_ENTER(h);
   if (inter_fast_ok(F, D, mode, emb ? (const void*)emb : (const void*)dense, dense, emb_ld, dense_ld) && (demb_ld & 3) == 0 &&
       (ddense_ld & 3) == 0 && ((((uintptr_t)(demb ? (const void*)demb : (const void*)ddense)) | ((uintptr_t)ddense)) & 15) == 0) {
     const size_t sm = (size_t)INTER_WARPS * (sizeof(float4) * (size_t)F * 32 + sizeof(float) * (size_t)F * 36);
@@ -419,7 +419,7 @@
   ORX_REQUIRE(h != nullptr && x && w && y, "null pointer");
   ORX_REQUIRE(B >= 0 && in > 0 && out > 0 && ldx >= in && ldy >= out && act >= 0 && act <= 2, "bad sizes");
   if (B == 0) return ORX_OK;
-  ORX_CUDA(cudaSetDevice(h->device));
+  ORX_ENTER(h);
   return launch_gemm<0, 0>(h, x, ldx, w, out, y, ldy, B, out, in, bias, act, (cudaStream_t)s);
 }
 
@@ -458,7 +458,7 @@
                                  int64_t lddy, float* dx, int64_t lddx, float* dw, float* db, orx_stream_t s) {
   ORX_REQUIRE(h != nullptr && x && y && w && dy && dw, "null pointer");
   ORX_REQUIRE(B > 0 && in > 0 && out > 0 && act >= 0 && act <= 2, "bad sizes");
-  ORX_CUDA(cudaSetDevice(h->device));
+  ORX_ENTER(h);
   cudaStream_t st = (cudaStream_t)s;
   if (act != 0) {
     const int64_t n = (int64_t)B * out;
@@ -533,7 +533,7 @@
                              float clip_threshold, float* pred_out, float* dpred, float* out4, orx_stream_t s) {
   ORX_REQUIRE(h != nullptr && pred && label && out4, "null pointer");
   ORX_REQUIRE(B > 0 && (kind == 0 || kind == 1), "bad sizes/kind");
-  ORX_CUDA(cudaSetDevice(h->device));
+  ORX_ENTER(h);
   cudaStream_t st = (cudaStream_t)s;
   int blocks = (B + 255) / 256;
   if (blocks > 256) blocks = 256;
diff --git a/openrec_b200/csrc/orx_misc.cu b/openrec_b200/csrc/orx_misc.cu
--- a/openrec_b200/csrc/orx_misc.cu
+++ b/openrec_b200/csrc/orx_misc.cu
@@ -21,7 +21,7 @@
                                 orx_stream_t s) {
   ORX_REQUIRE(h != nullptr && dst != nullptr && n >= 0, "null handle/dst or negative n");
   if (n == 0) return ORX_OK;
-  ORX_CUDA(cudaSetDevice(h->device));
+  ORX_ENTER(h);
   int64_t blocks = (n + 1023) / 1024;
   if (blocks > (int64_t)h->num_sms * 16) blocks = (int64_t)h->num_sms * 16;
   k_fill_uniform<<<(int)blocks, 256, 0, (cudaStream_t)s>>>(dst, n, lo, hi, seed);
@@ -56,7 +56,7 @@
   ORX_REQUIRE(rows > 0 && dim > 0 && n >= 0, "bad sizes");
   if (n == 0) return ORX_OK;
   ORX_REQUIRE(ids && out, "null pointer");
-  ORX_CUDA(cudaSetDevice(h->device));
+  ORX_ENTER(h);
   int64_t blocks = (n + 7) / 8;
   if (blocks > (int64_t)h->num_sms * 32) blocks = (int64_t)h->num_sms * 32;
   if (id_is_i64)
@@ -118,7 +118,7 @@
   ORX_REQUIRE(h != nullptr && tab && ids, "null pointer");
   ORX_REQUIRE(rows > 0 && dim > 0 && n >= 0, "bad sizes");
   if (n == 0) return ORX_OK;
-  ORX_CUDA(cudaSetDevice(h->device));
+  ORX_ENTER(h);
   cudaStream_t st = (cudaStream_t)s;
   int rc = orx_ensure_workspace(h, n, h->g_dim > 0 ? h->g_dim : 1);
   if (rc) return rc;
@@ -143,7 +143,7 @@
   ORX_REQUIRE(h != nullptr && var && grad && opt, "null pointer");
   ORX_REQUIRE(n >= 0, "negative n");
   if (n == 0) return ORX_OK;
-  ORX_CUDA(cudaSetDevice(h->device));
+  ORX_ENTER(h);
   const OrxOptDev o = orx_opt_to_dev(opt);
   int64_t blocks = (n + 255) / 256;
   if (blocks > (int64_t)h->num_sms * 16) blocks = (int64_t)h->num_sms * 16;
@@ -231,7 +231,7 @@
   ORX_REQUIRE(kind == ORX_SCORE_DOT || kind == ORX_SCORE_NEG_SQDIST, "unknown score kind");
   ORX_REQUIRE(U > 0 && I > 0 && dim > 0 && Bu >= 0, "bad sizes");
   if (Bu == 0) return ORX_OK;
-  ORX_CUDA(cudaSetDevice(h->device));
+  ORX_ENTER(h);
   dim3 grid((unsigned)((I + 63) / 64), (unsigned)((Bu + 63) / 64));
   if (kind == ORX_SCORE_DOT)
     k_score_all<ORX_SCORE_DOT><<<grid, 256, 0, (cudaStream_t)s>>>(user_tab, U, uid, Bu, scale, item_tab, item_bias, I, dim, scores);
@@ -332,7 +332,7 @@
   ORX_REQUIRE(R >= 0 && I > 0 && n_at >= 0 && n_at <= ORX_MAX_AT, "bad sizes (at most 8 cut-offs)");
   ORX_REQUIRE(n_at == 0 || at_host, "null cut-offs");
   if (R == 0) return ORX_OK;
-  ORX_CUDA(cudaSetDevice(h->device));
+  ORX_ENTER(h);
   RankArgs a;
   a.pred = pred; a.pos = pos; a.excl = excl; a.R = R; a.I = I; a.n_at = n_at;
   for (int k = 0; k < ORX_MAX_AT; ++k) a.at[k] = k < n_at ? at_host[k] : 0;
diff --git a/openrec_b200/csrc/orx_pairwise.cu b/openrec_b200/csrc/orx_pairwise.cu
--- a/openrec_b200/csrc/orx_pairwise.cu
+++ b/openrec_b200/csrc/orx_pairwise.cu
@@ -4,24 +4,28 @@
 #include "orx_common.cuh"
 #include "orx_pair.cuh"
 
+template <bool CHAIN>
 __global__ void k_index_build(OrxHash hu, OrxHash hi, const int32_t* __restrict__ a, int64_t rows_a,
                               const int32_t* __restrict__ b0, const int32_t* __restrict__ b1, int64_t rows_b, int n,
                               int stage_all, int32_t* bad) {
+  if (CHAIN) orx_pdl_trigger();
   const int i = blockIdx.x * blockDim.x + threadIdx.x;
-  if (i >= (b1 ? 3 : 2) * n) return;
-  const int t = i < n ? i : (i < 2 * n ? i - n : i - 2 * n);
-  const int32_t ia = a[t], ib0 = b0[t], ib1 = b1 ? b1[t] : 0;
-  const bool ga = ia >= 0 && (int64_t)ia < rows_a, gb0 = ib0 >= 0 && (int64_t)ib0 < rows_b,
-             gb1 = ib1 >= 0 && (int64_t)ib1 < rows_b;
-  const bool all = ga && gb0 && gb1;
-  if (i < n) {
-    if (!ga) atomicAdd(bad, 1);
-    else if (all) orx_hash_insert(hu, ia, stage_all);
-  } else {
-    const bool g = i < 2 * n ? gb0 : gb1;
-    if (!g) atomicAdd(bad, 1);
-    else if (all) orx_hash_insert(hi, i < 2 * n ? ib0 : ib1, stage_all);
-  }
+  if (i < (b1 ? 3 : 2) * n) {
+    const int t = i < n ? i : (i < 2 * n ? i - n : i - 2 * n);
+    const int32_t ia = a[t], ib0 = b0[t], ib1 = b1 ? b1[t] : 0;
+    const bool ga = ia >= 0 && (int64_t)ia < rows_a, gb0 = ib0 >= 0 && (int64_t)ib0 < rows_b,
+               gb1 = ib1 >= 0 && (int64_t)ib1 < rows_b;
+    const bool all = ga && gb0 && gb1;
+    if (i < n) {
+      if (!ga) atomicAdd(bad, 1);
+      else if (all) orx_hash_insert(hu, ia, stage_all);
+    } else {
+      const bool g = i < 2 * n ? gb0 : gb1;
+      if (!g) atomicAdd(bad, 1);
+      else if (all) orx_hash_insert(hi, i < 2 * n ? ib0 : ib1, stage_all);
+    }
+  }
+  if (CHAIN && blockIdx.x == 0) orx_pdl_wait();
 }
 
 __global__ void k_index_build_strided(OrxHash hu, const int32_t* __restrict__ a, int64_t stride, int64_t rows, int n,
@@ -49,7 +53,8 @@
   if (total <= 0) return ORX_OK;
   int rc = orx_next_epoch(c, st);
   if (rc) return rc;
-  k_index_build<<<(total + 255) / 256, 256, 0, st>>>(c->hu, c->hi, a, rows_a, b0, b1, rows_b, n, mode, c->counters + 3);
+  k_index_build<false><<<(total + 255) / 256, 256, 0, st>>>(c->hu, c->hi, a, rows_a, b0, b1, rows_b, n, mode,
+                                                            c->counters + 3);
   ORX_LAUNCH_CHECK();
   return ORX_OK;
 }
@@ -335,6 +340,7 @@
 template <int OPT>
 __global__ void __launch_bounds__(256) k_sparse_tail(const TailArgs a) {
   __shared__ bool last;
+  orx_pdl_trigger();
   orx_pdl_wait();
   const int nu = *a.hu.counter, ni = a.I ? *a.hi.counter : 0;
   orx_tail_rows<OPT>(a, nu, ni);
@@ -367,10 +373,19 @@
   if (last && threadIdx.x < 4) a.counters[threadIdx.x] = 0;
 }
 
-int orx_launch_tail(orx_ctx* c, const TailArgs& ta, int opt_kind, cudaStream_t st) {
-  const int grid = c->num_sms * 4;
+template <int OPT>
+static int tail_ctas_per_sm() {
+  static int nb = 0;
+  if (nb < 1 && (cudaOccupancyMaxActiveBlocksPerMultiprocessor(&nb, k_sparse_tail<OPT>, 256, 0) != cudaSuccess || nb < 1))
+    nb = 1;
+  return nb < 4 ? nb : 4;
+}
+
+int orx_launch_tail(orx_ctx* c, const TailArgs& ta, int opt_kind, cudaStream_t st, bool one_wave) {
   orx_dispatch_opt(opt_kind, [&](auto O) {
-    orx_launch_pdl(k_sparse_tail<decltype(O)::value>, dim3(grid), dim3(256), 0, st, ta);
+    constexpr int OPT = decltype(O)::value;
+    const int per_sm = one_wave ? tail_ctas_per_sm<OPT>() : 4;
+    orx_launch_pdl(k_sparse_tail<OPT>, dim3(c->num_sms * per_sm), dim3(256), 0, st, ta);
   });
   ORX_LAUNCH_CHECK();
   return ORX_OK;
@@ -455,32 +470,59 @@
   return ORX_OK;
 }
 
+static int prefetch_join(orx_ctx* c, cudaStream_t st) {
+  const int k = c->pf_set;
+  if (c->pf_in_stream) {
+    if (c->pf_stream == st) return ORX_OK;
+    ORX_CUDA(cudaEventRecord(c->pf_done[k], c->pf_stream));
+  }
+  ORX_CUDA(cudaStreamWaitEvent(st, c->pf_done[k], 0));
+  return ORX_OK;
+}
+
+static int prefetch_release(orx_ctx* c, int k, cudaStream_t st, bool record) {
+  c->pf_rel_st[k] = st;
+  c->pf_rel_lazy[k] = !record;
+  c->pf_free_valid[k] = record;
+  if (record) ORX_CUDA(cudaEventRecord(c->pf_free[k], st));
+  return ORX_OK;
+}
+
 static int prefetch_drop(orx_ctx* c, cudaStream_t st) {
   if (!c->pf_valid) return ORX_OK;
   const int k = c->pf_set;
-  ORX_CUDA(cudaStreamWaitEvent(st, c->pf_done[k], 0));
+  int rc = prefetch_join(c, st);
+  if (rc) return rc;
   ORX_CUDA(cudaMemsetAsync(c->counters + 4 * (1 + k), 0, sizeof(int32_t) * 4, st));
-  ORX_CUDA(cudaEventRecord(c->pf_free[k], st));
-  c->pf_free_valid[k] = 1;
   c->pf_valid = 0;
-  return ORX_OK;
+  return prefetch_release(c, k, st, !c->pf_in_stream);
 }
 
 static int prefetch_issue(orx_ctx* c, const int32_t* uid, const int32_t* pid, const int32_t* nid, int B, int64_t rows_u,
-                          int64_t rows_i, int mode) {
+                          int64_t rows_i, int mode, bool in_stream, cudaStream_t st) {
   const int k = c->pf_next;
   c->pf_next ^= 1;
-  cudaStream_t ss = c->side_stream;
-  if (c->pf_free_valid[k]) ORX_CUDA(cudaStreamWaitEvent(ss, c->pf_free[k], 0));
-  int rc = orx_next_epoch(c, ss);
-  if (rc) return rc;
+  cudaStream_t bs = in_stream ? st : c->side_stream;
+  int rc;
+  if (!in_stream) {
+    if (c->pf_rel_lazy[k] && (rc = prefetch_release(c, k, c->pf_rel_st[k], true))) return rc;
+    if (c->pf_free_valid[k]) ORX_CUDA(cudaStreamWaitEvent(bs, c->pf_free[k], 0));
+  }
+  if ((rc = orx_next_epoch(c, bs))) return rc;
   c->pf_u[k].epoch = c->pf_i[k].epoch = c->epoch;
-  k_index_build<<<(3 * B + 255) / 256, 256, 0, ss>>>(c->pf_u[k], c->pf_i[k], uid, rows_u, pid, nid, rows_i, B, mode,
-                                                     c->counters + 4 * (1 + k) + 3);
+  const dim3 grid((3 * B + 255) / 256);
+  int32_t* bad = c->counters + 4 * (1 + k) + 3;
+  if (in_stream)
+    orx_launch_pdl(k_index_build<true>, grid, dim3(256), 0, bs, c->pf_u[k], c->pf_i[k], uid, rows_u, pid, nid, rows_i, B,
+                   mode, bad);
+  else
+    k_index_build<false><<<grid, 256, 0, bs>>>(c->pf_u[k], c->pf_i[k], uid, rows_u, pid, nid, rows_i, B, mode, bad);
   ORX_LAUNCH_CHECK();
-  ORX_CUDA(cudaEventRecord(c->pf_done[k], ss));
+  if (!in_stream) ORX_CUDA(cudaEventRecord(c->pf_done[k], bs));
   c->pf_valid = 1; c->pf_set = k; c->pf_uid = uid; c->pf_pid = pid; c->pf_nid = nid; c->pf_B = B;
   c->pf_rows_u = rows_u; c->pf_rows_i = rows_i; c->pf_mode = mode;
+  c->pf_in_stream = in_stream; c->pf_stream = bs;
+  c->pf_last_mode = in_stream ? ORX_PREFETCH_IN_STREAM : ORX_PREFETCH_SIDE_STREAM;
   return ORX_OK;
 }
 
@@ -489,17 +531,21 @@
                                      orx_stream_t ids_stream) {
   ORX_REQUIRE(h != nullptr && user && item && uid && pid && nid && B > 0, "bad arguments");
   ORX_REQUIRE(orx_opt_kind_ok(opt_kind), "unknown optimizer kind");
-  ORX_CUDA(cudaSetDevice(h->device));
   cudaStream_t is = (cudaStream_t)ids_stream;
+  const bool behind_tail = ids_ready && h->chain_armed && h->chain_st == is;
+  ORX_ENTER(h);
   int rc = orx_ensure_workspace(h, B, user->dim);
   if (rc) return rc;
   if ((rc = side_stream_ensure(h))) return rc;
   if ((rc = prefetch_drop(h, is))) return rc;
+  const int k = h->pf_next;
+  const bool in_stream = behind_tail && ((!h->pf_free_valid[k] && !h->pf_rel_lazy[k]) || h->pf_rel_st[k] == is);
   if (!ids_ready) {
     ORX_CUDA(cudaEventRecord(h->side_ev, is));
     ORX_CUDA(cudaStreamWaitEvent(h->side_stream, h->side_ev, 0));
   }
-  return prefetch_issue(h, uid, pid, nid, B, user->rows, item->rows, opt_kind == ORX_OPT_ADAM_DENSE ? 1 : 0);
+  return prefetch_issue(h, uid, pid, nid, B, user->rows, item->rows, opt_kind == ORX_OPT_ADAM_DENSE ? 1 : 0, in_stream,
+                        is);
 }
 
 static int pairwise_step_impl(orx_ctx* c, int kind, const orx_table_t* user, const orx_table_t* item,
@@ -529,10 +575,12 @@
   pa.partials = c->partials;
   orx_prof_mark(c, 0, st);
   int set = 0;
+  bool in_stream = false;
   if (c->pf_valid && c->pf_uid == uid && c->pf_pid == pid && c->pf_nid == nid && c->pf_B == B &&
       c->pf_rows_u == user->rows && c->pf_rows_i == item->rows && c->pf_mode == (dense ? 1 : 0)) {
     set = 1 + c->pf_set;
-    ORX_CUDA(cudaStreamWaitEvent(st, c->pf_done[c->pf_set], 0));
+    in_stream = c->pf_in_stream;
+    if ((rc = prefetch_join(c, st))) return rc;
     c->pf_valid = 0;
   } else {
     if ((rc = prefetch_drop(c, st))) return rc;
@@ -557,10 +605,10 @@
   ta.partials = c->partials; ta.n_partials = n_partials;
   ta.loss_scale = (kind == ORX_PAIR_BPR) ? pa.inv_B : 1.0f;
   ta.counters = ctr; ta.out4 = out4;
-  rc = orx_launch_tail(c, ta, opt->kind, st);
+  rc = orx_launch_tail(c, ta, opt->kind, st, in_stream);
   if (set) {
-    ORX_CUDA(cudaEventRecord(c->pf_free[set - 1], st));
-    c->pf_free_valid[set - 1] = 1;
+    const int r = prefetch_release(c, set - 1, st, !in_stream);
+    if (!rc) rc = r;
   }
   orx_prof_mark(c, 3, st);
   orx_prof_next(c);
@@ -572,9 +620,14 @@
                                  const int32_t* nid, int32_t B, float margin, float c_loss, float c_l2,
                                  const orx_opt_t* opt, float* out4, orx_stream_t s) {
   ORX_REQUIRE(h != nullptr, "null handle");
-  ORX_CUDA(cudaSetDevice(h->device));
-  return pairwise_step_impl(h, kind, user, item, item_bias, uid, pid, nid, B, margin, c_loss, c_l2, opt, out4,
-                            (cudaStream_t)s);
+  ORX_ENTER(h);
+  const int rc = pairwise_step_impl(h, kind, user, item, item_bias, uid, pid, nid, B, margin, c_loss, c_l2, opt, out4,
+                                    (cudaStream_t)s);
+  if (rc == ORX_OK) {
+    h->chain_armed = 1;
+    h->chain_st = (cudaStream_t)s;
+  }
+  return rc;
 }
 
 extern "C" int orx_pairwise_step_host(orx_handle_t h, int32_t kind, const orx_table_t* user, const orx_table_t* item,
@@ -583,7 +636,7 @@
                                       const orx_opt_t* opt, float* out4_host, orx_stream_t s) {
   ORX_REQUIRE(h != nullptr, "null handle");
   ORX_REQUIRE(B > 0 && uid_host && pid_host && nid_host && out4_host && user && item && opt, "empty batch or null host buffers");
-  ORX_CUDA(cudaSetDevice(h->device));
+  ORX_ENTER(h);
   cudaStream_t st = (cudaStream_t)s;
   int rc = orx_ensure_stage(h, 3 * (int64_t)B);
   if (rc) return rc;
@@ -598,7 +651,7 @@
   ORX_CUDA(cudaMemcpyAsync(ids + B, pid_host, sizeof(int32_t) * B, cudaMemcpyHostToDevice, ss));
   ORX_CUDA(cudaMemcpyAsync(ids + 2 * (int64_t)B, nid_host, sizeof(int32_t) * B, cudaMemcpyHostToDevice, ss));
   if ((rc = prefetch_issue(h, ids, ids + B, ids + 2 * (int64_t)B, B, user->rows, item->rows,
-                           opt->kind == ORX_OPT_ADAM_DENSE ? 1 : 0)))
+                           opt->kind == ORX_OPT_ADAM_DENSE ? 1 : 0, false, st)))
     return rc;
   rc = pairwise_step_impl(h, kind, user, item, item_bias, ids, ids + B, ids + 2 * (int64_t)B, B, margin, c_loss, c_l2,
                           opt, h->out_stage[f], st);
@@ -757,7 +810,7 @@
                                 const orx_table_t* item_bias, const int32_t* uid, const int32_t* pid,
                                 const int32_t* nid, int32_t B, float margin, float* out4, orx_stream_t s) {
   ORX_REQUIRE(h != nullptr && out4 != nullptr, "null handle/out");
-  ORX_CUDA(cudaSetDevice(h->device));
+  ORX_ENTER(h);
   return pair_fwd_grad(h, kind, user, item, item_bias, uid, pid, nid, B, margin, 1.f, 1.f, nullptr, nullptr, nullptr,
                        nullptr, nullptr, nullptr, out4, (cudaStream_t)s);
 }
@@ -767,7 +820,7 @@
                                  const int32_t* nid, int32_t B, float margin, float c_loss, float c_l2, float* d_user,
                                  float* d_pos, float* d_neg, float* d_bp, float* d_bn, float* g_out, orx_stream_t s) {
   ORX_REQUIRE(h != nullptr, "null handle");
-  ORX_CUDA(cudaSetDevice(h->device));
+  ORX_ENTER(h);
   return pair_fwd_grad(h, kind, user, item, item_bias, uid, pid, nid, B, margin, c_loss, c_l2, d_user, d_pos, d_neg,
                        d_bp, d_bn, g_out, nullptr, (cudaStream_t)s);
 }
@@ -779,7 +832,7 @@
   ORX_REQUIRE(h != nullptr && rows && uslot && pslot && nslot && d_rows && out4, "null pointer");
   ORX_REQUIRE(kind == ORX_PAIR_BPR || kind == ORX_PAIR_UCML, "unknown pairwise kind");
   ORX_REQUIRE(B > 0 && dim > 0 && ld > dim, "bad sizes (ld must exceed dim: the bias lives in column dim)");
-  ORX_CUDA(cudaSetDevice(h->device));
+  ORX_ENTER(h);
   PairGradArgs a = {};
   a.U = rows; a.I = rows;
   a.rowsU = 3 * (int64_t)B; a.rowsI = 3 * (int64_t)B; a.D = dim;
diff --git a/openrec_b200/csrc/orx_pointwise.cu b/openrec_b200/csrc/orx_pointwise.cu
--- a/openrec_b200/csrc/orx_pointwise.cu
+++ b/openrec_b200/csrc/orx_pointwise.cu
@@ -316,7 +316,7 @@
   ORX_REQUIRE(h != nullptr && opt != nullptr && out4 != nullptr, "null handle/opt/out");
   ORX_REQUIRE(orx_opt_kind_ok(opt->kind), "unknown optimizer kind");
   ORX_REQUIRE(B > 0 && uid && iid && label, "empty batch or null inputs");
-  ORX_CUDA(cudaSetDevice(h->device));
+  ORX_ENTER(h);
   cudaStream_t st = (cudaStream_t)s;
   int rc = check_point(kind, user, item, item_bias, w, opt->kind);
   if (rc) return rc;
@@ -384,7 +384,7 @@
                                  const int32_t* iid, const float* label, int32_t B, float a, float b,
                                  int32_t use_sigmoid, float* out4, orx_stream_t s) {
   ORX_REQUIRE(h != nullptr && out4 != nullptr, "null handle/out");
-  ORX_CUDA(cudaSetDevice(h->device));
+  ORX_ENTER(h);
   return point_fwd_grad(h, kind, user, item, item_bias, w, uid, iid, label, B, a, b, use_sigmoid, 1.f, 1.f, nullptr,
                         nullptr, nullptr, nullptr, nullptr, out4, (cudaStream_t)s);
 }
@@ -395,7 +395,7 @@
                                   int32_t use_sigmoid, float c_loss, float c_l2, float* d_user, float* d_item,
                                   float* d_bias, float* d_w, float* g_out, orx_stream_t s) {
   ORX_REQUIRE(h != nullptr, "null handle");
-  ORX_CUDA(cudaSetDevice(h->device));
+  ORX_ENTER(h);
   return point_fwd_grad(h, kind, user, item, item_bias, w, uid, iid, label, B, a, b, use_sigmoid, c_loss, c_l2, d_user,
                         d_item, d_bias, d_w, g_out, nullptr, (cudaStream_t)s);
 }
diff --git a/openrec_b200/csrc/orx_sampler.cu b/openrec_b200/csrc/orx_sampler.cu
--- a/openrec_b200/csrc/orx_sampler.cu
+++ b/openrec_b200/csrc/orx_sampler.cu
@@ -150,7 +150,7 @@
   if (rc) return rc;
   ORX_REQUIRE(uid && pid && nid && B >= 0 && (int64_t)B <= sd->n_records, "bad batch (at most one epoch per batch)");
   if (B == 0) return ORX_OK;
-  ORX_CUDA(cudaSetDevice(h->device));
+  ORX_ENTER(h);
   k_sample_pairwise<<<(B + 255) / 256, 256, 0, (cudaStream_t)s>>>(sampler_dev(sd), seed, stream_pos, B, uid, pid, nid);
   ORX_LAUNCH_CHECK();
   return ORX_OK;
@@ -164,7 +164,7 @@
   ORX_REQUIRE(uid && iid && label && n_pos_out && B >= 0 && (int64_t)B <= sd->n_records, "bad batch (at most one epoch per batch)");
   ORX_REQUIRE(pos_ratio >= 0.f && pos_ratio <= 1.f, "pos_ratio must be in [0, 1]");
   if (B == 0) return ORX_OK;
-  ORX_CUDA(cudaSetDevice(h->device));
+  ORX_ENTER(h);
   k_sample_stratified<<<1, 1024, 0, (cudaStream_t)s>>>(sampler_dev(sd), seed, stream_pos, B, pos_ratio, uid, iid, label, n_pos_out);
   ORX_LAUNCH_CHECK();
   return ORX_OK;
@@ -177,7 +177,7 @@
   ORX_REQUIRE(uid && iid && label && B >= 0 && quota >= 0 && quota <= ORX_MAX_QUOTA && quota < sd->total_items, "bad batch / quota");
   ORX_REQUIRE((int64_t)B / (quota + 1) + 2 <= sd->n_records, "at most one epoch of records per batch");
   if (B == 0) return ORX_OK;
-  ORX_CUDA(cudaSetDevice(h->device));
+  ORX_ENTER(h);
   k_sample_per_positive<<<(B + 127) / 128, 128, 0, (cudaStream_t)s>>>(sampler_dev(sd), seed, stream_pos, B, quota, uid, iid, label);
   ORX_LAUNCH_CHECK();
   return ORX_OK;
diff --git a/openrec_b200/csrc/orx_shard.cu b/openrec_b200/csrc/orx_shard.cu
--- a/openrec_b200/csrc/orx_shard.cu
+++ b/openrec_b200/csrc/orx_shard.cu
@@ -805,7 +805,7 @@
   ORX_REQUIRE(opt->kind == ORX_OPT_SGD || opt->kind == ORX_OPT_ADAGRAD || opt->kind == ORX_OPT_ADAM_LAZY,
               "the sharded step supports SGD, Adagrad and row-sparse Adam");
   ORX_REQUIRE(orx_opt_slots_ok(opt->kind, {user, item, item_bias}), "optimizer slot rows missing");
-  ORX_CUDA(cudaSetDevice(h->device));
+  ORX_ENTER(h);
   cudaStream_t st = (cudaStream_t)s;
   const int64_t need = x->home_cap > (x->gin_cap + 1) / 2 ? x->home_cap : (x->gin_cap + 1) / 2;
   if ((rc = orx_ensure_workspace(h, need, x->dim))) return rc;
diff --git a/openrec_b200/csrc/orx_sharded.cu b/openrec_b200/csrc/orx_sharded.cu
--- a/openrec_b200/csrc/orx_sharded.cu
+++ b/openrec_b200/csrc/orx_sharded.cu
@@ -55,7 +55,7 @@
                                          int32_t* slot, orx_stream_t s) {
   ORX_REQUIRE(h != nullptr && ids && counts && send_local && slot, "null pointer");
   ORX_REQUIRE(n >= 0 && n_user >= 0 && n_user <= n && world >= 1 && world <= 1024 && total_users > 0, "bad sizes");
-  ORX_CUDA(cudaSetDevice(h->device));
+  ORX_ENTER(h);
   cudaStream_t st = (cudaStream_t)s;
   ORX_CUDA(cudaMemsetAsync(counts, 0, sizeof(int32_t) * world, st));
   if (n == 0) return ORX_OK;
@@ -142,7 +142,7 @@
   ORX_REQUIRE(n >= 0 && tab->rows > 0 && tab->dim > 0, "bad sizes");
   ORX_REQUIRE(orx_opt_kind_ok(opt->kind), "unknown optimizer kind");
   ORX_REQUIRE(orx_opt_slots_ok(opt->kind, {tab}), "optimizer slot rows missing");
-  ORX_CUDA(cudaSetDevice(h->device));
+  ORX_ENTER(h);
   cudaStream_t st = (cudaStream_t)s;
   const bool dense = opt->kind == ORX_OPT_ADAM_DENSE;
   if (n == 0 && !dense) return ORX_OK;
diff --git a/openrec_b200/native.py b/openrec_b200/native.py
--- a/openrec_b200/native.py
+++ b/openrec_b200/native.py
@@ -128,6 +128,11 @@
         _lib.check(self.lib.orx_debug_dispatch_log(self.h, rec, _lib.ORX_DISPATCH_LOG_CAP, C.byref(n)),
                    "orx_debug_dispatch_log")
         return [Dispatch(*rec[8 * i:8 * i + 8]) for i in range(n.value)]
+
+    def debug_last_prefetch_mode(self):
+        m = C.c_int32()
+        _lib.check(self.lib.orx_debug_last_prefetch_mode(self.h, C.byref(m)), "orx_debug_last_prefetch_mode")
+        return m.value
 
     def pairwise_fwd(self, kind, user, item, bias, uid, pid, nid, out4, margin=0.5):
         _lib.check(self.lib.orx_pairwise_fwd(self.h, kind, C.byref(user), C.byref(item), C.byref(bias), _ptr(uid),
```

Measured after the change: 365.8 million (median of 6 runs). +2.1%, better.
